# ilovin/lstm_ctc_ocr

Measured on AMD Instinct MI355X. Metric: captcha images/sec training (32x256, bs=64/GPU), higher is better.
Workload: dtype bf16; 1 GPU; VGG-7 + BiLSTM(256) + CTC train step, H=32 W=256, 10-char labels, C=64, bs=64/GPU (BASELINE.json configs[1]), Adam lr 1e-4 wd 1e-5 clip 10; global_batch=64, parallelism=dp1, hipgraph=True

## Files before the change

### include/ocr_hip.h

```cpp
#ifndef OCR_HIP_H
#define OCR_HIP_H
#include <stddef.h>
#ifdef __cplusplus
extern "C" {
#endif

enum { OCR_STATUS_OK = 0, OCR_STATUS_MEMOPS = 1, OCR_STATUS_INVALID = 2, OCR_STATUS_EXEC = 3 };

enum {
    OCR_EPI_BIAS = 1, OCR_EPI_RELU = 2, OCR_EPI_OUT_F32 = 4,
    OCR_EPI_MASK = 16, OCR_EPI_ROWSWAP = 32, OCR_EPI_ACCUM = 64
};

const char* ocr_status_string(int status);
int ocr_abi_version(void);
const char* ocr_build_id(void);

int ocr_ctc_workspace_size(int max_label_len, int max_time, int minibatch, size_t* bytes);
int ocr_ctc_loss(const float* activations, float* gradients, const int* flat_labels, const int* label_lengths,
                 const int* input_lengths, int alphabet_size, int minibatch, int max_time, int max_label_len,
                 int blank_label, float* costs, void* workspace, void* stream);
int ocr_ctc_debug(void* dbg);
int ocr_ctc_train_supported(int alphabet_size, int max_time, int max_label_len);
int ocr_ctc_loss_train(const float* activations, void* grad_ntc_bf16, float scale, const int* flat_labels,
                       const int* label_lengths, const int* input_lengths, int alphabet_size, int minibatch, int max_time,
                       int max_label_len, int blank_label, float* costs, void* stream);
int ocr_set_ctc_engine(int fast);
int ocr_ctc_greedy_decode(const float* activations, const int* input_lengths, int alphabet_size, int minibatch,
                          int max_time, int blank_label, int pad_value, int* decoded, int* decoded_lengths,
                          void* stream);

int ocr_ctc_beam_workspace_size(int alphabet_size, int minibatch, int max_time, int beam_width, size_t* bytes);
int ocr_ctc_beam_decode(const float* activations, const int* input_lengths, int alphabet_size, int minibatch,
                        int max_time, int beam_width, int merge_repeated, int pad_value, int* decoded,
                        int* decoded_lengths, float* neg_log_prob, void* workspace, size_t workspace_bytes, void* stream);

int ocr_gemm_nt_bf16(const void* P, long ldp, const void* Q, long ldq, void* out, long ldo, int M, int N, int K,
                     const float* bias, const void* mask, long ldmask, int flags, int splits, int row_group,
                     int row_skip, int swap_inner, int swap_outer, void* stream);
int ocr_set_gemm_engine(int use_large_tile);
int ocr_conv3x3_bf16(const void* x, const void* wpack, void* y, int Nb, int W, int H, int Cin, int Cout,
                     const float* bias, const void* mask, int flags, void* stream);
int ocr_conv3x3_stats_rows(int Nb, int W, int H, int Cin, int Cout, int flags);
int ocr_conv3x3_bf16_stats(const void* x, const void* wpack, void* y, int Nb, int W, int H, int Cin, int Cout, const float* bias, int flags,
                           float* partials, void* stream);
int ocr_conv3x3_kernel_choice(int Nb, int W, int H, int Cin, int Cout, int flags, int kw, int kh);
int ocr_conv3x3_accum_supported(int Nb, int W, int H, int Cin, int Cout);
int ocr_conv_halo_clock_debug(void* dbg);
int ocr_conv_ws_debug(void* dbg);
int ocr_conv3x3_pool_supported(int Nb, int W, int H, int Cin, int Cout, int kw, int kh);
int ocr_conv3x3_relu_pool_bf16(const void* x, const void* wpack, void* y, void* pooled, int Nb, int W, int H, int Cin, int Cout,
                               const float* bias, int kw, int kh, void* stream);
int ocr_gemm_tn_bf16(const void* A, long lda, const void* B, long ldb, float* out, long ldo, int Mk, int I, int J,
                     int row_group, int row_skip, long a_row_off, float scale, int splits, float* colsum, void* stream);
long ocr_gemm_tn_split_workspace_floats(int Mk, int I, int J);
int ocr_gemm_tn_split_bf16(const void* A, long lda, const void* B, long ldb, float* out, long ldo, int Mk, int I, int J, float scale,
                           float* colsum, float* part, long part_floats, void* stream);
int ocr_gemm_tn_batched_bf16(const void* A, long lda, long strideA, const void* B, long ldb, long strideB, float* out, long ldo,
                             long strideOut, int Mk, int I, int J, int nbatch, float scale, int splits, float* colsum,
                             long strideColsum, void* stream);
typedef struct ocr_tn_job {
    const void* A; long lda; long strideA;
    const void* B; long ldb; long strideB;
    float* out; long ldo; long strideOut;
    float* colsum; long strideColsum;
    int Mk, I, J, nbatch;
    int row_group, row_skip;
    float scale; int reserved;
} ocr_tn_job;
int ocr_gemm_tn_jobs_supported(const ocr_tn_job* jobs, int njobs);
int ocr_gemm_tn_jobs_bf16(const ocr_tn_job* jobs, int njobs, void* stream);
int ocr_set_wgrad_engine(int engine);
int ocr_conv3x3_wgrad_bf16(const void* x, const void* dy, float* dw, float* dbias, int Nb, int W, int H, int Cin,
                           int Cout, int splits, void* stream);
int ocr_conv3x3_wgrad_kernel_choice(int Nb, int W, int H, int Cin, int Cout, int has_workspace, int splits);

int ocr_conv3x3_wgrad_workspace_size(int Nb, int W, int H, int Cin, int Cout, size_t* bytes);
int ocr_conv3x3_wgrad_ws_bf16(const void* x, const void* dy, float* dw, float* dbias, int Nb, int W, int H, int Cin,
                              int Cout, int splits, void* workspace, size_t workspace_bytes, void* stream);
int ocr_conv3x3_wgrad_defer_bf16(const void* x, const void* dy, float* dw, float* dbias, int Nb, int W, int H, int Cin, int Cout,
                                 void* workspace, size_t workspace_bytes, void* job, int* job_blocks, int* deferred, void* stream);
int ocr_wgrad9_reduce_jobs(const void* jobs, int njobs, int total_blocks, void* stream);

int ocr_conv1_fwd(const float* x, const float* w, const float* bias, void* y, int Nb, int W, int H, int Cout,
                  int relu, void* stream);
int ocr_conv1_wgrad(const float* x, const void* dz, float* dw, float* db, int Nb, int W, int H, int Cout,
                    void* stream);
int ocr_eltwise_bf16(int op, const void* a, const void* b, void* out, long n, void* stream);
int ocr_conv1_pool_fwd(const float* x, const float* w, const float* bias, void* p, int Nb, int W, int H, int Cout, void* stream);
int ocr_conv1_pool_fwd_train(const float* x, const float* w, const float* bias, void* p, int Nb, int W, int H, int Cout,
                             void* codes, float* zero, long zero_n, void* ones, long ones_n, void* stream);
int ocr_conv1_pool_bwd_codes(const float* x, const float* w, const float* bias, const void* dp, float* dw, float* db,
                             int Nb, int W, int H, int Cout, const void* codes, void* stream);
int ocr_conv1_pool_bwd_slab_rows(int Nb, int W, int H);
int ocr_conv1_pool_bwd_slab(const float* x, const float* w, const float* bias, const void* dp, int Nb, int W, int H, int Cout,
                            const void* codes, float* slab, void* stream);
int ocr_conv1_pool_bwd(const float* x, const float* w, const float* bias, const void* dp, float* dw, float* db, int Nb,
                       int W, int H, int Cout, void* stream);
int ocr_maxpool_fwd(const void* x, void* y, int Nb, int W, int H, int C, int kw, int kh, void* stream);
int ocr_maxpool_bwd(const void* x, const void* dy, void* dx, int Nb, int W, int H, int C, int kw, int kh,
                    int relu_mask, void* stream);
size_t ocr_bn_workspace_bytes(long M, int C);
int ocr_bn_train_fwd(const void* x, void* y, const float* gamma, const float* beta, float* save_mean,
                     float* save_rstd, long M, int C, float eps, int relu, void* workspace, const void* residual, void* stream);
int ocr_bn_train_bwd(const void* x, const void* y, const void* dy, void* dx, const float* gamma,
                     const float* save_mean, const float* save_rstd, float* dgamma, float* dbeta, long M, int C,
                     int relu, void* workspace, void* stream);
int ocr_bn_train_fwd2(const void* x, void* y, const float* gamma, const float* beta, float* save_mean, float* save_rstd, long M, int C,
                      float eps, int relu, void* workspace, const void* residual, int partial_rows, void* pooled, void* stream);
int ocr_bn_train_bwd2(const void* x, const void* y, const void* dy, void* dx, const float* gamma, const float* save_mean,
                      const float* save_rstd, float* dgamma, float* dbeta, long M, int C, int relu, void* workspace, int pooled_dy,
                      int partial_rows, void* stream);
int ocr_conv3x3_bnbwd_rows(int Nb, int W, int H, int Cin, int Cout);
int ocr_conv3x3_dgrad_bnbwd_bf16(const void* dy, const void* wdgrad, void* dx, int Nb, int W, int H, int Cin, int Cout, const void* mask_y,
                                 const void* z, const float* mean, const float* rstd, float* partials, void* stream);
int ocr_colsum_bf16(const void* a, float* out, long M, int C, long lda, void* stream);
int ocr_pack_transpose(const float* in, void* out, int R, int Cc, long ldin, int lstm_units, void* stream);
int ocr_pack_conv_dgrad(const float* w, void* out, int Cin, int Cout, void* stream);
int ocr_pack_jobs(const void* jobs, int njobs, int total_blocks, void* stream);
int ocr_cast_f32_bf16(const float* in, void* out, long n, void* stream);
int ocr_u8_to_unit_f32(const void* in, float* out, long n, void* stream);
int ocr_step_report(const float* costs, int n, const double* scalars, const void* word_addrs, int nwords, double* out, void* stream);
int ocr_bind_batch(const void* pixels, int pixels_are_u8, float* x, long n_pixels, const int* seq_len, int* seq_len_dst, int n_seq,
                   const int* labels, int* labels_dst, int n_labels, const int* labels_len, int* labels_len_dst, int n_labels_len,
                   void* stream);
int ocr_cast2d_f32_bf16(const float* in, long ldin, void* out, long ldout, int rows, int cols, void* stream);
int ocr_tnc_to_ntc_bf16(const float* in, void* out, int T, int N, int C, float scale, void* stream);
int ocr_conv5_col2im(const void* col, void* dx, int Nb, int W, int HC, void* stream);

int ocr_bn_infer_fwd(const void* x, void* y, const float* gamma, const float* beta, const float* mean, const float* var,
                     long M, int C, float eps, int relu, void* stream);
int ocr_bn_infer_bwd(const void* x, const void* y, const void* dy, void* dx, const float* gamma, const float* mean,
                     const float* var, float* dgamma, float* dbeta, long M, int C, float eps, int relu, void* stream);
int ocr_dropout_bf16(const void* in, void* out, long n, unsigned seed, const void* step_counter, float keep_prob, void* stream);
int ocr_avgpool_bf16(const void* src, void* dst, int Nb, int W, int H, int C, int kw, int kh, int backward, void* stream);
int ocr_subsample_bf16(const void* src, void* dst, int Nb, int W, int H, int C, int Wo, int Ho, int sw, int sh, int ow, int oh,
                       int backward, void* stream);
int ocr_softmax_f32(const float* in, float* out, long rows, int C, void* stream);

int ocr_lstm_fwd_step(const float* xproj, const void* whT_packed, const int* seq_len, void* hout, float* gates,
                      float* cell, int Nb, int T, int U, int step, float forget_bias, int ndir, void* stream);
int ocr_lstm_bwd_step(const void* wh, long ldw, long w_dir_stride, const int* seq_len, const void* dhout,
                      const float* gates, const float* cell, void* dz, float* dc_state, int Nb, int T, int U,
                      int step, int ndir, void* stream);
int ocr_lstm_seq_supported(int Nb, int U);
long ocr_lstm_seq_sync_words(int Nb, int U);
int ocr_lstm_seq_debug(void* dbg );
int ocr_lstm_seq_test_skew(int units, int at);
int ocr_lstm_fwd_seq(const float* xproj, const void* whT_packed, const int* seq_len, void* hout, float* gates,
                     float* cell, int Nb, int T, int U, float forget_bias, void* sync, void* stream);
int ocr_lstm_bwd_seq(const void* wh, long ldw, long w_dir_stride, const int* seq_len, const void* dhout,
                     const float* gates, const float* cell, void* dz, int Nb, int T, int U, void* sync, void* stream);
#define OCR_LSTM_PREPARED 1
int ocr_lstm_fwd_seq2(const float* xproj, const void* whT_packed, const int* seq_len, void* hout, float* gates,
                      float* cell, int Nb, int T, int U, float forget_bias, void* sync, int flags, void* stream);
int ocr_lstm_bwd_seq2(const void* wh, long ldw, long w_dir_stride, const int* seq_len, const void* dhout,
                      const float* gates, const float* cell, void* dz, int Nb, int T, int U, void* sync, int flags, void* stream);
int ocr_lstm_fwd_seq_x_supported(int Nb, int U, int D);
int ocr_lstm_fwd_seq_x(const void* x, const void* wxT_packed, const float* bias_packed, int D, const void* whT_packed,
                       const int* seq_len, void* hout, float* gates, float* cell, int Nb, int T, int U, float forget_bias,
                       void* sync, int flags, void* stream);
int ocr_set_lstm_proto(int proto);
int ocr_set_lstm_ksplit(int waves);
int ocr_lstm_hprev(const void* hout, const int* seq_len, void* hprev, int Nb, int T, int U, int ndir, void* stream);
int ocr_lstm_xh(const void* x, const void* hout, const int* seq_len, void* xh, int Nb, int T, int D, int U, int ndir, void* stream);
int ocr_lstm_pack_bias(const float* b_fw, const float* b_bw , float* out, int U, int ndir, void* stream);

int ocr_optim_scalar_count(void);
int ocr_optim_init(void* scalars , double lr, void* stream);
int ocr_optim_set_lr(void* scalars, double lr, int multiply, void* stream);
int ocr_optim_step(float* params, float* grads, float* state1, float* state2, long n, long reg_begin, long reg_end,
                   float weight_decay, float clip_norm, int solver, float beta1, float beta2, float eps,
                   void* scalars, void* stream);
int ocr_optim_step_guarded(float* params, float* grads, float* state1, float* state2, long n, long reg_begin, long reg_end,
                           float weight_decay, float clip_norm, int solver, float beta1, float beta2, float eps,
                           void* scalars, const void* guard_addrs, int nguard, void* stream);
int ocr_optim_step_guarded2(float* params, float* grads, float* state1, float* state2, long n, long reg_begin, long reg_end,
                            float weight_decay, float clip_norm, int solver, float beta1, float beta2, float eps,
                            void* scalars, const void* guard_addrs, int nguard, const float* drop_flag, void* stream);
int ocr_guard_flag(const void* guard_addrs, int nguard, float* flag_out, void* stream);

int ocr_captcha_synth(const int* params, int n_images, int words_per_image, int max_glyphs, const void* atlas, const int* stamp, int n_stamp,
                      void* out, int W, int out_h, int canvas_cap, int width_cap, void* stream);

int ocr_wgrad9_debug(void* dbg);

int ocr_probe_tr16(const int* addr , int* out , void* stream);
int ocr_probe_xcc(int* out , int nblocks, int threads, void* stream);
int ocr_occupy_cus(int nblocks, int threads, int lds_bytes, float us, void* stream);
int ocr_mfma_busy_probe(float* out, int nblocks, int threads , int iters, long long* clk, void* stream);

#ifdef __cplusplus
}
#endif
#endif
// ... 1 lines not shown
```

### lstm_ctc_ocr_amd/_native.py

```python
import ctypes
import os
import re

_HERE = os.path.dirname(os.path.abspath(__file__))
LIB_PATH = os.environ.get("OCR_NATIVE_LIB") or os.path.join(_HERE, "libocrhip.so")
HEADER_PATH = os.path.join(os.path.dirname(_HERE), "include", "ocr_hip.h")

EPI_BIAS, EPI_RELU, EPI_OUT_F32, EPI_MASK, EPI_ROWSWAP, EPI_ACCUM = 1, 2, 4, 16, 32, 64

_P, _I, _L, _F, _D = ctypes.c_void_p, ctypes.c_int, ctypes.c_long, ctypes.c_float, ctypes.c_double

_SIGS = {
    "ocr_abi_version": ([], _I),
    "ocr_build_id": ([], ctypes.c_char_p),
    "ocr_status_string": ([_I], ctypes.c_char_p),
    "ocr_ctc_workspace_size": ([_I, _I, _I, ctypes.POINTER(ctypes.c_size_t)], _I),
    "ocr_ctc_loss": ([_P, _P, _P, _P, _P, _I, _I, _I, _I, _I, _P, _P, _P], _I),
    "ocr_set_ctc_engine": ([_I], _I),
    "ocr_ctc_debug": ([_P], _I),
    "ocr_ctc_train_supported": ([_I, _I, _I], _I),
    "ocr_ctc_loss_train": ([_P, _P, _F, _P, _P, _P, _I, _I, _I, _I, _I, _P, _P], _I),
    "ocr_ctc_greedy_decode": ([_P, _P, _I, _I, _I, _I, _I, _P, _P, _P], _I),
    "ocr_ctc_beam_workspace_size": ([_I, _I, _I, _I, ctypes.POINTER(ctypes.c_size_t)], _I),
    "ocr_ctc_beam_decode": ([_P, _P, _I, _I, _I, _I, _I, _I, _P, _P, _P, _P, ctypes.c_size_t, _P], _I),
    "ocr_gemm_nt_bf16": ([_P, _L, _P, _L, _P, _L, _I, _I, _I, _P, _P, _L, _I, _I, _I, _I, _I, _I, _P], _I),
    "ocr_set_gemm_engine": ([_I], _I),
    "ocr_gemm_tn_batched_bf16": ([_P, _L, _L, _P, _L, _L, _P, _L, _L, _I, _I, _I, _I, _F, _I, _P, _L, _P], _I),
    "ocr_gemm_tn_jobs_supported": ([_P, _I], _I),
    "ocr_gemm_tn_jobs_bf16": ([_P, _I, _P], _I),
    "ocr_lstm_xh": ([_P, _P, _P, _P, _I, _I, _I, _I, _I, _P], _I),
    "ocr_set_wgrad_engine": ([_I], _I),
    "ocr_conv3x3_bf16": ([_P, _P, _P, _I, _I, _I, _I, _I, _P, _P, _I, _P], _I),
    "ocr_conv_halo_clock_debug": ([_P], _I),
    "ocr_occupy_cus": ([_I, _I, _I, _F, _P], _I),
    "ocr_conv_ws_debug": ([_P], _I),
    "ocr_conv3x3_accum_supported": ([_I, _I, _I, _I, _I], _I),
    "ocr_conv3x3_kernel_choice": ([_I, _I, _I, _I, _I, _I, _I, _I], _I),
    "ocr_conv3x3_pool_supported": ([_I, _I, _I, _I, _I, _I, _I], _I),
    "ocr_conv3x3_relu_pool_bf16": ([_P, _P, _P, _P, _I, _I, _I, _I, _I, _P, _I, _I, _P], _I),
    "ocr_gemm_tn_bf16": ([_P, _L, _P, _L, _P, _L, _I, _I, _I, _I, _I, _L, _F, _I, _P, _P], _I),
    "ocr_gemm_tn_split_workspace_floats": ([_I, _I, _I], _L),
    "ocr_gemm_tn_split_bf16": ([_P, _L, _P, _L, _P, _L, _I, _I, _I, _F, _P, _P, _L, _P], _I),
    "ocr_conv3x3_wgrad_bf16": ([_P, _P, _P, _P, _I, _I, _I, _I, _I, _I, _P], _I),
    "ocr_conv3x3_wgrad_kernel_choice": ([_I, _I, _I, _I, _I, _I, _I], _I),
    "ocr_conv3x3_wgrad_workspace_size": ([_I, _I, _I, _I, _I, ctypes.POINTER(ctypes.c_size_t)], _I),
    "ocr_conv3x3_wgrad_ws_bf16": ([_P, _P, _P, _P, _I, _I, _I, _I, _I, _I, _P, ctypes.c_size_t, _P], _I),
    "ocr_conv3x3_wgrad_defer_bf16": ([_P, _P, _P, _P, _I, _I, _I, _I, _I, _P, ctypes.c_size_t, _P, ctypes.POINTER(_I),
                                      ctypes.POINTER(_I), _P], _I),
    "ocr_wgrad9_reduce_jobs": ([_P, _I, _I, _P], _I),
    "ocr_conv1_fwd": ([_P, _P, _P, _P, _I, _I, _I, _I, _I, _P], _I),
    "ocr_conv1_wgrad": ([_P, _P, _P, _P, _I, _I, _I, _I, _P], _I),
    "ocr_eltwise_bf16": ([_I, _P, _P, _P, _L, _P], _I),
    "ocr_conv1_pool_fwd": ([_P, _P, _P, _P, _I, _I, _I, _I, _P], _I),
    "ocr_conv1_pool_fwd_train": ([_P, _P, _P, _P, _I, _I, _I, _I, _P, _P, _L, _P, _L, _P], _I),
    "ocr_conv1_pool_bwd_codes": ([_P, _P, _P, _P, _P, _P, _I, _I, _I, _I, _P, _P], _I),
    "ocr_conv1_pool_bwd_slab_rows": ([_I, _I, _I], _I),
    "ocr_conv1_pool_bwd_slab": ([_P, _P, _P, _P, _I, _I, _I, _I, _P, _P, _P], _I),
    "ocr_conv1_pool_bwd": ([_P, _P, _P, _P, _P, _P, _I, _I, _I, _I, _P], _I),
    "ocr_maxpool_fwd": ([_P, _P, _I, _I, _I, _I, _I, _I, _P], _I),
    "ocr_maxpool_bwd": ([_P, _P, _P, _I, _I, _I, _I, _I, _I, _I, _P], _I),
    "ocr_bn_workspace_bytes": ([_L, _I], ctypes.c_size_t),
    "ocr_bn_train_fwd": ([_P, _P, _P, _P, _P, _P, _L, _I, _F, _I, _P, _P, _P], _I),
    "ocr_bn_train_bwd": ([_P, _P, _P, _P, _P, _P, _P, _P, _P, _L, _I, _I, _P, _P], _I),
    "ocr_bn_train_fwd2": ([_P, _P, _P, _P, _P, _P, _L, _I, _F, _I, _P, _P, _I, _P, _P], _I),
    "ocr_bn_train_bwd2": ([_P, _P, _P, _P, _P, _P, _P, _P, _P, _L, _I, _I, _P, _I, _I, _P], _I),
    "ocr_conv3x3_bnbwd_rows": ([_I, _I, _I, _I, _I], _I),
    "ocr_conv3x3_dgrad_bnbwd_bf16": ([_P, _P, _P, _I, _I, _I, _I, _I, _P, _P, _P, _P, _P, _P], _I),
    "ocr_conv3x3_stats_rows": ([_I, _I, _I, _I, _I, _I], _I),
    "ocr_conv3x3_bf16_stats": ([_P, _P, _P, _I, _I, _I, _I, _I, _P, _I, _P, _P], _I),
    "ocr_bn_infer_fwd": ([_P, _P, _P, _P, _P, _P, _L, _I, _F, _I, _P], _I),
    "ocr_bn_infer_bwd": ([_P, _P, _P, _P, _P, _P, _P, _P, _P, _L, _I, _F, _I, _P], _I),
    "ocr_dropout_bf16": ([_P, _P, _L, ctypes.c_uint, _P, _F, _P], _I),
    "ocr_avgpool_bf16": ([_P, _P, _I, _I, _I, _I, _I, _I, _I, _P], _I),
    "ocr_subsample_bf16": ([_P, _P, _I, _I, _I, _I, _I, _I, _I, _I, _I, _I, _I, _P], _I),
    "ocr_softmax_f32": ([_P, _P, _L, _I, _P], _I),
    "ocr_colsum_bf16": ([_P, _P, _L, _I, _L, _P], _I),
    "ocr_pack_transpose": ([_P, _P, _I, _I, _L, _I, _P], _I),
    "ocr_pack_conv_dgrad": ([_P, _P, _I, _I, _P], _I),
    "ocr_pack_jobs": ([_P, _I, _I, _P], _I),
    "ocr_cast_f32_bf16": ([_P, _P, _L, _P], _I),
    "ocr_u8_to_unit_f32": ([_P, _P, _L, _P], _I),
    "ocr_step_report": ([_P, _I, _P, _P, _I, _P, _P], _I),
    "ocr_bind_batch": ([_P, _I, _P, _L, _P, _P, _I, _P, _P, _I, _P, _P, _I, _P], _I),
    "ocr_captcha_synth": ([_P, _I, _I, _I, _P, _P, _I, _P, _I, _I, _I, _I, _P], _I),
    "ocr_cast2d_f32_bf16": ([_P, _L, _P, _L, _I, _I, _P], _I),
    "ocr_tnc_to_ntc_bf16": ([_P, _P, _I, _I, _I, _F, _P], _I),
    "ocr_conv5_col2im": ([_P, _P, _I, _I, _I, _P], _I),
    "ocr_lstm_fwd_step": ([_P, _P, _P, _P, _P, _P, _I, _I, _I, _I, _F, _I, _P], _I),
    "ocr_lstm_bwd_step": ([_P, _L, _L, _P, _P, _P, _P, _P, _P, _I, _I, _I, _I, _I, _P], _I),
    "ocr_lstm_seq_supported": ([_I, _I], _I),
    "ocr_lstm_seq_debug": ([_P], _I),
    "ocr_lstm_seq_test_skew": ([_I, _I], _I),
    "ocr_lstm_seq_sync_words": ([_I, _I], _L),
    "ocr_lstm_fwd_seq": ([_P, _P, _P, _P, _P, _P, _I, _I, _I, _F, _P, _P], _I),
    "ocr_lstm_bwd_seq": ([_P, _L, _L, _P, _P, _P, _P, _P, _I, _I, _I, _P, _P], _I),
    "ocr_lstm_fwd_seq2": ([_P, _P, _P, _P, _P, _P, _I, _I, _I, _F, _P, _I, _P], _I),
    "ocr_lstm_fwd_seq_x_supported": ([_I, _I, _I], _I),
    "ocr_lstm_fwd_seq_x": ([_P, _P, _P, _I, _P, _P, _P, _P, _P, _I, _I, _I, _F, _P, _I, _P], _I),
    "ocr_lstm_bwd_seq2": ([_P, _L, _L, _P, _P, _P, _P, _P, _I, _I, _I, _P, _I, _P], _I),
    "ocr_lstm_hprev": ([_P, _P, _P, _I, _I, _I, _I, _P], _I),
    "ocr_lstm_pack_bias": ([_P, _P, _P, _I, _I, _P], _I),
    "ocr_optim_scalar_count": ([], _I),
    "ocr_optim_init": ([_P, _D, _P], _I),
    "ocr_optim_set_lr": ([_P, _D, _I, _P], _I),
    "ocr_optim_step": ([_P, _P, _P, _P, _L, _L, _L, _F, _F, _I, _F, _F, _F, _P, _P], _I),
    "ocr_optim_step_guarded": ([_P, _P, _P, _P, _L, _L, _L, _F, _F, _I, _F, _F, _F, _P, _P, _I, _P], _I),
    "ocr_optim_step_guarded2": ([_P, _P, _P, _P, _L, _L, _L, _F, _F, _I, _F, _F, _F, _P, _P, _I, _P, _P], _I),
    "ocr_guard_flag": ([_P, _I, _P, _P], _I),
    "ocr_wgrad9_debug": ([_P], _I),
    "ocr_probe_tr16": ([_P, _P, _P], _I),
    "ocr_set_lstm_proto": ([_I], _I),
    "ocr_set_lstm_ksplit": ([_I], _I),
    "ocr_probe_xcc": ([_P, _I, _I, _P], _I),
    "ocr_mfma_busy_probe": ([_P, _I, _I, _I, _P, _P], _I),
}


class NativeError(RuntimeError):
    pass


def declared_symbols(header=HEADER_PATH):
    text = open(header).read()
    text = re.sub(r"/\*.*?\*/", "", text, flags=re.S)
    return sorted(set(re.findall(r"\b(ocr_[a-z0-9_]+)\s*\(", text)))


def source_build_id(csrc=os.path.join(_HERE, "csrc"), experiments=False):
    import glob
    import hashlib
    rel = [os.path.basename(f) for f in glob.glob(os.path.join(csrc, "*.hip"))]
    h = hashlib.sha256()
    for f in sorted(rel) + ["common.h", "conv_plan.h", "Makefile"]:
        h.update(open(os.path.join(csrc, f), "rb").read())
    return h.hexdigest()[:16] + ("-exp" if experiments else "")


def build_id():
    return lib().ocr_build_id().decode()


_lib = None


def lib():
    global _lib
    if _lib is None:
        if not os.path.exists(LIB_PATH):
# ... 32 lines not shown
```

### lstm_ctc_ocr_amd/csrc/common.h

```cpp
#pragma once
#include <stdlib.h>
#include <hip/hip_runtime.h>
#include <stdint.h>
#include <atomic>

#define OCR_WAVE 64

enum {
    OCR_OK = 0,
    OCR_ERR_MEMOPS = 1,
    OCR_ERR_INVALID = 2,
    OCR_ERR_EXEC = 3,
};

#define OCR_CHECK_LAUNCH()                                        \
    do {                                                          \
        hipError_t e__ = hipGetLastError();                       \
        if (e__ != hipSuccess) return OCR_ERR_EXEC;               \
    } while (0)

typedef uint16_t bf16_t;
typedef __attribute__((ext_vector_type(8))) __bf16 bf16x8;
typedef __attribute__((ext_vector_type(4))) float f32x4;
typedef __attribute__((ext_vector_type(4))) unsigned int u32x4;
typedef __attribute__((ext_vector_type(2))) unsigned int u32x2;

__device__ __forceinline__ bf16_t f2bf(float f) {
    uint32_t u = __float_as_uint(f);
    if ((u & 0x7fffffffu) > 0x7f800000u) return (bf16_t)((u >> 16) | 0x40);
    u += 0x7fffu + ((u >> 16) & 1u);
    return (bf16_t)(u >> 16);
}
__device__ __forceinline__ float bf2f(bf16_t h) { return __uint_as_float(((uint32_t)h) << 16); }
typedef __attribute__((ext_vector_type(2))) __bf16 bf16x2_t;
__device__ __forceinline__ uint32_t pack_bf2(float lo, float hi) {
    bf16x2_t v = {(__bf16)lo, (__bf16)hi};
    return __builtin_bit_cast(uint32_t, v);
}
__device__ __forceinline__ float bf_lo(uint32_t p) { return __uint_as_float(p << 16); }
__device__ __forceinline__ float bf_hi(uint32_t p) { return __uint_as_float(p & 0xffff0000u); }

__device__ __forceinline__ float wave_sum(float v) {
#pragma unroll
    for (int o = 32; o > 0; o >>= 1) v += __shfl_xor(v, o, 64);
    return v;
}
__device__ __forceinline__ float wave_max(float v) {
#pragma unroll
    for (int o = 32; o > 0; o >>= 1) v = fmaxf(v, __shfl_xor(v, o, 64));
    return v;
}

__device__ __forceinline__ float sigmoidf_(float x) { return __frcp_rn(1.0f + __expf(-x)); }
__device__ __forceinline__ float tanhf_(float x) {
    float e = __expf(-2.0f * fabsf(x));
    float t = (1.0f - e) * __frcp_rn(1.0f + e);
    return copysignf(t, x);
}

static inline const char* ocr_tune_env(const char* name) {
#ifdef OCR_EXPERIMENTS
    return getenv(name);
#else
    (void)name; return nullptr;
#endif
}
__device__ __forceinline__ long long ocr_wall_clock() { return (long long)__builtin_amdgcn_s_memrealtime(); }
__device__ __forceinline__ void ocr_clk_enter(long long* clk) {
    clk[0] = (long long)__builtin_amdgcn_s_memtime(); clk[1] = ocr_wall_clock();
}
__device__ __forceinline__ void ocr_clk_exit(long long* clk) {
    const long long c = (long long)__builtin_amdgcn_s_memtime(), t = ocr_wall_clock();
    clk[2] = c; clk[3] = t;
    clk[4] += c - clk[0]; clk[5] += t - clk[1]; clk[6] += 1;
}
__host__ __device__ static inline int ceil_div(long a, long b) { return (int)((a + b - 1) / b); }

#define OCR_MAX_DEVICES 64
template <auto KERNEL>
static inline hipError_t ocr_allow_lds(int bytes) {
    static std::atomic<int> allowed[OCR_MAX_DEVICES];
    int dev = 0;
    if (hipGetDevice(&dev) != hipSuccess || dev < 0 || dev >= OCR_MAX_DEVICES) return hipErrorInvalidDevice;
    int have = allowed[dev].load(std::memory_order_acquire);
    if (bytes <= have) return hipSuccess;
    const hipError_t e = hipFuncSetAttribute((const void*)KERNEL, hipFuncAttributeMaxDynamicSharedMemorySize, bytes);
    if (e != hipSuccess) return e;
    while (have < bytes && !allowed[dev].compare_exchange_weak(have, bytes, std::memory_order_acq_rel)) {}
    return hipSuccess;
}
```

### lstm_ctc_ocr_amd/csrc/conv_k3.hip

```cpp
#include "conv_plan.h"
#include <type_traits>

enum { K3_BIAS = 1, K3_RELU = 2, K3_MASK = 16, K3_ACCUM = 64 };

struct K3Args {
    const bf16_t* P; const bf16_t* Q;
    int M, N, C;
    int cW, cH;
    bf16_t* out; const float* bias; const bf16_t* mask; int flags;
    bf16_t* pool; int pool_kind;
    int prio;
    const bf16_t* bnz; const float* bn_mean; const float* bn_rstd;
};

#ifdef OCR_EXPERIMENTS
__device__ long long* k3_dbg;
extern "C" int ocr_conv_k3_debug(void* dbg) {
    long long* q = (long long*)dbg;
    return hipMemcpyToSymbol(HIP_SYMBOL(k3_dbg), &q, sizeof(q)) == hipSuccess ? OCR_OK : OCR_ERR_MEMOPS;
}
#define K3_PHASE(slot) do { if (k3_dbg && threadIdx.x == 0) k3_dbg[blockIdx.x * 8 + (slot)] = wall_clock64(); } while (0)
#else
#define K3_PHASE(slot) do { } while (0)
#endif
__device__ long long* g_k3_clk;
int k3_set_clock_debug(void* dbg) {
    long long* p = (long long*)dbg;
    return hipMemcpyToSymbol(HIP_SYMBOL(g_k3_clk), &p, sizeof(p)) == hipSuccess ? OCR_OK : OCR_ERR_EXEC;
}
__device__ __forceinline__ uint32_t k3_max2(uint32_t a, uint32_t b) {
    const uint32_t lo = (bf_lo(b) > bf_lo(a)) ? (b & 0xffffu) : (a & 0xffffu);
    const uint32_t hi = (bf_hi(b) > bf_hi(a)) ? (b & 0xffff0000u) : (a & 0xffff0000u);
    return lo | hi;
}
__device__ __forceinline__ u32x4 k3_max8(u32x4 a, u32x4 b) {
    u32x4 r = {k3_max2(a.x, b.x), k3_max2(a.y, b.y), k3_max2(a.z, b.z), k3_max2(a.w, b.w)};
    return r;
}
typedef __attribute__((address_space(3))) void* lptr_t;
#define K3_OOB 0x80000000u
#define K3_VMWAIT(n) asm volatile("s_waitcnt vmcnt(%0)" ::"n"(n) : "memory")

template <int FM , int BN ,
          int NST , int H ,
          bool SINGLE = false ,
          bool GENW = false ,
          bool BNB = false >
__device__ __forceinline__ void k3_body(const K3Args& g) {
    constexpr int NW = 8, FN = 4, BM = 256;
    constexpr int WN = BN / 64, WMW = 4 / WN;
    static_assert(FM * WMW == 16, "256-pixel tiles");
    constexpr int NC = BM / H, NCB = NC / 16;
    constexpr int PS = (NC + 2 + 7) / 8 * 8;
    constexpr int PPIECES = (H * PS / 8 + NW - 1) / NW * NW;
    constexpr int PBYTES = PPIECES * 1024, PI = PPIECES / NW;
    static_assert(H * PS <= PPIECES * 8 && PI <= 8, "planes fit the padded buffer; one piece per tap");
    constexpr int CBW = NCB / WMW > 0 ? NCB / WMW : 1;
    constexpr int HW = FM / CBW;
    constexpr int WGC = NCB / CBW;
    constexpr bool STATIC_H = HW == H;
    constexpr int QI = BN / 64;
    constexpr int QB = BN * 128, QTOT = NST * QB;
    constexpr int DEPTH = NST - 2;
    extern __shared__ __attribute__((aligned(16))) unsigned char smem[];

    const int tid = threadIdx.x, lane = tid & 63;
    K3_PHASE(0);
    long long* const clk = g_k3_clk;
    if (clk && blockIdx.x == 0 && tid == 0) ocr_clk_enter(clk);
    const int wave = __builtin_amdgcn_readfirstlane(tid >> 6);
    const int kh = wave >> 2, wm = (wave & 3) / WN, wn = (wave & 3) % WN;
    const int C = g.C;
    const int cb0 = (wm % WGC) * CBW, hbase = (wm / WGC) * HW;
    const bool top = STATIC_H || hbase == 0, bot = STATIC_H || hbase + HW == H;

    const int mtiles = g.M / BM, ntiles = (g.N + BN - 1) / BN;
    const int nblk = mtiles * ntiles;
    int Lb = blockIdx.x;
    if ((nblk & 7) == 0) Lb = (Lb & 7) * (nblk >> 3) + (Lb >> 3);
    const int m0 = (Lb / ntiles) * BM, n0 = (Lb % ntiles) * BN;
    const int col0 = m0 / H;
    const bool edge_l = col0 % g.cW == 0, edge_r = (col0 + NC) % g.cW == 0;

    const int rsub = lane >> 3;
    const int csrc = ((lane & 7) ^ rsub) * 8;

    const int pbytes_all = (int)((long)g.M * C * 2);
    const __amdgpu_buffer_rsrc_t qsrd = __builtin_amdgcn_make_buffer_rsrc((void*)g.Q, 0, (int)((long)g.N * 9 * C * 2), 0x00020000);
    unsigned voffQ[QI], voffP[PI];
#pragma unroll
    for (int j = 0; j < QI; ++j) {
        const int n = n0 + (wave * QI + j) * 8 + rsub;
        voffQ[j] = n < g.N ? (unsigned)(((long)n * 9 * C + csrc) * 2) : K3_OOB;
    }
    constexpr int KMAX = 8;
    const int b0w = g.cW - col0 % g.cW;
    auto kof = [&](int c) { int k = 0;
#pragma unroll
        for (int i = 0; i < KMAX; ++i) k += (c >= b0w + i * g.cW) ? 1 : 0;
        return k; };
#pragma unroll
    for (int j = 0; j < PI; ++j) {
        const int r = (j * NW + wave) * 8 + rsub;
        const int h = r / PS, cp = r % PS;
        if (!GENW) {
            const bool ok = h < H && cp < NC + 2 && !(cp == 0 && edge_l) && !(cp == NC + 1 && edge_r);
            const long m = (long)(col0 - 1 + cp) * H + h;
            voffP[j] = ok ? (unsigned)((m * C + csrc) * 2) : K3_OOB;
        } else {
            const int q = cp - 1, last = NC + kof(NC - 1);
            int n = 0; bool pad = false;
#pragma unroll
            for (int i = 0; i < KMAX; ++i) { const int z = b0w + i * g.cW + i; n += (q >= z) ? 1 : 0; pad = pad || q == z; }
            int col = col0 + q - n;
            bool ok = h < H && q >= 0 && q < last && !pad;
            if (h < H && q == -1) { ok = !edge_l; col = col0 - 1; }
            if (h < H && q == last) { ok = !edge_r; col = col0 + NC; }
            const long m = (long)col * H + h;
            voffP[j] = ok ? (unsigned)((m * C + csrc) * 2) : K3_OOB;
        }
    }
    auto load_q = [&](int k0 , int stage) {
#pragma unroll
        for (int j = 0; j < QI; ++j)
            __builtin_amdgcn_raw_ptr_buffer_load_lds(qsrd, (lptr_t)(smem + stage * QB + (wave * QI + j) * 1024), 16, (int)voffQ[j], k0 * 2, 0, 0);
    };
    auto load_p = [&](const __amdgpu_buffer_rsrc_t srd, int chunk, int buf, int j, unsigned voff) {
        __builtin_amdgcn_raw_ptr_buffer_load_lds(srd, (lptr_t)(smem + QTOT + buf * PBYTES + (j * NW + wave) * 1024), 16, (int)voff, chunk * 128, 0, 0);
    };

// ... 113 lines not shown
        if (decltype(khc)::value == 1) comp(std::integral_constant<int, 8>{}, khc);
    };
    if (kh == 0) run(std::integral_constant<int, 0>{}); else run(std::integral_constant<int, 1>{});
    asm volatile("s_waitcnt vmcnt(0)" ::: "memory");
    __syncthreads();
    K3_PHASE(2);

    constexpr int FH = FM / 2;
    auto tail = [&](auto half_c) {
        constexpr int KH = decltype(half_c)::value;
        {
            f32x4* mine = (f32x4*)smem + (size_t)wave * (FN * FH * 64);
            const f32x4* theirs = (const f32x4*)smem + (size_t)(wave ^ 4) * (FN * FH * 64);
#pragma unroll
            for (int a = 0; a < FN; ++a)
#pragma unroll
                for (int b = 0; b < FH; ++b) mine[(a * FH + b) * 64 + lane] = acc[a][(1 - KH) * FH + b];
            __syncthreads();
#pragma unroll
            for (int a = 0; a < FN; ++a)
#pragma unroll
                for (int b = 0; b < FH; ++b) acc[a][KH * FH + b] += theirs[(a * FH + b) * 64 + lane];
        }
        K3_PHASE(3);
        const int flags = g.flags;
        f32x4 bv[FN];
#pragma unroll
        for (int a = 0; a < FN; ++a) {
            const int n = n0 + wn * 64 + a * 16 + (lane >> 4) * 4;
            bv[a] = (f32x4){0.f, 0.f, 0.f, 0.f};
            if ((flags & K3_BIAS) && n < g.N) bv[a] = *(const f32x4*)(g.bias + n);
        }
        if (!(flags & K3_ACCUM)) {
            constexpr int ROWB = BN * 2, U = ROWB / 16, SWM = BN == 128 ? 7 : 3;
            __syncthreads();
#pragma unroll
            for (int bb = 0; bb < FH; ++bb) {
                const int b = KH * FH + bb;
                const int lp = ((cb0 + b % CBW) * 16 + frow) * H + hbase + b / CBW;
#pragma unroll
                for (int a = 0; a < FN; ++a) {
                    f32x4 v = acc[a][b] + bv[a];
                    if (flags & K3_RELU) {
                        v.x = fmaxf(v.x, 0.f); v.y = fmaxf(v.y, 0.f); v.z = fmaxf(v.z, 0.f); v.w = fmaxf(v.w, 0.f);
                    }
                    u32x2 pk;
                    pk.x = pack_bf2(v.x, v.y);
                    pk.y = pack_bf2(v.z, v.w);
                    const int slot = wn * 16 + a * 4 + (lane >> 4);
                    *(u32x2*)(smem + lp * ROWB + ((slot ^ ((frow & SWM) << 2)) << 3)) = pk;
                }
            }
            __syncthreads();
            constexpr int NIT = 256 * U / 512;
            u32x4 val[NIT], mk[NIT], zt[BNB ? NIT : 1];
            float st_s[8] = {0.f, 0.f, 0.f, 0.f, 0.f, 0.f, 0.f, 0.f}, st_q[8] = {0.f, 0.f, 0.f, 0.f, 0.f, 0.f, 0.f, 0.f};
            float bmu[8], brs[8];
            if (BNB) {
#pragma unroll
                for (int c = 0; c < 8; ++c) { bmu[c] = g.bn_mean[n0 + (tid % U) * 8 + c]; brs[c] = g.bn_rstd[n0 + (tid % U) * 8 + c]; }
            }
#pragma unroll
            for (int it = 0; it < NIT; ++it) {
                const int idx = it * 512 + tid, lp = idx / U, u = idx % U;
                if (flags & K3_MASK) mk[it] = *(const u32x4*)(g.mask + ((long)m0 + lp) * g.N + n0 + u * 8);
                if (BNB) zt[it] = *(const u32x4*)(g.bnz + ((long)m0 + lp) * g.N + n0 + u * 8);
                val[it] = *(const u32x4*)(smem + lp * ROWB + ((u ^ (((lp / H) & SWM) << 1)) << 4));
            }
#pragma unroll
            for (int it = 0; it < NIT; ++it) {
                const int idx = it * 512 + tid, lp = idx / U, u = idx % U;
                u32x4 v = val[it];
                if (flags & K3_MASK) {
                    const u32x4 q = mk[it];
                    if (!(bf_lo(q.x) > 0.f)) v.x &= 0xffff0000u;
                    if (!(bf_hi(q.x) > 0.f)) v.x &= 0x0000ffffu;
                    if (!(bf_lo(q.y) > 0.f)) v.y &= 0xffff0000u;
                    if (!(bf_hi(q.y) > 0.f)) v.y &= 0x0000ffffu;
                    if (!(bf_lo(q.z) > 0.f)) v.z &= 0xffff0000u;
                    if (!(bf_hi(q.z) > 0.f)) v.z &= 0x0000ffffu;
                    if (!(bf_lo(q.w) > 0.f)) v.w &= 0xffff0000u;
                    if (!(bf_hi(q.w) > 0.f)) v.w &= 0x0000ffffu;
                }
                *(u32x4*)(g.out + ((long)m0 + lp) * g.N + n0 + u * 8) = v;
                if (!BNB && g.pool_kind == 3) {
                    const float f[8] = {bf_lo(v.x), bf_hi(v.x), bf_lo(v.y), bf_hi(v.y), bf_lo(v.z), bf_hi(v.z), bf_lo(v.w), bf_hi(v.w)};
#pragma unroll
                    for (int c = 0; c < 8; ++c) { st_s[c] += f[c]; st_q[c] = fmaf(f[c], f[c], st_q[c]); }
                } else if (BNB) {
                    const u32x4 z = zt[it];
                    const float f[8] = {bf_lo(v.x), bf_hi(v.x), bf_lo(v.y), bf_hi(v.y), bf_lo(v.z), bf_hi(v.z), bf_lo(v.w), bf_hi(v.w)};
                    const float zf[8] = {bf_lo(z.x), bf_hi(z.x), bf_lo(z.y), bf_hi(z.y), bf_lo(z.z), bf_hi(z.z), bf_lo(z.w), bf_hi(z.w)};
#pragma unroll
                    for (int c = 0; c < 8; ++c) { st_s[c] += f[c]; st_q[c] = fmaf(f[c], (zf[c] - bmu[c]) * brs[c], st_q[c]); }
                }
            }
            if (BNB || g.pool_kind == 3) {
                constexpr int RL = 512 / U;
                float* red = (float*)(smem + 256 * ROWB);
                const int u = tid % U, rl = tid / U;
#pragma unroll
                for (int c = 0; c < 8; ++c) { red[rl * BN + u * 8 + c] = st_s[c]; red[(RL + rl) * BN + u * 8 + c] = st_q[c]; }
                __syncthreads();
                if (tid < 2 * BN) {
                    const int which = tid / BN, ch = tid % BN;
                    float t = 0.f;
                    for (int r = 0; r < RL; ++r) t += red[(which * RL + r) * BN + ch];
                    if (n0 + ch < g.N) ((float*)g.pool)[((long)(m0 / 256) * 2 + which) * g.N + n0 + ch] = t;
                }
            } else if (g.pool_kind) {
                const int kind = g.pool_kind;
                const int nq = kind == 1 ? 128 : 64;
                const long pbase = kind == 1 ? ((long)m0 >> 1) : (long)(col0 >> 1) * (H >> 1);
                for (int idx = tid; idx < nq * U; idx += 512) {
                    const int q = idx / U, u = idx % U;
                    int lp0, cl;
                    if (kind == 1) { lp0 = 2 * q; cl = lp0 / H; }
                    else { cl = 2 * (q / (H >> 1)); lp0 = cl * H + 2 * (q % (H >> 1)); }
                    const unsigned char* r0 = smem + lp0 * ROWB;
                    const int u0 = (u ^ ((cl & SWM) << 1)) << 4;
                    u32x4 m = k3_max8(*(const u32x4*)(r0 + u0), *(const u32x4*)(r0 + ROWB + u0));
                    if (kind == 2) {
                        const int u1 = (u ^ (((cl + 1) & SWM) << 1)) << 4;
                        m = k3_max8(m, k3_max8(*(const u32x4*)(r0 + H * ROWB + u1), *(const u32x4*)(r0 + (H + 1) * ROWB + u1)));
                    }
                    *(u32x4*)(g.pool + (pbase + q) * g.N + n0 + u * 8) = m;
                }
            }
            return;
        }
#pragma unroll
        for (int bb = 0; bb < FH; ++bb) {
            const int b = KH * FH + bb;
            const int h = hbase + b / CBW, col = col0 + (cb0 + b % CBW) * 16 + frow;
            const long m = (long)col * H + h;
#pragma unroll
            for (int a = 0; a < FN; ++a) {
                const int n = n0 + wn * 64 + a * 16 + (lane >> 4) * 4;
                if (n >= g.N) continue;
                f32x4 v = acc[a][b] + bv[a];
                if (flags & K3_RELU) {
                    v.x = fmaxf(v.x, 0.f); v.y = fmaxf(v.y, 0.f); v.z = fmaxf(v.z, 0.f); v.w = fmaxf(v.w, 0.f);
                }
                if (flags & K3_MASK) {
                    u32x2 mk = *(const u32x2*)(g.mask + m * g.N + n);
                    if (!(bf_lo(mk.x) > 0.f)) v.x = 0.f;
                    if (!(bf_hi(mk.x) > 0.f)) v.y = 0.f;
                    if (!(bf_lo(mk.y) > 0.f)) v.z = 0.f;
                    if (!(bf_hi(mk.y) > 0.f)) v.w = 0.f;
                }
                if (flags & K3_ACCUM) {
                    const u32x2 old = *(const u32x2*)(g.out + m * g.N + n);
                    v.x += bf_lo(old.x); v.y += bf_hi(old.x); v.z += bf_lo(old.y); v.w += bf_hi(old.y);
                }
                u32x2 pk;
                pk.x = pack_bf2(v.x, v.y);
                pk.y = pack_bf2(v.z, v.w);
                *(u32x2*)(g.out + m * g.N + n) = pk;
            }
        }
    };
    if (kh) tail(std::integral_constant<int, 1>{}); else tail(std::integral_constant<int, 0>{});
    if (clk && blockIdx.x == 0 && tid == 0) ocr_clk_exit(clk);
#ifdef OCR_EXPERIMENTS
    K3_PHASE(4);
    asm volatile("s_waitcnt vmcnt(0)" ::: "memory");
    K3_PHASE(5);
#endif
}

template <int FM, int BN, int NST, int H, bool SINGLE = false>
__global__ __launch_bounds__(512) __attribute__((amdgpu_waves_per_eu(2, 2))) void conv_k3_kernel(K3Args g) { k3_body<FM, BN, NST, H, SINGLE, false>(g); }
template <int FM, int BN, int NST, int H>
__global__ __launch_bounds__(512) __attribute__((amdgpu_waves_per_eu(2, 2))) void conv_k3w_kernel(K3Args g) { k3_body<FM, BN, NST, H, false, true>(g); }
template <int FM, int BN, int NST, int H, bool GENW>
__global__ __launch_bounds__(512) __attribute__((amdgpu_waves_per_eu(2, 2))) void conv_k3b_kernel(K3Args g) { k3_body<FM, BN, NST, H, false, GENW, true>(g); }

template <int FM, int BN, int NST, int H, bool GENW>
static int run_k3b(const K3Args& g, hipStream_t stream) {
    constexpr int PS = (256 / H + 2 + 7) / 8 * 8, PPIECES = (H * PS / 8 + 7) / 8 * 8;
    constexpr int need = NST * BN * 128 + 2 * PPIECES * 1024, xch = 8 * (FM / 2) * 4 * 1024, lds = need > xch ? need : xch;
    static_assert(lds <= 163840 && 256 * BN * 2 + 2 * (512 / (BN / 8)) * BN * 4 <= lds, "LDS");
    if (ocr_allow_lds<conv_k3b_kernel<FM, BN, NST, H, GENW>>(lds) != hipSuccess) return OCR_ERR_EXEC;
    conv_k3b_kernel<FM, BN, NST, H, GENW><<<(g.M / 256) * ((g.N + BN - 1) / BN), 512, lds, stream>>>(g);
    OCR_CHECK_LAUNCH();
    return OCR_OK;
}

template <int FM, int BN, int NST, int H, bool SINGLE = false, bool GENW = false>
static int run_k3(const K3Args& g, hipStream_t stream) {
    constexpr int PS = (256 / H + 2 + 7) / 8 * 8, PPIECES = (H * PS / 8 + 7) / 8 * 8;
    constexpr int need = NST * BN * 128 + (SINGLE ? 1 : 2) * PPIECES * 1024;
    constexpr int xch = 8 * (FM / 2) * 4 * 1024;
    constexpr int lds = need > xch ? need : xch;
    static_assert(lds <= 163840, "LDS");
    static_assert(256 * BN * 2 + 2 * (512 / (BN / 8)) * BN * 4 <= lds, "staged image + the statistics scratch behind it");
    const int mt = g.M / 256, nt = (g.N + BN - 1) / BN;
    if constexpr (GENW) {
        if (ocr_allow_lds<conv_k3w_kernel<FM, BN, NST, H>>(lds) != hipSuccess) return OCR_ERR_EXEC;
        conv_k3w_kernel<FM, BN, NST, H><<<mt * nt, 512, lds, stream>>>(g);
    } else {
        if (ocr_allow_lds<conv_k3_kernel<FM, BN, NST, H, SINGLE>>(lds) != hipSuccess) return OCR_ERR_EXEC;
        conv_k3_kernel<FM, BN, NST, H, SINGLE><<<mt * nt, 512, lds, stream>>>(g);
    }
    OCR_CHECK_LAUNCH();
    return OCR_OK;
}

int launch_k3(const ConvPlan& p, const ConvOperands& o, hipStream_t stream) {
    const K3Args g = {(const bf16_t*)o.x, (const bf16_t*)o.wpack, p.M, p.Cout, p.Cin, p.W, p.H, (bf16_t*)o.y, o.bias, (const bf16_t*)o.mask,
                      p.flags, (bf16_t*)o.pool, p.epi_kind, p.prio, (const bf16_t*)o.bnz, o.bn_mean, o.bn_rstd};
    const int H = p.H;
    const bool A = p.tile == 'A';
    if (p.epi_kind == CONV_EPI_BNBWD) {
        if (A) {
            if (p.genw) return H == 4 ? run_k3b<8, 128, 5, 4, true>(g, stream) : run_k3b<8, 128, 5, 8, true>(g, stream);
            return H == 4 ? run_k3b<8, 128, 5, 4, false>(g, stream) : run_k3b<8, 128, 5, 8, false>(g, stream);
        }
        if (p.genw) return H == 4 ? run_k3b<4, 64, 4, 4, true>(g, stream) : run_k3b<4, 64, 4, 8, true>(g, stream);
        return H == 4 ? run_k3b<4, 64, 4, 4, false>(g, stream) : run_k3b<4, 64, 4, 8, false>(g, stream);
    }
    if (p.genw) {
        if (A) return H == 2 ? run_k3<8, 128, 5, 2, false, true>(g, stream) : H == 4 ? run_k3<8, 128, 5, 4, false, true>(g, stream)
                                                                                   : run_k3<8, 128, 5, 8, false, true>(g, stream);
        return H == 2 ? run_k3<4, 64, 4, 2, false, true>(g, stream) : H == 4 ? run_k3<4, 64, 4, 4, false, true>(g, stream)
                                                                               : run_k3<4, 64, 4, 8, false, true>(g, stream);
    }
    if (A) {
        if (H == 16) return p.single ? run_k3<8, 128, 5, 16, true>(g, stream) : run_k3<8, 128, 4, 16>(g, stream);
        return H == 4 ? run_k3<8, 128, 5, 4>(g, stream) : run_k3<8, 128, 5, 8>(g, stream);
    }
    if (H == 16) return p.single ? run_k3<4, 64, 4, 16, true>(g, stream) : run_k3<4, 64, 4, 16>(g, stream);
    return H == 4 ? run_k3<4, 64, 4, 4>(g, stream) : run_k3<4, 64, 4, 8>(g, stream);
}
```

### lstm_ctc_ocr_amd/csrc/conv_plan.h

```cpp
#pragma once
#include "common.h"

enum {
    CONV_GEMM = 0,
    CONV_HALO = 1,
    CONV_K2 = 2,
    CONV_K3 = 4,
    CONV_WS = 8,
};
enum {
    CONV_EPI_PLAIN = 0,
    CONV_EPI_POOL12 = 1,
    CONV_EPI_POOL22 = 2,
    CONV_EPI_STATS = 3,
    CONV_EPI_BNBWD = 4,
};

struct ConvPlan {
    int family;
    int M, W, H, Cin, Cout;
    int flags, epi_kind;
    char tile;
    int bn, nw;
    bool genw;
    bool single;
    int ws_nc, ws_ksplit;
    int grid, slots, per_slot, xcd_map;
    int prio, stagger, stagger_bit, abl;
    int nst;
    int choice() const {
        if (family == CONV_K2) return CONV_K2 + (tile == 'D');
        if (family == CONV_K3) return CONV_K3 + (tile == 'D') + 2 * genw;
        return family;
    }
};
ConvPlan conv3x3_plan(int M, int W, int H, int Cin, int Cout, int flags, int epi_kind);

struct ConvOperands {
    const void* x; const void* wpack; void* y;
    const float* bias; const void* mask;
    void* pool;
    const void* bnz; const float* bn_mean; const float* bn_rstd;
};
int launch_halo(const ConvPlan& p, const ConvOperands& o, hipStream_t stream);
int launch_k2(const ConvPlan& p, const ConvOperands& o, hipStream_t stream);
int launch_k3(const ConvPlan& p, const ConvOperands& o, hipStream_t stream);
int launch_ws(const ConvPlan& p, const ConvOperands& o, hipStream_t stream);
```

### lstm_ctc_ocr_amd/csrc/conv_ws.hip

```cpp
#include "conv_plan.h"
#include <type_traits>

enum { WS_BIAS = 1, WS_RELU = 2, WS_MASK = 16, WS_ACCUM = 64 };

struct WsArgs {
    const bf16_t* P; const bf16_t* Q;
    int M, N, C, cW, cH;
    bf16_t* out; const float* bias; const bf16_t* mask; int flags;
    bf16_t* pool; int pool_kind;
    int ntiles, slots, per_slot, xcd_map;
};

typedef __attribute__((address_space(3))) void* ws_lptr_t;
#define WS_OOB 0x80000000u

__device__ long long* g_ws_dbg;
extern "C" int ocr_conv_ws_debug(void* dbg) {
    long long* q = (long long*)dbg;
    return hipMemcpyToSymbol(HIP_SYMBOL(g_ws_dbg), &q, sizeof(q)) == hipSuccess ? OCR_OK : OCR_ERR_MEMOPS;
}
#define WS_PHASE(slot) do { if (wsdbg && tid == 0 && (slot) < 64) wsdbg[blockIdx.x * 64 + (slot)] = ocr_wall_clock(); } while (0)
__device__ long long* g_ws_clk;
int ws_set_clock_debug(void* dbg) {
    long long* p = (long long*)dbg;
    return hipMemcpyToSymbol(HIP_SYMBOL(g_ws_clk), &p, sizeof(p)) == hipSuccess ? OCR_OK : OCR_ERR_EXEC;
}

typedef short ws_s16x2 __attribute__((ext_vector_type(2)));
__device__ __forceinline__ uint32_t ws_max2(uint32_t a, uint32_t b) {
    return __builtin_bit_cast(uint32_t, __builtin_elementwise_max(__builtin_bit_cast(ws_s16x2, a), __builtin_bit_cast(ws_s16x2, b)));
}
__device__ __forceinline__ u32x4 ws_max8(u32x4 a, u32x4 b) {
    u32x4 r = {ws_max2(a.x, b.x), ws_max2(a.y, b.y), ws_max2(a.z, b.z), ws_max2(a.w, b.w)};
    return r;
}

template <int H, int NC, int KSPLIT>
struct WsCfg {
    static constexpr int BM = NC * H;
    static constexpr int PG = 4 / KSPLIT;
    static constexpr int CF = NC < 16 ? NC : 16;
    static constexpr int HF = 16 / CF;
    static constexpr int HW = 4 * HF;
    static constexpr int PS = NC + 2;
    static constexpr int CHB = (H + 2) * PS * 128;
    static constexpr int BUFB = KSPLIT * CHB;
    static constexpr int PPC = H * PS / 8;
    static constexpr int PI = KSPLIT * PPC / 4;
    static constexpr int NFE = 4 / KSPLIT;
    static constexpr int HWE = NFE * HF;
    static constexpr int NPE = NC * HWE;
    static constexpr int XOFF = 2 * BUFB;
    static constexpr int SOFF = XOFF + (KSPLIT == 2 ? 4 * 8192 : 0);
    static constexpr int STW = NPE * 128;
    static constexpr int TOFF = SOFF + 4 * STW;
    static constexpr int BOFF = TOFF + 4 * PI * 128;
    static constexpr int MOFF = BOFF + 256;
    static constexpr int LDS_PLAIN = MOFF, LDS_MASK = MOFF + 4 * STW;
    static_assert(((NC + 1) * H + H) * 128 * 2 / 16 * 4 < 65536, "table entries fit 16 bits");
    static_assert(NC == CF && PG * HW == H && (H * PS) % 8 == 0 && (KSPLIT * PPC) % 4 == 0 && LDS_MASK <= 163840, "geometry");
    static_assert(((H + 1) * PS) * 128 < 65536, "ds_read immediates");
};

template <int H, int NC, int KSPLIT, bool MASK >
__global__ __launch_bounds__(256) __attribute__((amdgpu_waves_per_eu(1, 1))) void conv_ws_kernel(WsArgs g) {
    using G = WsCfg<H, NC, KSPLIT>;
    constexpr int CF = G::CF, HF = G::HF, PS = G::PS, PI = G::PI, HWE = G::HWE, NPE = G::NPE;
    extern __shared__ __attribute__((aligned(16))) unsigned char smem[];

    const int tid = threadIdx.x, lane = tid & 63, lane_id = lane;
    long long* const clk = g_ws_clk;
    long long* const wsdbg = g_ws_dbg;
    if (clk && blockIdx.x == 0 && tid == 0) ocr_clk_enter(clk);
    WS_PHASE(0);
    const int wave = __builtin_amdgcn_readfirstlane(tid >> 6);
    const int pg = KSPLIT == 1 ? wave : (wave & 1), kh = KSPLIT == 1 ? 0 : (wave >> 1);
    const int C = g.C, N = g.N;

    int id = blockIdx.x, nt, slot;
    if (g.xcd_map) {
        const int per_xcd = (int)gridDim.x >> 3, j = id >> 3;
        nt = j % g.ntiles; slot = (id & 7) * (per_xcd / g.ntiles) + j / g.ntiles;
    } else { nt = id % g.ntiles; slot = id / g.ntiles; }
    const int n0 = nt * 64;
    const int mtiles = g.M / G::BM;
    const int t_begin = slot * g.per_slot;
    int t_end = t_begin + g.per_slot; if (t_end > mtiles) t_end = mtiles;

    const int frow = lane & 15, fq = lane >> 4;
    const int rsub = lane >> 3;
    const unsigned lds0 = (unsigned)(size_t)(ws_lptr_t)smem;

    unsigned short* const dtab = (unsigned short*)(smem + G::TOFF) + wave * PI * 64 + lane;
#pragma unroll
    for (int j = 0; j < PI; ++j) {
        const int q = j * 4 + wave;
        const int c = q / G::PPC, pc = q % G::PPC;
        const int r = pc * 8 + rsub;
        const int h = r / PS, cp = r % PS;
        const unsigned off = (unsigned)((((cp * H + h) * C + c * 64) + (((lane & 7) ^ (cp & 7)) << 3)) * 2);
        dtab[j * 64] = (unsigned short)((off >> 2) | (cp == 0 ? 1u : 0u) | (cp == NC + 1 ? 2u : 0u));
    }
    if (tid < 64) ((float*)(smem + G::BOFF))[tid] = (g.flags & WS_BIAS) ? g.bias[n0 + tid] : 0.f;
    const long pbytes = (long)g.M * C * 2;
    unsigned e_[PI];
    auto read_table = [&]() {
#pragma unroll
        for (int j = 0; j < PI; ++j) e_[j] = dtab[j * 64];
    };
    auto issue_halo = [&](int t, int buf, auto partc) {
        constexpr int PART = decltype(partc)::value;
        const int col0 = t * NC;
        const bool edge_l = col0 % g.cW == 0, edge_r = (col0 + NC) % g.cW == 0;
        const long base = (long)(col0 - 1) * H * C * 2;
        long left = pbytes - base; if (left > 0x7fffffffL) left = 0x7fffffffL;
        const __amdgpu_buffer_rsrc_t srd = __builtin_amdgcn_make_buffer_rsrc((void*)((const char*)g.P + base), 0, (int)left, 0x00020000);
        const unsigned em = (edge_l ? 1u : 0u) | (edge_r ? 2u : 0u);
#pragma unroll
        for (int j = (PART < 0 ? 0 : PART); j < (PART < 0 ? PI : PART + 1); ++j) {
            const int q = j * 4 + wave;
            const unsigned e = e_[j];
            const unsigned v = (e & em) ? WS_OOB : ((e & ~3u) << 2);
            __builtin_amdgcn_raw_ptr_buffer_load_lds(srd, (ws_lptr_t)(smem + buf * G::BUFB + (q / G::PPC) * G::CHB + PS * 128 + (q % G::PPC) * 1024), 16, (int)v, 0, 0, 0);
        }
    };

    unsigned pb[3][2];
    {
        const int colf = frow % CF, hsub = frow / CF;
#pragma unroll
        for (int d = 0; d < 3; ++d)
#pragma unroll
            for (int j = 0; j < 2; ++j) {
                const int cp = colf + d;
                pb[d][j] = lds0 + kh * G::CHB + ((pg * 4 * HF + hsub) * PS + cp) * 128 + (((j * 4 + fq) ^ (cp & 7)) << 4);
            }
    }

    asm volatile("s_waitcnt lgkmcnt(0)" ::: "memory");
    read_table();
    if (t_begin < t_end) issue_halo(t_begin, 0, std::integral_constant<int, -1>{});

    u32x4 wq[4][18];
    {
        constexpr int NSH = 4 / KSPLIT, R = KSPLIT == 1 ? 2 : 4, FR = 72 / R, OWN = 72 / NSH;
        static_assert(KSPLIT * FR * 1024 <= G::BUFB && FR % NSH == 0, "a round fits buffer 1");
        const int rank = KSPLIT == 1 ? wave : pg;
// ... 61 lines not shown
#pragma unroll
        for (int a = 0; a < 4; ++a) {
            binit[a] = *(const f32x4*)(smem + G::BOFF + (a * 16 + fq * 4) * 4);
            if (KSPLIT == 2 && kh) binit[a] = (f32x4){0.f, 0.f, 0.f, 0.f};
        }
        asm volatile("s_waitcnt lgkmcnt(0)" : "+v"(binit[0]), "+v"(binit[1]), "+v"(binit[2]), "+v"(binit[3]));
        f32x4 acc[4][4];
        u32x4 bfr[2][4];
#define WS_RD(S_, DST_) do { \
            constexpr int TAP_ = (S_) >> 1, J_ = (S_) & 1, DW_ = TAP_ / 3, DH_ = TAP_ % 3 - 1; \
            asm volatile("ds_read_b128 %0, %1 offset:%2" : "=v"(DST_[0]) : "v"(pb[DW_][J_]), "n"(((0 * HF + 1 + DH_) * PS) * 128)); \
            asm volatile("ds_read_b128 %0, %1 offset:%2" : "=v"(DST_[1]) : "v"(pb[DW_][J_]), "n"(((1 * HF + 1 + DH_) * PS) * 128)); \
            asm volatile("ds_read_b128 %0, %1 offset:%2" : "=v"(DST_[2]) : "v"(pb[DW_][J_]), "n"(((2 * HF + 1 + DH_) * PS) * 128)); \
            asm volatile("ds_read_b128 %0, %1 offset:%2" : "=v"(DST_[3]) : "v"(pb[DW_][J_]), "n"(((3 * HF + 1 + DH_) * PS) * 128)); \
        } while (0)
#define WS_MM(S_, SRC_, FIRST_) do { \
            _Pragma("unroll") for (int b = 0; b < 4; ++b) \
            _Pragma("unroll") for (int a = 0; a < 4; ++a) \
                acc[a][b] = __builtin_amdgcn_mfma_f32_16x16x32_bf16(__builtin_bit_cast(bf16x8, wq[a][S_]), __builtin_bit_cast(bf16x8, SRC_[b]), \
                                                                    (FIRST_) ? binit[a] : acc[a][b], 0, 0, 0); \
        } while (0)
#define WS_WAIT(N_, SRC_) asm volatile("s_waitcnt lgkmcnt(" #N_ ")" : "+v"(SRC_[0]), "+v"(SRC_[1]), "+v"(SRC_[2]), "+v"(SRC_[3]))
#define WS_STEP(S_) do { \
            WS_RD((S_) + 1, bfr[((S_) + 1) & 1]); \
            WS_WAIT(4, bfr[(S_) & 1]);               \
            WS_MM(S_, bfr[(S_) & 1], (S_) == 0); \
            __builtin_amdgcn_sched_barrier(0); \
        } while (0)
        WS_RD(0, bfr[0]);
        WS_STEP(0); WS_STEP(1); WS_STEP(2); WS_STEP(3); WS_STEP(4); WS_STEP(5); WS_STEP(6); WS_STEP(7); WS_STEP(8);
        WS_STEP(9); WS_STEP(10); WS_STEP(11); WS_STEP(12); WS_STEP(13); WS_STEP(14); WS_STEP(15); WS_STEP(16);
        WS_WAIT(0, bfr[1]);
        WS_MM(17, bfr[1], false);
        __builtin_amdgcn_sched_barrier(0);
#undef WS_STEP
#undef WS_WAIT
#undef WS_MM
#undef WS_RD
        WS_PHASE(ph0 + 2);
        asm volatile("s_waitcnt vmcnt(0)" ::: "memory");
        WS_PHASE(ph0 + 3);

        auto tail = [&](auto khc) {
            constexpr int KH = decltype(khc)::value;
            constexpr int B0 = KSPLIT == 2 ? 2 * KH : 0;
            if (KSPLIT == 2) {
                f32x4* mine = (f32x4*)(smem + G::XOFF) + (size_t)wave * 512;
                const f32x4* theirs = (const f32x4*)(smem + G::XOFF) + (size_t)(wave ^ 2) * 512;
#pragma unroll
                for (int a = 0; a < 4; ++a)
#pragma unroll
                    for (int i = 0; i < 2; ++i) mine[(a * 2 + i) * 64 + lane_id] = acc[a][2 * (1 - KH) + i];
                asm volatile("s_waitcnt lgkmcnt(0)" ::: "memory");
                __builtin_amdgcn_s_barrier();
                asm volatile("" ::: "memory");
#pragma unroll
                for (int a = 0; a < 4; ++a)
#pragma unroll
                    for (int i = 0; i < 2; ++i) acc[a][B0 + i] += theirs[(a * 2 + i) * 64 + lane_id];
            }
            WS_PHASE(ph0 + 4);
            int lane = lane_id;
            asm volatile("" : "+v"(lane));
            const int frow = lane & 15, fq = lane >> 4;
            unsigned char* const S = smem + G::SOFF + wave * G::STW;
            const int colf = frow % CF, hsub = frow / CF;
            const bool relu = (g.flags & WS_RELU) != 0;
#pragma unroll
            for (int i = 0; i < G::NFE; ++i) {
                const int row = colf * HWE + i * HF + hsub;
#pragma unroll
                for (int a = 0; a < 4; ++a) {
                    const f32x4 v = acc[a][B0 + i];
                    u32x2 pk;
                    pk.x = pack_bf2(v.x, v.y);
                    pk.y = pack_bf2(v.z, v.w);
                    if (relu) { pk.x = ws_max2(pk.x, 0u); pk.y = ws_max2(pk.y, 0u); }
                    const int slot = a * 4 + fq;
                    *(u32x2*)(S + row * 128 + ((slot ^ ((colf & 3) << 2)) << 3)) = pk;
                }
            }
            asm volatile("s_waitcnt lgkmcnt(0)" ::: "memory");
            u32x4 val[NIT], mkv[MASK ? NIT : 1];
#pragma unroll
            for (int it = 0; it < NIT; ++it) {
                const int idx = it * 64 + lane, row = idx >> 3, u = idx & 7;
                val[it] = *(const u32x4*)(S + row * 128 + ((u ^ (((row / HWE) & 3) << 1)) << 4));
                if (has_mask) mkv[it] = *(const u32x4*)(smem + G::MOFF + wave * G::STW + idx * 16);
            }
#pragma unroll
            for (int it = 0; it < NIT; ++it) {
                const int idx = it * 64 + lane, row = idx >> 3, u = idx & 7;
                u32x4 v = val[it];
                if (has_mask) {
                    const u32x4 q = mkv[it];
                    if (!(bf_lo(q.x) > 0.f)) v.x &= 0xffff0000u;
                    if (!(bf_hi(q.x) > 0.f)) v.x &= 0x0000ffffu;
                    if (!(bf_lo(q.y) > 0.f)) v.y &= 0xffff0000u;
                    if (!(bf_hi(q.y) > 0.f)) v.y &= 0x0000ffffu;
                    if (!(bf_lo(q.z) > 0.f)) v.z &= 0xffff0000u;
                    if (!(bf_hi(q.z) > 0.f)) v.z &= 0x0000ffffu;
                    if (!(bf_lo(q.w) > 0.f)) v.w &= 0xffff0000u;
                    if (!(bf_hi(q.w) > 0.f)) v.w &= 0x0000ffffu;
                }
                const long m = (long)(col0 + row / HWE) * H + h_lo + row % HWE;
                *(u32x4*)(g.out + m * N + n0 + u * 8) = v;
            }
            if (g.pool_kind == 1) {
                constexpr int NQ = NC * (HWE / 2), PIT = NQ * 8 / 64;
                static_assert(NQ * 8 % 64 == 0, "whole wave iterations");
                u32x4 p0[PIT], p1[PIT];
#pragma unroll
                for (int it = 0; it < PIT; ++it) {
                    const int idx = it * 64 + lane, q = idx >> 3, u = idx & 7, col = q / (HWE / 2), ph = q % (HWE / 2);
                    const unsigned char* r0 = S + (col * HWE + 2 * ph) * 128 + ((u ^ ((col & 3) << 1)) << 4);
                    p0[it] = *(const u32x4*)r0; p1[it] = *(const u32x4*)(r0 + 128);
                }
#pragma unroll
                for (int it = 0; it < PIT; ++it) {
                    const int idx = it * 64 + lane, q = idx >> 3, u = idx & 7, col = q / (HWE / 2), ph = q % (HWE / 2);
                    const long pm = (long)(col0 + col) * (H / 2) + (h_lo >> 1) + ph;
                    *(u32x4*)(g.pool + pm * N + n0 + u * 8) = ws_max8(p0[it], p1[it]);
                }
            } else if (g.pool_kind == 2) {
                constexpr int NQ = (NC / 2) * (HWE / 2), PIT = NQ * 8 / 64;
                static_assert(NQ * 8 % 64 == 0, "whole wave iterations");
                u32x4 p0[PIT], p1[PIT], p2[PIT], p3[PIT];
#pragma unroll
                for (int it = 0; it < PIT; ++it) {
                    const int idx = it * 64 + lane, q = idx >> 3, u = idx & 7, pc = q / (HWE / 2), ph = q % (HWE / 2);
                    const int c0 = 2 * pc, c1 = c0 + 1;
                    const unsigned char* r0 = S + (c0 * HWE + 2 * ph) * 128 + ((u ^ ((c0 & 3) << 1)) << 4);
                    const unsigned char* r1 = S + (c1 * HWE + 2 * ph) * 128 + ((u ^ ((c1 & 3) << 1)) << 4);
                    p0[it] = *(const u32x4*)r0; p1[it] = *(const u32x4*)(r0 + 128); p2[it] = *(const u32x4*)r1; p3[it] = *(const u32x4*)(r1 + 128);
                }
#pragma unroll
                for (int it = 0; it < PIT; ++it) {
                    const int idx = it * 64 + lane, q = idx >> 3, u = idx & 7, pc = q / (HWE / 2), ph = q % (HWE / 2);
                    const long pm = (long)((col0 >> 1) + pc) * (H / 2) + (h_lo >> 1) + ph;
                    *(u32x4*)(g.pool + pm * N + n0 + u * 8) = ws_max8(ws_max8(p0[it], p1[it]), ws_max8(p2[it], p3[it]));
                }
            }
        };
        if (KSPLIT == 2 && kh) tail(std::integral_constant<int, 1>{}); else tail(std::integral_constant<int, 0>{});
        WS_PHASE(ph0 + 5);
        const unsigned flip = buf ? (unsigned)-G::BUFB : (unsigned)G::BUFB;
#pragma unroll
        for (int d = 0; d < 3; ++d)
#pragma unroll
            for (int j = 0; j < 2; ++j) pb[d][j] += flip;
    }
    if (clk && blockIdx.x == 0 && tid == 0) ocr_clk_exit(clk);
}

template <int H, int NC, int KSPLIT, bool MASK>
static int launch_ws_(const WsArgs& g, int grid, hipStream_t stream) {
    using G = WsCfg<H, NC, KSPLIT>;
    constexpr int lds = MASK ? G::LDS_MASK : G::LDS_PLAIN;
    if (ocr_allow_lds<conv_ws_kernel<H, NC, KSPLIT, MASK>>(lds) != hipSuccess) return OCR_ERR_EXEC;
    conv_ws_kernel<H, NC, KSPLIT, MASK><<<grid, 256, lds, stream>>>(g);
    OCR_CHECK_LAUNCH();
    return OCR_OK;
}
template <int H, int NC, int KSPLIT>
static int launch_ws(const WsArgs& g, int grid, hipStream_t stream) {
    return (g.flags & WS_MASK) ? launch_ws_<H, NC, KSPLIT, true>(g, grid, stream) : launch_ws_<H, NC, KSPLIT, false>(g, grid, stream);
}
int launch_ws(const ConvPlan& p, const ConvOperands& o, hipStream_t stream) {
    const WsArgs g = {(const bf16_t*)o.x, (const bf16_t*)o.wpack, p.M, p.Cout, p.Cin, p.W, p.H, (bf16_t*)o.y, o.bias, (const bf16_t*)o.mask,
                      p.flags, (bf16_t*)o.pool, p.epi_kind, p.Cout / 64, p.slots, p.per_slot, p.xcd_map};
    if (p.H == 16 && p.ws_ksplit == 1) return launch_ws<16, 16, 1>(g, p.grid, stream);
    if (p.H == 16) return launch_ws<16, 8, 2>(g, p.grid, stream);
    return launch_ws<8, 16, 2>(g, p.grid, stream);
}
```

### lstm_ctc_ocr_amd/csrc/gemm.hip

```cpp
#include "conv_plan.h"
#include <string.h>

enum {
    EPI_BIAS = 1,
    EPI_RELU = 2,
    EPI_OUT_F32 = 4,
    EPI_ATOMIC = 8,
    EPI_MASK = 16,
    EPI_ROWSWAP = 32,
    EPI_ACCUM = 64,
};

struct GemmArgs {
    const bf16_t* P;
    const bf16_t* Q;
    long ldp, ldq;
    int M, N, K;
    int k_per_split;
    int grp, skip;
    int cW, cH, cC;
    void* out;
    long ldo;
    const float* bias;
    const bf16_t* mask;
// ... 390 lines not shown
        if (M % (epi_kind == CONV_EPI_POOL22 ? 2 * H : 2)) return p;
    }
    if (k.k2 && plan_k3_k2(p, k)) return p;
    plan_halo(p, k);
    return p;
}

static int conv3x3_launch(const ConvPlan& p, const ConvOperands& o, hipStream_t stream) {
    switch (p.family) {
    case CONV_WS: return launch_ws(p, o, stream);
    case CONV_K3: return launch_k3(p, o, stream);
    case CONV_K2: return launch_k2(p, o, stream);
    case CONV_HALO: return launch_halo(p, o, stream);
    }
    return OCR_ERR_INVALID;
}
static int conv3x3_pixels(int Nb, int W, int H, int Cin, int Cout) {
    const long M = (long)Nb * W * H;
    return (Nb <= 0 || W <= 0 || H <= 0 || Cin <= 0 || Cout <= 0 || M > 0x7fffffffL) ? 0 : (int)M;
}

extern "C" int ocr_conv3x3_accum_supported(int Nb, int W, int H, int Cin, int Cout) {
    return conv3x3_plan(conv3x3_pixels(Nb, W, H, Cin, Cout), W, H, Cin, Cout, EPI_ACCUM, CONV_EPI_PLAIN).family != CONV_GEMM;
}
extern "C" int ocr_conv3x3_kernel_choice(int Nb, int W, int H, int Cin, int Cout, int flags, int kw, int kh) {
    if (Nb <= 0 || W <= 0 || H <= 0 || Cin <= 0 || Cout <= 0) return -OCR_ERR_INVALID;
    const int pool_kind = (kw == 1 && kh == 2) ? 1 : ((kw == 2 && kh == 2) ? 2 : 0);
    if ((kw || kh) && !pool_kind) return 0;
    return conv3x3_plan(Nb * W * H, W, H, Cin, Cout, flags & ~(EPI_ATOMIC | EPI_ROWSWAP), pool_kind).choice();
}

extern "C" int ocr_conv3x3_bf16(const void* x, const void* wpack, void* y, int Nb, int W, int H,
                                int Cin, int Cout, const float* bias, const void* mask, int flags,
                                void* stream) {
    GemmArgs g = {};
    g.P = (const bf16_t*)x; g.Q = (const bf16_t*)wpack; g.ldp = Cin; g.ldq = 9L * Cin;
    g.M = Nb * W * H; g.N = Cout; g.K = 9 * Cin; g.cW = W; g.cH = H; g.cC = Cin;
    g.out = y; g.ldo = Cout; g.bias = bias; g.mask = (const bf16_t*)mask; g.ldmask = Cout;
    g.flags = flags & ~(EPI_ATOMIC | EPI_ROWSWAP);
    if ((flags & EPI_BIAS) && !bias) return OCR_ERR_INVALID;
    if ((flags & EPI_MASK) && !mask) return OCR_ERR_INVALID;
    if ((flags & EPI_ACCUM) && !ocr_conv3x3_accum_supported(Nb, W, H, Cin, Cout)) return OCR_ERR_INVALID;
    if (!x || !wpack || !y || g.M <= 0 || Cout <= 0 || Cin <= 0) return dispatch_gemm(g, 1, 1, (hipStream_t)stream);
    const ConvPlan p = conv3x3_plan(g.M, W, H, Cin, Cout, g.flags, CONV_EPI_PLAIN);
    if (p.family != CONV_GEMM) return conv3x3_launch(p, {x, wpack, y, bias, mask}, (hipStream_t)stream);
    if (g_use_igemm) {
        int rc = ig_try_dispatch(x, Cin, wpack, 9L * Cin, y, Cout, g.M, Cout, 9 * Cin, bias, mask, Cout, g.flags, 1, 0, 0, W, H, Cin,
                                 0, 0, (hipStream_t)stream);
        if (rc >= 0) return rc;
    }
    return dispatch_gemm(g, 1, 1, (hipStream_t)stream);
}
extern "C" int ocr_conv3x3_stats_rows(int Nb, int W, int H, int Cin, int Cout, int flags) {
    const int M = conv3x3_pixels(Nb, W, H, Cin, Cout);
    return conv3x3_plan(M, W, H, Cin, Cout, flags & ~(EPI_ATOMIC | EPI_ROWSWAP), CONV_EPI_STATS).family != CONV_GEMM ? M / 256 : 0;
}
extern "C" int ocr_conv3x3_bf16_stats(const void* x, const void* wpack, void* y, int Nb, int W, int H, int Cin, int Cout, const float* bias,
                                      int flags, float* partials, void* stream) {
    if (!x || !wpack || !y || !partials || ((flags & EPI_BIAS) && !bias) || !ocr_conv3x3_stats_rows(Nb, W, H, Cin, Cout, flags)) return OCR_ERR_INVALID;
    const ConvPlan p = conv3x3_plan(Nb * W * H, W, H, Cin, Cout, flags & ~(EPI_ATOMIC | EPI_ROWSWAP), CONV_EPI_STATS);
    return conv3x3_launch(p, {x, wpack, y, bias, nullptr, partials}, (hipStream_t)stream);
}
extern "C" int ocr_conv3x3_bnbwd_rows(int Nb, int W, int H, int Cin, int Cout) {
    const int M = conv3x3_pixels(Nb, W, H, Cin, Cout);
    return conv3x3_plan(M, W, H, Cin, Cout, EPI_MASK, CONV_EPI_BNBWD).family != CONV_GEMM ? M / 256 : 0;
}
extern "C" int ocr_conv3x3_dgrad_bnbwd_bf16(const void* dy, const void* wdgrad, void* dx, int Nb, int W, int H, int Cin, int Cout, const void* mask_y,
                                            const void* z, const float* mean, const float* rstd, float* partials, void* stream) {
    if (!dy || !wdgrad || !dx || !mask_y || !z || !mean || !rstd || !partials || !ocr_conv3x3_bnbwd_rows(Nb, W, H, Cin, Cout)) return OCR_ERR_INVALID;
    const ConvPlan p = conv3x3_plan(Nb * W * H, W, H, Cin, Cout, EPI_MASK, CONV_EPI_BNBWD);
    return conv3x3_launch(p, {dy, wdgrad, dx, nullptr, mask_y, partials, z, mean, rstd}, (hipStream_t)stream);
}
static int conv3x3_pool_kind(int kw, int kh) { return (kw == 1 && kh == 2) ? 1 : ((kw == 2 && kh == 2) ? 2 : 0); }
extern "C" int ocr_conv3x3_pool_supported(int Nb, int W, int H, int Cin, int Cout, int kw, int kh) {
    const int kind = conv3x3_pool_kind(kw, kh);
    return kind && conv3x3_plan(conv3x3_pixels(Nb, W, H, Cin, Cout), W, H, Cin, Cout, EPI_BIAS | EPI_RELU, kind).family != CONV_GEMM;
}
extern "C" int ocr_conv3x3_relu_pool_bf16(const void* x, const void* wpack, void* y, void* pooled, int Nb, int W, int H, int Cin,
                                          int Cout, const float* bias, int kw, int kh, void* stream) {
    if (!x || !wpack || !y || !pooled || !bias || !ocr_conv3x3_pool_supported(Nb, W, H, Cin, Cout, kw, kh)) return OCR_ERR_INVALID;
    const ConvPlan p = conv3x3_plan(Nb * W * H, W, H, Cin, Cout, EPI_BIAS | EPI_RELU, conv3x3_pool_kind(kw, kh));
    return conv3x3_launch(p, {x, wpack, y, bias, nullptr, pooled}, (hipStream_t)stream);
}
```

### lstm_ctc_ocr_amd/csrc/nn_ops.hip

```cpp
#include "common.h"
#include <stdlib.h>

__device__ __forceinline__ void unpack8(u32x4 p, float* f) {
    f[0] = bf_lo(p.x); f[1] = bf_hi(p.x); f[2] = bf_lo(p.y); f[3] = bf_hi(p.y);
    f[4] = bf_lo(p.z); f[5] = bf_hi(p.z); f[6] = bf_lo(p.w); f[7] = bf_hi(p.w);
}

__global__ __launch_bounds__(256) void conv1_fwd_kernel(const float* __restrict__ x,
                                                        const float* __restrict__ w,
                                                        const float* __restrict__ bias,
                                                        bf16_t* __restrict__ y, int Nb, int W, int H,
                                                        int Cout, int relu) {
    const int groups = Cout >> 3;
    const int gq = threadIdx.x % groups;
    const int plane = threadIdx.x / groups;
    const int planes = 256 / groups;
    float wr[9][8], br[8];
#pragma unroll
    for (int t = 0; t < 9; ++t)
#pragma unroll
        for (int c = 0; c < 8; ++c) wr[t][c] = w[t * Cout + gq * 8 + c];
#pragma unroll
    for (int c = 0; c < 8; ++c) br[c] = bias[gq * 8 + c];
    const long npix = (long)Nb * W * H;
// ... 428 lines not shown
}
__device__ __forceinline__ u32x4 max8(u32x4 a, u32x4 b) {
    u32x4 r = {max2(a.x, b.x), max2(a.y, b.y), max2(a.z, b.z), max2(a.w, b.w)};
    return r;
}

template <int KW, int KH>
__global__ __launch_bounds__(256) void maxpool_fwd_kernel(const bf16_t* __restrict__ x, bf16_t* __restrict__ y,
                                                          int Nb, int W, int H, int C) {
    constexpr int kw = KW, kh = KH;
    const int Wo = W / kw, Ho = H / kh, groups = C >> 3;
    const long total = (long)Nb * Wo * Ho * groups;
    for (long idx = (long)blockIdx.x * 256 + threadIdx.x; idx < total; idx += (long)gridDim.x * 256) {
        int gq = (int)(idx % groups);
        long op = idx / groups;
        int ho = (int)(op % Ho);
        long q = op / Ho;
        int wo = (int)(q % Wo);
        long n = q / Wo;
        const bf16_t* base = x + (((n * W + (long)wo * kw) * H) + (long)ho * kh) * C + gq * 8;
        u32x4 m = *(const u32x4*)base;
#pragma unroll
        for (int a = 0; a < kw; ++a)
#pragma unroll
            for (int b = 0; b < kh; ++b) {
                if (a == 0 && b == 0) continue;
                m = max8(m, *(const u32x4*)(base + ((long)a * H + b) * C));
            }
        *(u32x4*)(y + op * C + gq * 8) = m;
    }
}

template <int KW, int KH>
__global__ __launch_bounds__(256) void maxpool_bwd_kernel(const bf16_t* __restrict__ x, const bf16_t* __restrict__ dy,
                                                          bf16_t* __restrict__ dx, int Nb, int W, int H, int C,
                                                          int relu_mask) {
    constexpr int kw = KW, kh = KH, cnt_all = KW * KH;
    const int Wo = W / kw, Ho = H / kh, groups = C >> 3;
    const long total = (long)Nb * Wo * Ho * groups;
    for (long idx = (long)blockIdx.x * 256 + threadIdx.x; idx < total; idx += (long)gridDim.x * 256) {
        int gq = (int)(idx % groups);
        long op = idx / groups;
        int ho = (int)(op % Ho);
        long q = op / Ho;
        int wo = (int)(q % Wo);
        long n = q / Wo;
        long boff = (((n * W + (long)wo * kw) * H) + (long)ho * kh) * C + gq * 8;
        float xv[cnt_all][8];
#pragma unroll
        for (int a = 0; a < kw; ++a)
#pragma unroll
            for (int b = 0; b < kh; ++b) {
                u32x4 v = *(const u32x4*)(x + boff + ((long)a * H + b) * C);
                unpack8(v, xv[a * kh + b]);
            }
        float g[8];
        unpack8(*(const u32x4*)(dy + op * C + gq * 8), g);
        int win[8];
#pragma unroll
        for (int c = 0; c < 8; ++c) {
            int best = 0; float bv = xv[0][c];
#pragma unroll
            for (int e = 1; e < cnt_all; ++e) if (xv[e][c] > bv) { bv = xv[e][c]; best = e; }
            win[c] = best;
        }
#pragma unroll
        for (int a = 0; a < kw; ++a)
#pragma unroll
            for (int b = 0; b < kh; ++b) {
                const int cnt = a * kh + b;
                float o[8];
#pragma unroll
                for (int c = 0; c < 8; ++c) {
                    float v = (win[c] == cnt) ? g[c] : 0.f;
                    if (relu_mask && !(xv[cnt][c] > 0.f)) v = 0.f;
                    o[c] = v;
                }
                u32x4 pk = {pack_bf2(o[0], o[1]), pack_bf2(o[2], o[3]), pack_bf2(o[4], o[5]), pack_bf2(o[6], o[7])};
                *(u32x4*)(dx + boff + ((long)a * H + b) * C) = pk;
            }
    }
}

template <typename AccT, bool STORE = false>
__device__ __forceinline__ void block_channel_reduce(const float (&v)[8], float* red, AccT* dst, int C, int groups,
                                                     int rl, int gq, int rlanes) {
    __syncthreads();
    if (rl < rlanes) {
#pragma unroll
        for (int c = 0; c < 8; ++c) red[rl * C + gq * 8 + c] = v[c];
    }
    __syncthreads();
    for (int ch = threadIdx.x; ch < C; ch += 256) {
        float t = 0.f;
        for (int r = 0; r < rlanes; ++r) t += red[r * C + ch];
        if (STORE) dst[ch] = (AccT)t;
        else atomicAdd(&dst[ch], (AccT)t);
    }
}

static int bn_rows_per_block_host(long M, int target) {
    long r = (M + target - 1) / target;
    r = (r + 7) / 8 * 8;
    return (int)(r < 8 ? 8 : r);
}
__global__ __launch_bounds__(256) void bn_stats_kernel(const bf16_t* __restrict__ x, float* __restrict__ part,
                                                       long M, int C, int rows_per_block) {
    const int groups = C >> 3;
    const int rl = threadIdx.x / groups;
    const int gq = threadIdx.x % groups;
    const int rlanes = 256 / groups;
    const long r0 = (long)blockIdx.x * rows_per_block, r1 = min(M, r0 + rows_per_block);
    float s[8], ss[8];
#pragma unroll
    for (int c = 0; c < 8; ++c) { s[c] = 0.f; ss[c] = 0.f; }
    if (rl < rlanes) {
#pragma unroll 4
        for (long r = r0 + rl; r < r1; r += rlanes) {
            float v[8];
            unpack8(*(const u32x4*)(x + r * C + gq * 8), v);
#pragma unroll
            for (int c = 0; c < 8; ++c) { s[c] += v[c]; ss[c] = fmaf(v[c], v[c], ss[c]); }
        }
    }
    __shared__ float red[2048];
    float* dst = part + (long)blockIdx.x * 2 * C;
    block_channel_reduce<float, true>(s, red, dst, C, groups, rl, gq, rlanes);
    block_channel_reduce<float, true>(ss, red, dst + C, C, groups, rl, gq, rlanes);
}
__device__ __forceinline__ bool bn_pair_sum(const float* __restrict__ part, int nblk, int C, double& t0, double& t1, int& ch) {
    __shared__ double red[2][16][17];
    const int cl = threadIdx.x & 15, rl = threadIdx.x >> 4;
    ch = blockIdx.x * 16 + cl;
    double a0 = 0, a1 = 0;
    if (ch < C) {
#pragma unroll 4
        for (int b = rl; b < nblk; b += 16) {
            a0 += (double)part[(long)b * 2 * C + ch];
            a1 += (double)part[(long)b * 2 * C + C + ch];
        }
    }
    red[0][rl][cl] = a0; red[1][rl][cl] = a1;
    __syncthreads();
    if (rl != 0 || ch >= C) return false;
    t0 = 0; t1 = 0;
#pragma unroll
    for (int r = 0; r < 16; ++r) { t0 += red[0][r][cl]; t1 += red[1][r][cl]; }
    return true;
}
__global__ __launch_bounds__(256) void bn_finalize_kernel(const float* __restrict__ part, int nblk, float* __restrict__ mean,
                                                          float* __restrict__ rstd, long M, int C, float eps) {
    double s, ss; int c;
    if (bn_pair_sum(part, nblk, C, s, ss, c)) {
        double mu = s / (double)M;
        double var = ss / (double)M - mu * mu;
        if (var < 0) var = 0;
        mean[c] = (float)mu;
        rstd[c] = (float)(1.0 / sqrt(var + (double)eps));
    }
}
__global__ __launch_bounds__(256) void bn_apply_kernel(const bf16_t* __restrict__ x, bf16_t* __restrict__ y,
                                                       const float* __restrict__ mean, const float* __restrict__ rstd,
                                                       const float* __restrict__ gamma, const float* __restrict__ beta,
                                                       long M, int C, int relu, int rows_per_block, const bf16_t* __restrict__ res) {
    const int groups = C >> 3;
    const int rl = threadIdx.x / groups, gq = threadIdx.x % groups, rlanes = 256 / groups;
    if (rl >= rlanes) return;
    float mu[8], rs[8], gm[8], bt[8];
#pragma unroll
    for (int c = 0; c < 8; ++c) {
        const int ch = gq * 8 + c;
        mu[c] = mean[ch]; rs[c] = rstd[ch]; gm[c] = gamma[ch]; bt[c] = beta[ch];
    }
    const long r0 = (long)blockIdx.x * rows_per_block, r1 = min(M, r0 + rows_per_block);
#pragma unroll 4
    for (long r = r0 + rl; r < r1; r += rlanes) {
        float v[8], o[8];
        unpack8(*(const u32x4*)(x + r * C + gq * 8), v);
#pragma unroll
        for (int c = 0; c < 8; ++c) o[c] = (v[c] - mu[c]) * rs[c] * gm[c] + bt[c];
        if (res != nullptr) {
            float q[8];
            unpack8(*(const u32x4*)(res + r * C + gq * 8), q);
            u32x4 rb = {pack_bf2(o[0], o[1]), pack_bf2(o[2], o[3]), pack_bf2(o[4], o[5]), pack_bf2(o[6], o[7])};
            unpack8(rb, o);
#pragma unroll
            for (int c = 0; c < 8; ++c) o[c] += q[c];
        }
        if (relu) {
#pragma unroll
            for (int c = 0; c < 8; ++c) o[c] = fmaxf(o[c], 0.f);
        }
        u32x4 pk = {pack_bf2(o[0], o[1]), pack_bf2(o[2], o[3]), pack_bf2(o[4], o[5]), pack_bf2(o[6], o[7])};
        *(u32x4*)(y + r * C + gq * 8) = pk;
    }
}
__global__ __launch_bounds__(256) void bn_apply_pool_kernel(const bf16_t* __restrict__ x, bf16_t* __restrict__ y, bf16_t* __restrict__ pooled,
                                                            const float* __restrict__ mean, const float* __restrict__ rstd,
                                                            const float* __restrict__ gamma, const float* __restrict__ beta,
                                                            long M, int C, int relu, int pairs_per_block) {
    const int groups = C >> 3;
    const int rl = threadIdx.x / groups, gq = threadIdx.x % groups, rlanes = 256 / groups;
    if (rl >= rlanes) return;
    float mu[8], rs[8], gm[8], bt[8];
#pragma unroll
    for (int c = 0; c < 8; ++c) {
        const int ch = gq * 8 + c;
        mu[c] = mean[ch]; rs[c] = rstd[ch]; gm[c] = gamma[ch]; bt[c] = beta[ch];
    }
    const long q0 = (long)blockIdx.x * pairs_per_block, q1 = min(M >> 1, q0 + pairs_per_block);
#pragma unroll 2
    for (long q = q0 + rl; q < q1; q += rlanes) {
        u32x4 pk[2];
#pragma unroll
        for (int e = 0; e < 2; ++e) {
            float v[8], o[8];
            unpack8(*(const u32x4*)(x + (2 * q + e) * C + gq * 8), v);
#pragma unroll
            for (int c = 0; c < 8; ++c) {
                o[c] = (v[c] - mu[c]) * rs[c] * gm[c] + bt[c];
                if (relu) o[c] = fmaxf(o[c], 0.f);
            }
            pk[e] = (u32x4){pack_bf2(o[0], o[1]), pack_bf2(o[2], o[3]), pack_bf2(o[4], o[5]), pack_bf2(o[6], o[7])};
            *(u32x4*)(y + (2 * q + e) * C + gq * 8) = pk[e];
        }
        *(u32x4*)(pooled + q * C + gq * 8) = max8(pk[0], pk[1]);
    }
}
__device__ __forceinline__ void bn_pool_route(const bf16_t* __restrict__ y, const bf16_t* __restrict__ dp, long r, int C, int gq,
                                              const float (&yv)[8], float (&g)[8]) {
    float other[8];
    unpack8(*(const u32x4*)(y + (r ^ 1) * C + gq * 8), other);
    unpack8(*(const u32x4*)(dp + (r >> 1) * C + gq * 8), g);
    const bool odd = (r & 1) != 0;
#pragma unroll
    for (int c = 0; c < 8; ++c) {
        const bool win = odd ? (yv[c] > other[c]) : !(other[c] > yv[c]);
        if (!win) g[c] = 0.f;
    }
}
__global__ __launch_bounds__(256) void bn_bwd_stats_kernel(const bf16_t* __restrict__ x, const bf16_t* __restrict__ y,
                                                           const bf16_t* __restrict__ dy, const float* __restrict__ mean,
                                                           const float* __restrict__ rstd, float* __restrict__ part,
                                                           long M, int C, int rows_per_block, int relu, int pooled) {
    const int groups = C >> 3;
    const int rl = threadIdx.x / groups, gq = threadIdx.x % groups, rlanes = 256 / groups;
    const long r0 = (long)blockIdx.x * rows_per_block, r1 = min(M, r0 + rows_per_block);
    float s[8], sx[8], mu[8], rs[8];
#pragma unroll
    for (int c = 0; c < 8; ++c) { s[c] = 0.f; sx[c] = 0.f; mu[c] = mean[gq * 8 + c]; rs[c] = rstd[gq * 8 + c]; }
    if (rl < rlanes) {
#pragma unroll 4
        for (long r = r0 + rl; r < r1; r += rlanes) {
            float xv[8], yv[8], g[8];
            unpack8(*(const u32x4*)(x + r * C + gq * 8), xv);
            if (relu || pooled) unpack8(*(const u32x4*)(y + r * C + gq * 8), yv);
            if (pooled) bn_pool_route(y, dy, r, C, gq, yv, g);
            else unpack8(*(const u32x4*)(dy + r * C + gq * 8), g);
            if (relu) {
#pragma unroll
                for (int c = 0; c < 8; ++c) if (!(yv[c] > 0.f)) g[c] = 0.f;
            }
#pragma unroll
            for (int c = 0; c < 8; ++c) { s[c] += g[c]; sx[c] = fmaf(g[c], (xv[c] - mu[c]) * rs[c], sx[c]); }
        }
    }
    __shared__ float red[2048];
    float* dst = part + (long)blockIdx.x * 2 * C;
    block_channel_reduce<float, true>(s, red, dst, C, groups, rl, gq, rlanes);
    block_channel_reduce<float, true>(sx, red, dst + C, C, groups, rl, gq, rlanes);
}
__global__ __launch_bounds__(256) void bn_bwd_finalize_kernel(const float* __restrict__ part, int nblk, double* __restrict__ sums,
                                                              float* __restrict__ dgamma, float* __restrict__ dbeta, int C) {
    double s, sx; int c;
    if (bn_pair_sum(part, nblk, C, s, sx, c)) {
        sums[c] = s; sums[C + c] = sx;
        dbeta[c] += (float)s;
        dgamma[c] += (float)sx;
    }
}
__global__ __launch_bounds__(256) void bn_bwd_apply_kernel(const bf16_t* __restrict__ x, const bf16_t* __restrict__ y,
                                                           const bf16_t* __restrict__ dy, bf16_t* __restrict__ dx,
                                                           const float* __restrict__ mean, const float* __restrict__ rstd,
                                                           const float* __restrict__ gamma, const double* __restrict__ sums,
                                                           float* __restrict__ dgamma, float* __restrict__ dbeta,
                                                           long M, int C, int relu, int rows_per_block, int pooled) {
    const int groups = C >> 3;
    const int rl = threadIdx.x / groups, gq = threadIdx.x % groups, rlanes = 256 / groups;
    if (rl >= rlanes) return;
    const double invM = 1.0 / (double)M;
    float mu[8], rs[8], gr[8], mdz[8], mdzx[8];
#pragma unroll
    for (int c = 0; c < 8; ++c) {
        const int ch = gq * 8 + c;
        mu[c] = mean[ch]; rs[c] = rstd[ch]; gr[c] = gamma[ch] * rstd[ch];
        mdz[c] = (float)(sums[ch] * invM); mdzx[c] = (float)(sums[C + ch] * invM);
    }
    const long r0 = (long)blockIdx.x * rows_per_block, r1 = min(M, r0 + rows_per_block);
#pragma unroll 2
    for (long r = r0 + rl; r < r1; r += rlanes) {
        float xv[8], yv[8], g[8], o[8];
        unpack8(*(const u32x4*)(x + r * C + gq * 8), xv);
        if (relu || pooled) unpack8(*(const u32x4*)(y + r * C + gq * 8), yv);
        if (pooled) bn_pool_route(y, dy, r, C, gq, yv, g);
        else unpack8(*(const u32x4*)(dy + r * C + gq * 8), g);
        if (relu) {
#pragma unroll
            for (int c = 0; c < 8; ++c) if (!(yv[c] > 0.f)) g[c] = 0.f;
        }
#pragma unroll
        for (int c = 0; c < 8; ++c) {
            float xh = (xv[c] - mu[c]) * rs[c];
            o[c] = gr[c] * (g[c] - mdz[c] - xh * mdzx[c]);
        }
        u32x4 pk = {pack_bf2(o[0], o[1]), pack_bf2(o[2], o[3]), pack_bf2(o[4], o[5]), pack_bf2(o[6], o[7])};
        *(u32x4*)(dx + r * C + gq * 8) = pk;
    }
}

#ifdef OCR_EXPERIMENTS
struct BnBar { unsigned cnt[16][32]; unsigned gen[16][32]; unsigned gcnt[32]; unsigned timeouts[32]; };
__device__ BnBar bn_bar;
__device__ __forceinline__ bool bn_grid_barrier(unsigned nblocks) {
    __syncthreads();
    __shared__ int ok_s;
    if (threadIdx.x == 0) {
        int ok = 1;
        __threadfence();
        const unsigned g = blockIdx.x & 15u, ngroups = nblocks < 16u ? nblocks : 16u, ng = (nblocks - g + 15u) >> 4;
        const unsigned gen = __hip_atomic_load(&bn_bar.gen[g][0], __ATOMIC_RELAXED, __HIP_MEMORY_SCOPE_AGENT);
        const unsigned prev = __hip_atomic_fetch_add(&bn_bar.cnt[g][0], 1u, __ATOMIC_RELAXED, __HIP_MEMORY_SCOPE_AGENT);
        bool released = false;
        if (prev == ng - 1) {
            __hip_atomic_store(&bn_bar.cnt[g][0], 0u, __ATOMIC_RELAXED, __HIP_MEMORY_SCOPE_AGENT);
            const unsigned gp = __hip_atomic_fetch_add(&bn_bar.gcnt[0], 1u, __ATOMIC_RELAXED, __HIP_MEMORY_SCOPE_AGENT);
            if (gp == ngroups - 1) {
                __hip_atomic_store(&bn_bar.gcnt[0], 0u, __ATOMIC_RELAXED, __HIP_MEMORY_SCOPE_AGENT);
                for (unsigned k = 0; k < ngroups; ++k) __hip_atomic_store(&bn_bar.gen[k][0], gen + 1u, __ATOMIC_RELAXED, __HIP_MEMORY_SCOPE_AGENT);
                released = true;
            }
        }
        if (!released) {
            long spins = 0;
            while (__hip_atomic_load(&bn_bar.gen[g][0], __ATOMIC_RELAXED, __HIP_MEMORY_SCOPE_AGENT) == gen) {
                __builtin_amdgcn_s_sleep(2);
                if (++spins > (1L << 22)) { ok = 0; atomicAdd(&bn_bar.timeouts[0], 1u); break; }
            }
        }
        __threadfence();
        ok_s = ok;
    }
    __syncthreads();
    return ok_s != 0;
}
constexpr int BNF_NIT = 16;
__device__ __forceinline__ void bnf_pair_total(const float* __restrict__ part, int nblk, int C, int ch, double* red , double& t0, double& t1) {
    double a0 = 0, a1 = 0;
    for (int b = threadIdx.x; b < nblk; b += 256) { a0 += (double)part[(long)b * 2 * C + ch]; a1 += (double)part[(long)b * 2 * C + C + ch]; }
    red[threadIdx.x] = a0; red[256 + threadIdx.x] = a1;
    __syncthreads();
    for (int s = 128; s > 0; s >>= 1) {
        if (threadIdx.x < s) { red[threadIdx.x] += red[threadIdx.x + s]; red[256 + threadIdx.x] += red[256 + threadIdx.x + s]; }
        __syncthreads();
    }
    t0 = red[0]; t1 = red[256];
    __syncthreads();
}
__global__ __launch_bounds__(256) void bn_fused_fwd_kernel(const bf16_t* __restrict__ x, bf16_t* __restrict__ y, const float* __restrict__ gamma,
                                                           const float* __restrict__ beta, float* __restrict__ mean, float* __restrict__ rstd,
                                                           float* __restrict__ part, long M, int C, float eps, int relu, int rows_per_block,
                                                           const bf16_t* __restrict__ res) {
    const int groups = C >> 3, rl = threadIdx.x / groups, gq = threadIdx.x % groups, rlanes = 256 / groups;
    const long r0 = (long)blockIdx.x * rows_per_block, r1 = min(M, r0 + rows_per_block);
    const bool act = rl < rlanes;
    u32x4 v[BNF_NIT];
    float s[8], ss[8];
#pragma unroll
    for (int c = 0; c < 8; ++c) { s[c] = 0.f; ss[c] = 0.f; }
#pragma unroll
    for (int i = 0; i < BNF_NIT; ++i) {
        const long r = r0 + rl + (long)i * rlanes;
        v[i] = (u32x4){0, 0, 0, 0};
        if (act && r < r1) v[i] = *(const u32x4*)(x + r * C + gq * 8);
    }
#pragma unroll
    for (int i = 0; i < BNF_NIT; ++i) {
        float f[8];
        unpack8(v[i], f);
#pragma unroll
        for (int c = 0; c < 8; ++c) { s[c] += f[c]; ss[c] = fmaf(f[c], f[c], ss[c]); }
    }
// ... 440 lines not shown
                                                                                                 zero_n / 4, nullptr, (u32x4*)ones, ones_n / 4);
    }
    OCR_CHECK_LAUNCH();
    return OCR_OK;
}
extern "C" int ocr_conv1_pool_fwd(const float* x, const float* w, const float* bias, void* p, int Nb, int W, int H, int Cout,
                                  void* stream) {
    return conv1_pool_fwd_impl(x, w, bias, p, Nb, W, H, Cout, nullptr, 0, nullptr, nullptr, 0, stream);
}
extern "C" int ocr_conv1_pool_fwd_train(const float* x, const float* w, const float* bias, void* p, int Nb, int W, int H, int Cout,
                                        void* codes, float* zero, long zero_n, void* ones, long ones_n, void* stream) {
    return conv1_pool_fwd_impl(x, w, bias, p, Nb, W, H, Cout, zero, zero_n, codes, ones, ones_n, stream);
}
static int conv1_ppb() {
    static int v = -1;
    if (v < 0) { const char* e = getenv("OCR_CONV1_PPB"); v = e ? atoi(e) : 256; if (v < 32 || v > 1024 || (v & 31)) v = 256; }
    return v;
}
static int conv1_pool_bwd_impl(const float* x, const float* w, const float* bias, const void* dp, float* dw, float* db,
                               int Nb, int W, int H, int Cout, const void* codes, float* slab, void* stream) {
    if (!x || !w || !bias || !dp || (!slab && (!dw || !db)) || Cout != 64 || (W & 1) || (H & 1) || ((size_t)codes & 3)) return OCR_ERR_INVALID;
    long npix = (long)Nb * (W / 2) * (H / 2);
    int ppb = slab ? conv1_ppb() : 256;
#ifdef OCR_EXPERIMENTS
    if (!codes && !slab && !conv1_v1() && npix < 0x7fffffffL - 512 && (long)Nb * W * H < 0x7fffffffL)
        conv1_pool_bwd2_kernel<<<ceil_div(npix, ppb), 256, 0, (hipStream_t)stream>>>(x, w, bias, (const bf16_t*)dp, dw, db, Nb, W, H,
                                                                                     Cout, ppb);
    else
#endif
    {
        if (codes) conv1_pool_bwd_kernel<true><<<ceil_div(npix, ppb), 256, 0, (hipStream_t)stream>>>(x, w, bias, (const bf16_t*)dp, dw, db, Nb, W, H,
                                                                                                   Cout, ppb, (const uint32_t*)codes, slab);
        else conv1_pool_bwd_kernel<false><<<ceil_div(npix, ppb), 256, 0, (hipStream_t)stream>>>(x, w, bias, (const bf16_t*)dp, dw, db, Nb, W, H,
                                                                                               Cout, ppb, nullptr, slab);
    }
    OCR_CHECK_LAUNCH();
    return OCR_OK;
}
extern "C" int ocr_conv1_pool_bwd(const float* x, const float* w, const float* bias, const void* dp, float* dw, float* db,
                                  int Nb, int W, int H, int Cout, void* stream) {
    return conv1_pool_bwd_impl(x, w, bias, dp, dw, db, Nb, W, H, Cout, nullptr, nullptr, stream);
}
extern "C" int ocr_conv1_pool_bwd_codes(const float* x, const float* w, const float* bias, const void* dp, float* dw, float* db,
                                        int Nb, int W, int H, int Cout, const void* codes, void* stream) {
    if (!codes) return OCR_ERR_INVALID;
    return conv1_pool_bwd_impl(x, w, bias, dp, dw, db, Nb, W, H, Cout, codes, nullptr, stream);
}
extern "C" int ocr_conv1_pool_bwd_slab_rows(int Nb, int W, int H) {
    if (Nb <= 0 || W <= 0 || H <= 0 || (W & 1) || (H & 1)) return 0;
    return (int)ceil_div((long)Nb * (W / 2) * (H / 2), (long)conv1_ppb());
}
extern "C" int ocr_conv1_pool_bwd_slab(const float* x, const float* w, const float* bias, const void* dp, int Nb, int W, int H, int Cout,
                                       const void* codes, float* slab, void* stream) {
    if (!slab || ((size_t)slab & 15)) return OCR_ERR_INVALID;
    return conv1_pool_bwd_impl(x, w, bias, dp, nullptr, nullptr, Nb, W, H, Cout, codes, slab, stream);
}
extern "C" int ocr_maxpool_fwd(const void* x, void* y, int Nb, int W, int H, int C, int kw, int kh, void* stream) {
    if (!x || !y || (C & 7) || kw < 1 || kw > 2 || kh < 1 || kh > 2 || W % kw || H % kh) return OCR_ERR_INVALID;
    long total = (long)Nb * (W / kw) * (H / kh) * (C >> 3);
    const bf16_t* xi = (const bf16_t*)x; bf16_t* yo = (bf16_t*)y;
    hipStream_t st = (hipStream_t)stream;
    int gr = grid_for(total, 8192);
    if (kw == 2 && kh == 2) maxpool_fwd_kernel<2, 2><<<gr, 256, 0, st>>>(xi, yo, Nb, W, H, C);
    else if (kw == 1 && kh == 2) maxpool_fwd_kernel<1, 2><<<gr, 256, 0, st>>>(xi, yo, Nb, W, H, C);
    else if (kw == 2 && kh == 1) maxpool_fwd_kernel<2, 1><<<gr, 256, 0, st>>>(xi, yo, Nb, W, H, C);
    else return OCR_ERR_INVALID;
    OCR_CHECK_LAUNCH();
    return OCR_OK;
}
extern "C" int ocr_maxpool_bwd(const void* x, const void* dy, void* dx, int Nb, int W, int H, int C, int kw, int kh,
                               int relu_mask, void* stream) {
    if (!x || !dy || !dx || (C & 7) || kw < 1 || kw > 2 || kh < 1 || kh > 2 || W % kw || H % kh) return OCR_ERR_INVALID;
    long total = (long)Nb * (W / kw) * (H / kh) * (C >> 3);
    const bf16_t* xi = (const bf16_t*)x; const bf16_t* dyi = (const bf16_t*)dy; bf16_t* dxo = (bf16_t*)dx;
    hipStream_t st = (hipStream_t)stream;
    int gr = grid_for(total, 8192);
    if (kw == 2 && kh == 2) maxpool_bwd_kernel<2, 2><<<gr, 256, 0, st>>>(xi, dyi, dxo, Nb, W, H, C, relu_mask);
    else if (kw == 1 && kh == 2) maxpool_bwd_kernel<1, 2><<<gr, 256, 0, st>>>(xi, dyi, dxo, Nb, W, H, C, relu_mask);
    else if (kw == 2 && kh == 1) maxpool_bwd_kernel<2, 1><<<gr, 256, 0, st>>>(xi, dyi, dxo, Nb, W, H, C, relu_mask);
    else return OCR_ERR_INVALID;
    OCR_CHECK_LAUNCH();
    return OCR_OK;
}
extern "C" size_t ocr_bn_workspace_bytes(long M, int C) {
    if (M <= 0 || C <= 0) return 0;
    const long nblk = ceil_div(M, (long)bn_rows_per_block_host(M, 512));
    return (size_t)nblk * 2 * C * sizeof(float) + 2 * (size_t)C * sizeof(double);
}
static constexpr int bn_rows_per_thread() { return 4; }
static int bn_train_fwd_impl(const void* x, void* y, const float* gamma, const float* beta, float* save_mean,
                             float* save_rstd, long M, int C, float eps, int relu, void* workspace, const void* residual,
                             int partial_rows, void* pooled, void* stream_) {
    hipStream_t stream = (hipStream_t)stream_;
    if (!x || !y || !gamma || !beta || !save_mean || !save_rstd || !workspace || (C & 7) || C > 2048 || M <= 0)
        return OCR_ERR_INVALID;
    int rlanes = 256 / (C >> 3); if (rlanes < 1) return OCR_ERR_INVALID;
    if (partial_rows < 0 || (size_t)partial_rows * 2 * C * sizeof(float) > ocr_bn_workspace_bytes(M, C) - 2 * (size_t)C * sizeof(double)) return OCR_ERR_INVALID;
    if (pooled && ((M & 1) || residual)) return OCR_ERR_INVALID;
#ifdef OCR_EXPERIMENTS
    if (!partial_rows && !pooled) {
        int frpb = 0;
        const int fnb = bnf_blocks(M, C, &frpb);
        if (fnb > 0) {
            bn_fused_fwd_kernel<<<fnb, 256, 0, stream>>>((const bf16_t*)x, (bf16_t*)y, gamma, beta, save_mean, save_rstd, (float*)workspace, M, C,
                                                         eps, relu, frpb, (const bf16_t*)residual);
            OCR_CHECK_LAUNCH();
            return OCR_OK;
        }
    }
#endif
    const int rpb = bn_rows_per_block_host(M, 256);
    int nblk = (int)ceil_div(M, (long)rpb);
    if (partial_rows > 0) nblk = partial_rows;
    else {
        bn_stats_kernel<<<nblk, 256, 0, stream>>>((const bf16_t*)x, (float*)workspace, M, C, rpb);
        OCR_CHECK_LAUNCH();
    }
    bn_finalize_kernel<<<ceil_div(C, 16), 256, 0, stream>>>((const float*)workspace, nblk, save_mean, save_rstd, M, C, eps);
    OCR_CHECK_LAUNCH();
    const int arows = bn_rows_per_thread() * rlanes;
    if (pooled)
        bn_apply_pool_kernel<<<ceil_div(M / 2, (long)(arows / 2)), 256, 0, stream>>>((const bf16_t*)x, (bf16_t*)y, (bf16_t*)pooled, save_mean, save_rstd,
                                                                                       gamma, beta, M, C, relu, arows / 2);
    else
        bn_apply_kernel<<<ceil_div(M, (long)arows), 256, 0, stream>>>((const bf16_t*)x, (bf16_t*)y, save_mean, save_rstd, gamma,
                                                                        beta, M, C, relu, arows, (const bf16_t*)residual);
    OCR_CHECK_LAUNCH();
    return OCR_OK;
}
extern "C" int ocr_bn_train_fwd(const void* x, void* y, const float* gamma, const float* beta, float* save_mean,
                                float* save_rstd, long M, int C, float eps, int relu, void* workspace, const void* residual, void* stream_) {
    return bn_train_fwd_impl(x, y, gamma, beta, save_mean, save_rstd, M, C, eps, relu, workspace, residual, 0, nullptr, stream_);
}
extern "C" int ocr_bn_train_fwd2(const void* x, void* y, const float* gamma, const float* beta, float* save_mean, float* save_rstd, long M,
                                 int C, float eps, int relu, void* workspace, const void* residual, int partial_rows, void* pooled, void* stream_) {
    return bn_train_fwd_impl(x, y, gamma, beta, save_mean, save_rstd, M, C, eps, relu, workspace, residual, partial_rows, pooled, stream_);
}
static int bn_train_bwd_impl(const void* x, const void* y, const void* dy, void* dx, const float* gamma,
                             const float* save_mean, const float* save_rstd, float* dgamma, float* dbeta, long M,
                             int C, int relu, void* workspace, int pooled_dy, int partial_rows, void* stream_) {
    hipStream_t stream = (hipStream_t)stream_;
    if (!x || !y || !dy || !dx || !gamma || !save_mean || !save_rstd || !dgamma || !dbeta || !workspace || (C & 7) ||
        C > 2048 || M <= 0 || (pooled_dy && (M & 1)) || partial_rows < 0 || (partial_rows && pooled_dy))
        return OCR_ERR_INVALID;
    const int rpb = bn_rows_per_block_host(M, 512);
    const int nblk = (int)ceil_div(M, (long)rpb);
    float* part = (float*)workspace;
    double* sums = (double*)((char*)workspace + (size_t)nblk * 2 * C * sizeof(float));
#ifdef OCR_EXPERIMENTS
    {
        int frpb = 0;
        const int fnb = (pooled_dy || partial_rows) ? 0 : bnf_blocks(M, C, &frpb);
        if (fnb > 0) {
            bn_fused_bwd_kernel<<<fnb, 256, 0, stream>>>((const bf16_t*)x, (const bf16_t*)y, (const bf16_t*)dy, (bf16_t*)dx, save_mean, save_rstd,
                                                         gamma, part, sums, dgamma, dbeta, M, C, relu, frpb);
            OCR_CHECK_LAUNCH();
            return OCR_OK;
        }
    }
#endif
    if (partial_rows > nblk) return OCR_ERR_INVALID;
    if (partial_rows) relu = 0;
    else {
        bn_bwd_stats_kernel<<<nblk, 256, 0, stream>>>((const bf16_t*)x, (const bf16_t*)y, (const bf16_t*)dy, save_mean,
                                                      save_rstd, part, M, C, rpb, relu, pooled_dy);
        OCR_CHECK_LAUNCH();
    }
    bn_bwd_finalize_kernel<<<ceil_div(C, 16), 256, 0, stream>>>(part, partial_rows ? partial_rows : nblk, sums, dgamma, dbeta, C);
    OCR_CHECK_LAUNCH();
    const int arows = bn_rows_per_thread() * (256 / (C >> 3));
    bn_bwd_apply_kernel<<<ceil_div(M, (long)arows), 256, 0, stream>>>((const bf16_t*)x, (const bf16_t*)y, (const bf16_t*)dy,
                                                                        (bf16_t*)dx, save_mean, save_rstd, gamma,
                                                                        sums, dgamma, dbeta, M, C, relu, arows, pooled_dy);
    OCR_CHECK_LAUNCH();
    return OCR_OK;
}
extern "C" int ocr_bn_train_bwd(const void* x, const void* y, const void* dy, void* dx, const float* gamma,
                                const float* save_mean, const float* save_rstd, float* dgamma, float* dbeta, long M,
                                int C, int relu, void* workspace, void* stream_) {
    return bn_train_bwd_impl(x, y, dy, dx, gamma, save_mean, save_rstd, dgamma, dbeta, M, C, relu, workspace, 0, 0, stream_);
}
extern "C" int ocr_bn_train_bwd2(const void* x, const void* y, const void* dy, void* dx, const float* gamma, const float* save_mean,
                                 const float* save_rstd, float* dgamma, float* dbeta, long M, int C, int relu, void* workspace,
                                 int pooled_dy, int partial_rows, void* stream_) {
    return bn_train_bwd_impl(x, y, dy, dx, gamma, save_mean, save_rstd, dgamma, dbeta, M, C, relu, workspace, pooled_dy, partial_rows, stream_);
}
extern "C" int ocr_colsum_bf16(const void* a, float* out, long M, int C, long lda, void* stream) {
    if (!a || !out || (C & 7) || C > 2048 || M <= 0) return OCR_ERR_INVALID;
    int rpb = 128;
    colsum_kernel<<<ceil_div(M, rpb), 256, 0, (hipStream_t)stream>>>((const bf16_t*)a, out, M, C, lda, rpb);
    OCR_CHECK_LAUNCH();
    return OCR_OK;
}
extern "C" int ocr_pack_transpose(const float* in, void* out, int R, int Cc, long ldin, int lstm_units, void* stream) {
    if (!in || !out || R <= 0 || Cc <= 0) return OCR_ERR_INVALID;
    if (lstm_units > 0 && Cc != 4 * lstm_units) return OCR_ERR_INVALID;
    dim3 grid(ceil_div(Cc, 32), ceil_div(R, 32));
    pack_transpose_kernel<<<grid, 256, 0, (hipStream_t)stream>>>(in, (bf16_t*)out, R, Cc, ldin, lstm_units);
    OCR_CHECK_LAUNCH();
    return OCR_OK;
}
extern "C" int ocr_pack_conv_dgrad(const float* w, void* out, int Cin, int Cout, void* stream) {
    if (!w || !out) return OCR_ERR_INVALID;
    pack_conv_dgrad_kernel<<<grid_for(9L * Cin * Cout), 256, 0, (hipStream_t)stream>>>(w, (bf16_t*)out, Cin, Cout);
    OCR_CHECK_LAUNCH();
    return OCR_OK;
}
extern "C" int ocr_pack_jobs(const void* jobs, int njobs, int total_blocks, void* stream) {
    if (!jobs || njobs <= 0 || total_blocks <= 0) return OCR_ERR_INVALID;
    pack_jobs_kernel<<<total_blocks, 256, 0, (hipStream_t)stream>>>((const PackJob*)jobs, njobs);
    OCR_CHECK_LAUNCH();
    return OCR_OK;
}
extern "C" int ocr_cast_f32_bf16(const float* in, void* out, long n, void* stream) {
    if (!in || !out || n < 0) return OCR_ERR_INVALID;
    if (n == 0) return OCR_OK;
    cast_f32_bf16_kernel<<<grid_for((n + 3) / 4), 256, 0, (hipStream_t)stream>>>(in, (bf16_t*)out, n);
    OCR_CHECK_LAUNCH();
    return OCR_OK;
}
__global__ void u8_to_unit_f32_kernel(const uint8_t* __restrict__ in, float* __restrict__ out, long n4) {
    const long stride = (long)gridDim.x * blockDim.x;
    for (long i = (long)blockIdx.x * blockDim.x + threadIdx.x; i < n4; i += stride) {
        const uint32_t p = ((const uint32_t*)in)[i];
        f32x4 v = {__fdiv_rn((float)(p & 0xff), 255.0f), __fdiv_rn((float)((p >> 8) & 0xff), 255.0f),
                   __fdiv_rn((float)((p >> 16) & 0xff), 255.0f), __fdiv_rn((float)(p >> 24), 255.0f)};
        ((f32x4*)out)[i] = v;
    }
}
extern "C" int ocr_u8_to_unit_f32(const void* in, float* out, long n, void* stream) {
    if (!in || !out || n < 0 || (n & 3)) return OCR_ERR_INVALID;
    if (n == 0) return OCR_OK;
    u8_to_unit_f32_kernel<<<grid_for(n / 4), 256, 0, (hipStream_t)stream>>>((const uint8_t*)in, out, n / 4);
    OCR_CHECK_LAUNCH();
    return OCR_OK;
}
__global__ void bind_batch_kernel(const void* __restrict__ pix, int is_u8, float* __restrict__ x, long n4,
                                  const int* __restrict__ s0, int* __restrict__ d0, int n0, const int* __restrict__ s1, int* __restrict__ d1, int n1,
                                  const int* __restrict__ s2, int* __restrict__ d2, int n2) {
    const long stride = (long)gridDim.x * blockDim.x;
    for (long i = (long)blockIdx.x * blockDim.x + threadIdx.x; i < n4; i += stride) {
        if (is_u8) {
            const uint32_t p = ((const uint32_t*)pix)[i];
            ((f32x4*)x)[i] = (f32x4){__fdiv_rn((float)(p & 0xff), 255.0f), __fdiv_rn((float)((p >> 8) & 0xff), 255.0f),
                                     __fdiv_rn((float)((p >> 16) & 0xff), 255.0f), __fdiv_rn((float)(p >> 24), 255.0f)};
        } else {
            ((f32x4*)x)[i] = ((const f32x4*)pix)[i];
        }
    }
    if (blockIdx.x == gridDim.x - 1) {
        for (int i = threadIdx.x; i < n0; i += blockDim.x) d0[i] = s0[i];
        for (int i = threadIdx.x; i < n1; i += blockDim.x) d1[i] = s1[i];
        for (int i = threadIdx.x; i < n2; i += blockDim.x) d2[i] = s2[i];
    }
}
extern "C" int ocr_bind_batch(const void* pixels, int pixels_are_u8, float* x, long n_pixels, const int* seq_len, int* seq_len_dst, int n_seq,
                              const int* labels, int* labels_dst, int n_labels, const int* labels_len, int* labels_len_dst, int n_labels_len,
                              void* stream) {
    if (!pixels || !x || n_pixels <= 0 || (n_pixels & 3) || n_seq < 0 || n_labels < 0 || n_labels_len < 0) return OCR_ERR_INVALID;
    if ((n_seq && (!seq_len || !seq_len_dst)) || (n_labels && (!labels || !labels_dst)) || (n_labels_len && (!labels_len || !labels_len_dst)))
        return OCR_ERR_INVALID;
    if (((size_t)pixels & (pixels_are_u8 ? 3 : 15)) || ((size_t)x & 15)) return OCR_ERR_INVALID;
    bind_batch_kernel<<<grid_for(n_pixels / 4), 256, 0, (hipStream_t)stream>>>(pixels, pixels_are_u8, x, n_pixels / 4, seq_len, seq_len_dst, n_seq,
                                                                              labels, labels_dst, n_labels, labels_len, labels_len_dst, n_labels_len);
    OCR_CHECK_LAUNCH();
    return OCR_OK;
}
__global__ void step_report_kernel(const float* __restrict__ costs, int n, const double* __restrict__ scalars,
// ... 42 lines not shown
```

### lstm_ctc_ocr_amd/engine.py

```python
import math

import os
import time

import numpy as np
import torch

from . import dist as ocr_dist
from . import ops
from ._native import NativeError
from .layout import FlatLayout, execution_order, init_host_parameters
from ._native import call as nat_call

BF16, F32, I32 = torch.bfloat16, torch.float32, torch.int32
BN_EPS = 1e-3
ALIGN = 64


def _round_up(x, m):
    return (x + m - 1) // m * m


def _take_ring(sp, key):
    ready = getattr(sp, 'rings_ready', None)
# ... 34 lines not shown
        pass

    def bwd(self, sp):
        pass

    def y(self, sp):
        return sp.buf[self.key + '/y']

    def dy(self, sp):
        return sp.buf[self.key + '/dy']


class _InputOp(_Op):
    def __init__(self, eng):
        self.eng, self.name, self.prev, self.node = eng, 'data', None, None
        self.key = 'data'
        self.inputs, self.consumers = [], 0

    def y(self, sp):
        return sp.x

    def dy(self, sp):
        return None


class _ConvOp(_Op):
    def __init__(self, eng, node, prev):
        super(_ConvOp, self).__init__(eng, node, prev)
        a = node.attrs
        self.kh, self.kw, self.co, self.ci = a['k_h'], a['k_w'], a['c_o'], a['c_i']
        self.bn, self.relu, self.biased, self.padding = a['bn'], a['relu'], a['biased'], a['padding']
        if self.ci == 1:
            if (self.kh, self.kw, self.padding) != (3, 3, 'SAME') or self.co != 64 or self.bn or not self.biased:
                raise NotImplementedError('%s: the single-channel input conv is lowered for 3x3 SAME, 64 filters' % self.name)
            self.kind = 'c1'
        elif (self.kh, self.kw, self.padding) == (3, 3, 'SAME'):
            if self.ci % 32 or self.co % 8:
                raise NotImplementedError('%s: 3x3 conv needs C_in %% 32 == 0 and C_out %% 8 == 0' % self.name)
            self.kind = '3x3'
        elif (self.kh, self.kw) == (1, 1):
            if self.ci % 8 or self.co % 8:
                raise NotImplementedError('%s: 1x1 conv needs C_in %% 8 == 0 and C_out %% 8 == 0' % self.name)
            self.kind = '1x1'
        elif self.padding == 'VALID':
            self.kind = 'full'
        else:
            raise NotImplementedError('%s: %dx%d %s convolution is not lowered' % (self.name, self.kh, self.kw, self.padding))
        self.mask_in_consumer = self.relu and not self.bn
        dev = eng.device
        K = self.kh * self.kw * self.ci
        if self.kind != 'c1':
            self.wpack = torch.empty((self.co, K), dtype=BF16, device=dev)
            if self.kind == '3x3' and prev.dy_needed():
                self.wdgrad = torch.empty((self.ci, 9 * self.co), dtype=BF16, device=dev)

    def dy_needed(self):
        return True

    def out_shape(self, s):
        N, W, H = s[0], s[1], s[2]
        if self.kind == 'full':
            if self.kw != H:
                raise NotImplementedError('%s: VALID conv is lowered only when k_w equals the feature-axis size '
                                          '(got k_w=%d, H=%d)' % (self.name, self.kw, H))
            return (N, W - self.kh + 1, 1, self.co)
        return (N, W, H, self.co)

    fused_pool = None
    tail_into = None
    mask_from = None
    bn_pool = None
    pool_after = None

    def alloc(self, sp, s):
        o = self.out_shape(s)
        dev = self.eng.device
        sp.shape[self.key] = (s, o)
        if self.fused_pool is not None:
            if self.co == 64 and self.eng.defer_w9 and os.environ.get('OCR_CONV1_SLAB', '1') != '0':
                sp.buf[self.key + '/slab'] = torch.empty((ops.conv1_pool_bwd_slab_rows(s[0], s[1], s[2]), 640), dtype=F32, device=dev)
            if self.co == 64 and os.environ.get('OCR_CONV1_CODES', '1') != '0':
                sp.buf[self.key + '/codes'] = torch.empty((s[0] * (s[1] // 2) * (s[2] // 2), 8), dtype=torch.int32, device=dev)
            return
        sp.buf[self.key + '/y'] = torch.empty(o, dtype=BF16, device=dev)
        sp.buf[self.key + '/dy'] = torch.empty(o, dtype=BF16, device=dev)
        if self.bn:
            sp.buf[self.key + '/z'] = torch.empty(o, dtype=BF16, device=dev)
            sp.buf[self.key + '/dz'] = torch.empty(o, dtype=BF16, device=dev)
            sp.buf[self.key + '/mean'] = torch.empty(self.co, dtype=F32, device=dev)
            sp.buf[self.key + '/rstd'] = torch.empty(self.co, dtype=F32, device=dev)
            sp.buf[self.key + '/bnws'] = ops.bn_workspace(o[0] * o[1] * o[2], self.co, dev)
            rows = 0
            if self.kind == '3x3' and self.eng.fuse_bn_stats:
                rows = ops.conv3x3_stats_rows(s[0], s[1], s[2], self.ci, self.co, bias=self.biased)
                if rows * 2 * self.co * 4 > sp.buf[self.key + '/bnws'].numel() - 2 * self.co * 8:
                    rows = 0
            sp.bn_stat_rows = getattr(sp, 'bn_stat_rows', {})
            sp.bn_stat_rows[self.key] = rows
        if self.kind == 'full':
            N, W, H, C = s
            sp.buf[self.key + '/col'] = torch.empty((N * o[1], self.kh * H * C), dtype=BF16, device=dev)
        if self.pool_after is not None:
            p = self.pool_after
            sp.fused_pools = getattr(sp, 'fused_pools', set())
            if ops.conv3x3_pool_supported(s[0], s[1], s[2], self.ci, self.co, p.kw_t, p.kh_f):
                sp.fused_pools.add(p.key)
        if self.kind == '3x3' and hasattr(self, 'wdgrad') and self.eng.fuse_bn_stats and os.environ.get('OCR_FUSE_BN_BWD', '1') != '0':
            p = self.prev
            rows = 0
            if (isinstance(p, _ConvOp) and p.bn and p.relu and p.consumers == 1 and p.tail_into is None and p.mask_from is None
                    and p.bn_pool is None and p.kind != 'c1'):
                rows = ops.conv3x3_bnbwd_rows(s[0], s[1], s[2], self.co, self.ci)
                if rows * 2 * self.ci * 4 > sp.buf[p.key + '/bnws'].numel() - 2 * self.ci * 8:
                    rows = 0
            sp.bn_bwd_rows = getattr(sp, 'bn_bwd_rows', {})
            if isinstance(p, _ConvOp):
                assert p.bn_pool is None or not rows, (p.key, rows)
                sp.bn_bwd_rows[p.key] = rows
        if self.kind == '3x3':
            need = ops.conv3x3_wgrad_workspace_bytes(s[0], s[1], s[2], self.ci, self.co)
            have = sp.buf.get('wgrad_ws')
            if need and self.eng.defer_w9:
                pool = self.eng.w9_ws_pool
                have_ws = pool.get(self.key)
                if have_ws is None or have_ws.numel() < need:
                    wmax = max(int(os.environ.get('OCR_MAX_WIDTH', '320')), sp.W)
                    scale = max(1, wmax // sp.W + (1 if wmax % sp.W else 0))
                    big = need
                    if scale > 1:
                        big = max(need, ops.conv3x3_wgrad_workspace_bytes(s[0], s[1] * scale, s[2], self.ci, self.co))
                    have_ws = pool[self.key] = torch.empty(big, dtype=torch.uint8, device=dev)
                sp.buf[self.key + '/w9ws'] = have_ws[:need]
            elif need and (have is None or have.numel() < need):
                sp.buf['wgrad_ws'] = torch.empty(need, dtype=torch.uint8, device=dev)

    def shadow_params(self):
        return [self.name + '/weights'] if self.kind in ('1x1', 'full') else []

    def pack_jobs(self):
        if self.kind == 'c1':
            return []
        w = self.eng.param(self.name + '/weights')
        K = self.kh * self.kw * self.ci
        jobs = [dict(type=0, R=K, Cc=self.co, ldin=self.co, src=w, dst=self.wpack)]
        if hasattr(self, 'wdgrad'):
            jobs.append(dict(type=1, R=self.ci, Cc=self.co, src=w, dst=self.wdgrad, n=w.numel()))
        return jobs

    def fwd(self, sp):
        e = self.eng
        x = self.prev.y(sp)
        s, o = sp.shape[self.key]
        bias = e.param(self.name + '/biases') if self.biased else None
        if self.fused_pool is not None:
            zero, e._zero_pending = (e.grads if e._zero_pending else None), False
            codes = sp.buf.get(self.key + '/codes') if e.training else None
            ones, e._ones_pending = e._ones_pending, None
            ops.conv1_pool_fwd(x, e.param(self.name + '/weights'), bias, out=self.fused_pool.y(sp), zero=zero, codes=codes, ones=ones)
            sp.rings_ready = set(getattr(sp, 'lstm_sync_keys', ())) if ones is not None else set()
            sp.rings_armed = ones is not None
            return
        y = self.y(sp)
        if self.kind == 'c1':
            ops.conv1_fwd(x, e.param(self.name + '/weights'), bias, relu=self.relu, out=y)
            return
        tgt = sp.buf[self.key + '/z'] if self.bn else y
        relu_now = self.relu and not self.bn
        if self.kind == '3x3' and self.pool_after is not None and self.pool_after.key in sp.fused_pools:
            p = self.pool_after
            ops.conv3x3_relu_pool(x, self.wpack.view(self.co, 3, 3, self.ci), y, p.y(sp), bias, p.kw_t, p.kh_f)
        elif self.kind == '3x3' and self.bn and sp.bn_stat_rows[self.key]:
            ops.conv3x3_stats(x, self.wpack.view(self.co, 3, 3, self.ci), tgt, sp.buf[self.key + '/bnws'], bias=bias)
        elif self.kind == '3x3':
            ops.conv3x3(x, self.wpack.view(self.co, 3, 3, self.ci), out=tgt, bias=bias, relu=relu_now)
        elif self.kind == '1x1':
            Mx = s[0] * s[1] * s[2]
            ops.gemm_nt(x.view(Mx, self.ci), self.wpack, out=tgt.view(Mx, self.co), bias=bias, relu=relu_now)
        else:
            N, W, H, C = s
            Wo = o[1]
            ops.gemm_nt(x, self.wpack, out=tgt.view(N * Wo, self.co), M=N * Wo, N=self.co, K=self.kh * H * C,
                        ldp=H * C, ldq=self.kh * H * C, bias=bias, relu=relu_now, row_group=Wo, row_skip=self.kh - 1)
        if self.bn:
            M = o[0] * o[1] * o[2]
            res, relu = None, self.relu
            if self.tail_into is not None:
                add, other = self.tail_into
                y, res, relu = add.y(sp), other.y(sp).view(M, self.co), True
            pooled = self.bn_pool.y(sp).view(M // 2, self.co) if self.bn_pool is not None else None
            ops.bn_train_fwd(tgt.view(M, self.co), e.param('%s/%s/gamma' % (self.name, self.name)),
                             e.param('%s/%s/beta' % (self.name, self.name)), BN_EPS, relu,
                             sp.buf[self.key + '/bnws'], out=y.view(M, self.co),
                             save_mean=sp.buf[self.key + '/mean'], save_rstd=sp.buf[self.key + '/rstd'], residual=res,
                             partial_rows=sp.bn_stat_rows[self.key], pooled=pooled)

    def bwd(self, sp):
        e = self.eng
        if self.fused_pool is not None:
            slab = sp.buf.get(self.key + '/slab')
            if slab is not None:
                ops.conv1_pool_bwd_slab(self.prev.y(sp), e.param(self.name + '/weights'), e.param(self.name + '/biases'), self.fused_pool.dy(sp),
                                        slab, codes=sp.buf.get(self.key + '/codes'))
                S = slab.shape[0]
                for dst, off, n4 in ((e.grad(self.name + '/weights'), 0, 144), (e.grad(self.name + '/biases'), 576, 16)):
                    job = np.zeros(1, dtype=e.W9_JOB_DTYPE)
                    job['dw'], job['part'], job['n4'], job['slab4'] = dst.data_ptr(), slab.data_ptr() + 4 * off, n4, 160
                    job['S'], job['rows'], job['Cout'] = S, 8, 64
                    sp.w9_pending.append((job.tobytes(), (n4 + 31) // 32))
                return
            ops.conv1_pool_bwd(self.prev.y(sp), e.param(self.name + '/weights'), e.param(self.name + '/biases'),
                               self.fused_pool.dy(sp), e.grad(self.name + '/weights'), e.grad(self.name + '/biases'),
                               codes=sp.buf.get(self.key + '/codes'))
            return
        s, o = sp.shape[self.key]
        x = self.prev.y(sp)
        dy = self.dy(sp)
        M = o[0] * o[1] * o[2]
        dz = dy
        if self.bn:
            dz = sp.buf[self.key + '/dz']
            ymask, relu = self.y(sp), self.relu
            if self.mask_from is not None:
                dy, ymask, relu = self.mask_from.dy(sp), self.mask_from.y(sp), True
            dy2 = dy.view(M, self.co)
            if self.bn_pool is not None:
                dy2 = self.bn_pool.dy(sp).view(M // 2, self.co)
            ops.bn_train_bwd(sp.buf[self.key + '/z'].view(M, self.co), ymask.view(M, self.co), dy2,
                             e.param('%s/%s/gamma' % (self.name, self.name)), sp.buf[self.key + '/mean'],
                             sp.buf[self.key + '/rstd'], e.grad('%s/%s/gamma' % (self.name, self.name)),
                             e.grad('%s/%s/beta' % (self.name, self.name)), relu, sp.buf[self.key + '/bnws'],
                             out=dz.view(M, self.co), pooled_dy=self.bn_pool is not None,
                             partial_rows=getattr(sp, 'bn_bwd_rows', {}).get(self.key, 0))
        dw = e.grad(self.name + '/weights')
        db = e.grad(self.name + '/biases') if self.biased else None
        if self.kind == 'c1':
            ops.conv1_wgrad(x, dz, dw, db)
            return
        pmask = self.prev.y(sp) if self.prev.mask_in_consumer else None
        if self.kind == '3x3':
            own_ws = sp.buf.get(self.key + '/w9ws')
            if own_ws is not None:
                job, nblk = ops.conv3x3_wgrad_deferred(x, dz, dw, db, own_ws)
                if job is not None:
                    sp.w9_pending.append((job, nblk))
                    sp.w9_pending_bytes = getattr(sp, 'w9_pending_bytes', 0) + own_ws.numel()
                    if e.w9_flush_bytes and sp.w9_pending_bytes >= e.w9_flush_bytes:
                        e._flush_w9(sp)
            else:
                ops.conv3x3_wgrad(x, dz, dw, dbias=db, workspace=sp.buf.get('wgrad_ws'))
            pdy, finish, acc = e.grad_dst_acc(sp, self.prev, ops.conv3x3_accum_supported(o[0], o[1], o[2], self.co, self.ci))
            if pdy is not None:
                p = self.prev
                if getattr(sp, 'bn_bwd_rows', {}).get(p.key, 0) and not acc:
                    ops.conv3x3_dgrad_bnbwd(dz, self.wdgrad.view(self.ci, 3, 3, self.co), pdy, p.y(sp), sp.buf[p.key + '/z'],
                                            sp.buf[p.key + '/mean'], sp.buf[p.key + '/rstd'], sp.buf[p.key + '/bnws'])
                else:
                    ops.conv3x3(dz, self.wdgrad.view(self.ci, 3, 3, self.co), out=pdy, mask=pmask, accumulate=acc)
                finish()
            return
        pdy, finish = e.grad_dst(sp, self.prev)
        if self.kind == '1x1':
            ops.gemm_tn(x.view(M, self.ci), dz.view(M, self.co), dw.view(self.ci, self.co), colsum=db)
            if pdy is not None:
                wsh = e.shadow(self.name + '/weights').view(self.ci, self.co)
                ops.gemm_nt(dz.view(M, self.co), wsh, out=pdy.view(M, self.ci),
                            mask=None if pmask is None else pmask.view(M, self.ci))
                finish()
        else:
            N, W, H, C = s
            Wo = o[1]
            K = self.kh * H * C
            dz2, dw2 = dz.view(M, self.co), dw.view(K, self.co)
            e.tn_push(sp, ops.tn_job(x, H * C, dz2, self.co, dw2, self.co, M, K, self.co, row_group=Wo, row_skip=self.kh - 1, colsum=db),
                      (x, dz2, dw2, db),
                      lambda: ops.gemm_tn(x, dz2, dw2, Mk=M, I=K, J=self.co, lda=H * C, ldb=self.co,
                                          ldo=self.co, row_group=Wo, row_skip=self.kh - 1, colsum=db))
            if pdy is not None:
                if pmask is not None or self.kh != 2:
                    raise NotImplementedError('%s: data gradient of a full-height VALID conv is lowered for k_h = 2 '
                                              'behind a non-ReLU producer' % self.name)
                col = sp.buf[self.key + '/col']
                wsh = e.shadow(self.name + '/weights').view(K, self.co)
                ops.gemm_nt(dz.view(M, self.co), wsh, out=col, M=M, N=K, K=self.co)
                ops.conv5_col2im(col, pdy, N, W, H * C)
                finish()


class _FcOp(_ConvOp):

    def __init__(self, eng, node, prev):
        super(_FcOp, self).__init__(eng, node, prev)
        assert self.kind == '1x1'

    def out_shape(self, s):
        return tuple(s[:-1]) + (self.co,)

    def alloc(self, sp, s):
        o = self.out_shape(s)
        rows = int(np.prod(s[:-1]))
        sp.shape[self.key] = ((rows, 1, 1, s[-1]), (rows, 1, 1, self.co))
        sp.buf[self.key + '/y'] = torch.empty(o, dtype=BF16, device=self.eng.device)
        sp.buf[self.key + '/dy'] = torch.empty(o, dtype=BF16, device=self.eng.device)


class _PoolOp(_Op):
    def __init__(self, eng, node, prev):
        super(_PoolOp, self).__init__(eng, node, prev)
        a = node.attrs
        self.kw_t, self.kh_f = a['k_h'], a['k_w']
        if (a['s_h'], a['s_w']) != (a['k_h'], a['k_w']) or self.kw_t not in (1, 2) or self.kh_f not in (1, 2):
            raise NotImplementedError('%s: max-pool is lowered for window == stride in {1,2}' % self.name)

    def dy_needed(self):
        return True

    def out_shape(self, s):
        N, W, H, C = s
        if W % self.kw_t or H % self.kh_f:
            raise NotImplementedError('%s: pooled axes must divide evenly (W=%d, H=%d)' % (self.name, W, H))
        return (N, W // self.kw_t, H // self.kh_f, C)

    def alloc(self, sp, s):
        o = self.out_shape(s)
        sp.shape[self.key] = (s, o)
        sp.buf[self.key + '/y'] = torch.empty(o, dtype=BF16, device=self.eng.device)
        sp.buf[self.key + '/dy'] = torch.empty(o, dtype=BF16, device=self.eng.device)

    fused_into = None
    bn_fused_into = None

    def fwd(self, sp):
        if self.bn_fused_into is not None:
            return
        if self.fused_into is None and self.key not in getattr(sp, 'fused_pools', ()):
            ops.maxpool_fwd(self.prev.y(sp), self.kw_t, self.kh_f, out=self.y(sp))

    def bwd(self, sp):
        if self.fused_into is not None or self.bn_fused_into is not None:
            return
        pdy, finish = self.eng.grad_dst(sp, self.prev)
        if pdy is not None:
            ops.maxpool_bwd(self.prev.y(sp), self.dy(sp), self.kw_t, self.kh_f, self.prev.mask_in_consumer, out=pdy)
            finish()


class _ViewOp(_Op):

    def __init__(self, eng, node, prev):
        super(_ViewOp, self).__init__(eng, node, prev)
        self.mask_in_consumer = prev.mask_in_consumer

    def dy_needed(self):
        return True

    def out_shape(self, s):
        if self.node.op == 'reshape_squeeze':
            N, A, B, C = s
            return (N, A * B, C)
        return s

    def alloc(self, sp, s):
        sp.shape[self.key] = (s, self.out_shape(s))

    def y(self, sp):
        return self.prev.y(sp).view(sp.shape[self.key][1])

    def dy(self, sp):
        d = self.prev.dy(sp)
        return None if d is None else d.view(sp.shape[self.key][1])

    def grad_owner(self):
        return self.prev.grad_owner()


class _AddOp(_Op):

    def dy_needed(self):
        return True

    def out_shape(self, s):
        return s

    def alloc(self, sp, s):
        sp.shape[self.key] = (s, s)
        sp.buf[self.key + '/y'] = torch.empty(s, dtype=BF16, device=self.eng.device)
        sp.buf[self.key + '/dy'] = torch.empty(s, dtype=BF16, device=self.eng.device)

    relu = False

    fwd_by = None

    def fwd(self, sp):
        if self.fwd_by is None:
            ops.eltwise(3 if self.relu else 0, self.inputs[0].y(sp), self.inputs[1].y(sp), self.y(sp))

    def bwd(self, sp):
        for p in self.inputs:
            if getattr(p, 'mask_from', None) is self:
                continue
            self.eng.deliver(sp, p, self.dy(sp), mask=self.y(sp) if self.relu else None)


class _ReluOp(_Op):

    def dy_needed(self):
        return True

    def out_shape(self, s):
        return s

    fused_into = None

    def alloc(self, sp, s):
        sp.shape[self.key] = (s, s)
        if self.fused_into is None:
            sp.buf[self.key + '/y'] = torch.empty(s, dtype=BF16, device=self.eng.device)
            sp.buf[self.key + '/dy'] = torch.empty(s, dtype=BF16, device=self.eng.device)

    def y(self, sp):
        return self.fused_into.y(sp) if self.fused_into is not None else sp.buf[self.key + '/y']

    def dy(self, sp):
        return self.fused_into.dy(sp) if self.fused_into is not None else sp.buf[self.key + '/dy']

    def grad_owner(self):
# ... 1174 lines not shown
```

### lstm_ctc_ocr_amd/ops.py

```python
import ctypes

import torch

from . import _native as nat
from ._native import EPI_ACCUM, EPI_BIAS, EPI_MASK, EPI_OUT_F32, EPI_RELU, EPI_ROWSWAP, call, ptr

BF16 = torch.bfloat16
F32 = torch.float32


def _st():
    return nat.stream()


def _dev(t):
    if not t.is_cuda:
        raise nat.NativeError("hot-path operators take device tensors only (got a CPU tensor)")
    return t


def ctc_workspace_bytes(max_label_len, max_time, minibatch):
    sz = ctypes.c_size_t(0)
    call("ocr_ctc_workspace_size", max_label_len, max_time, minibatch, ctypes.byref(sz))
    return sz.value
# ... 30 lines not shown
    out = torch.empty((N, T), dtype=torch.int32, device=acts.device)
    lens = torch.empty(N, dtype=torch.int32, device=acts.device)
    call("ocr_ctc_greedy_decode", ptr(_dev(acts)), ptr(input_lengths), C, N, T, blank, pad_value, ptr(out), ptr(lens), _st())
    return out, lens


def ctc_beam_decode(acts, input_lengths, beam_width=100, merge_repeated=True, pad_value=0, workspace=None):
    T, N, C = acts.shape
    sz = ctypes.c_size_t(0)
    call("ocr_ctc_beam_workspace_size", C, N, T, beam_width, ctypes.byref(sz))
    if workspace is None or workspace.numel() < sz.value:
        workspace = torch.empty(sz.value, dtype=torch.uint8, device=acts.device)
    out = torch.empty((N, T), dtype=torch.int32, device=acts.device)
    lens = torch.empty(N, dtype=torch.int32, device=acts.device)
    nlp = torch.empty(N, dtype=F32, device=acts.device)
    call("ocr_ctc_beam_decode", ptr(_dev(acts)), ptr(input_lengths), C, N, T, beam_width, int(merge_repeated), pad_value,
         ptr(out), ptr(lens), ptr(nlp), ptr(workspace), workspace.numel(), _st())
    return out, lens, nlp


def gemm_nt(P, Q, out=None, *, M=None, N=None, K=None, ldp=None, ldq=None, ldo=None, bias=None, relu=False,
            out_f32=False, mask=None, accumulate=False, splits=1, row_group=0, row_skip=0, rowswap=None):
    M = P.shape[0] if M is None else M
    K = P.shape[1] if K is None else K
    N = Q.shape[0] if N is None else N
    ldp = P.stride(0) if ldp is None else ldp
    ldq = Q.stride(0) if ldq is None else ldq
    if out is None:
        out = torch.empty((M, N), dtype=F32 if out_f32 else BF16, device=P.device)
    ldo = out.stride(0) if ldo is None else ldo
    flags = 0
    if bias is not None: flags |= EPI_BIAS
    if relu: flags |= EPI_RELU
    if out.dtype == F32: flags |= EPI_OUT_F32
    if mask is not None: flags |= EPI_MASK
    if accumulate: flags |= EPI_ACCUM
    si = so = 0
    if rowswap is not None:
        flags |= EPI_ROWSWAP
        si, so = rowswap
    call("ocr_gemm_nt_bf16", ptr(_dev(P)), ldp, ptr(Q), ldq, ptr(out), ldo, M, N, K, ptr(bias), ptr(mask),
         mask.stride(0) if mask is not None else 0, flags, splits, row_group, row_skip, si, so, _st())
    return out


CONV_KERNEL_NAMES = ("gemm", "conv_halo", "conv_k2/A", "conv_k2/D", "conv_k3/A", "conv_k3/D", "conv_k3w/A", "conv_k3w/D", "conv_ws")


def conv3x3_kernel_choice(Nb, W, H, Cin, Cout, *, bias=True, relu=True, mask=False, accumulate=False, pool=(0, 0)):
    flags = (nat.EPI_BIAS if bias else 0) | (nat.EPI_RELU if relu else 0) | (nat.EPI_MASK if mask else 0) | (nat.EPI_ACCUM if accumulate else 0)
    rc = nat.lib().ocr_conv3x3_kernel_choice(int(Nb), int(W), int(H), int(Cin), int(Cout), flags, int(pool[0]), int(pool[1]))
    if rc < 0:
        raise nat.NativeError("ocr_conv3x3_kernel_choice failed: status %d (%s)" % (-rc, nat.status_string(-rc)))
    return CONV_KERNEL_NAMES[rc]


def conv3x3_accum_supported(Nb, W, H, Cin, Cout):
    return bool(nat.lib().ocr_conv3x3_accum_supported(Nb, W, H, Cin, Cout))


def conv3x3(x, wpack, out=None, *, bias=None, relu=False, mask=None, accumulate=False):
    Nb, W, H, Cin = x.shape
    Cout = wpack.shape[0]
    if out is None:
        assert not accumulate
        out = torch.empty((Nb, W, H, Cout), dtype=BF16, device=x.device)
    flags = ((EPI_BIAS if bias is not None else 0) | (EPI_RELU if relu else 0) | (EPI_MASK if mask is not None else 0) |
             (EPI_ACCUM if accumulate else 0))
    call("ocr_conv3x3_bf16", ptr(_dev(x)), ptr(wpack), ptr(out), Nb, W, H, Cin, Cout, ptr(bias), ptr(mask), flags, _st())
    return out


def conv3x3_pool_supported(Nb, W, H, Cin, Cout, kw, kh):
    return bool(nat.lib().ocr_conv3x3_pool_supported(Nb, W, H, Cin, Cout, kw, kh))


def conv3x3_relu_pool(x, wpack, out, pooled, bias, kw, kh):
    Nb, W, H, Cin = x.shape
    call("ocr_conv3x3_relu_pool_bf16", ptr(_dev(x)), ptr(wpack), ptr(out), ptr(pooled), Nb, W, H, Cin, wpack.shape[0], ptr(bias),
         kw, kh, _st())
    return out, pooled


def gemm_tn(A, B, out, *, Mk=None, I=None, J=None, lda=None, ldb=None, ldo=None, row_group=0, row_skip=0,
            a_row_off=0, scale=1.0, splits=0, colsum=None):
    Mk = B.shape[0] if Mk is None else Mk
    I = A.shape[1] if I is None else I
    J = B.shape[1] if J is None else J
    lda = A.stride(0) if lda is None else lda
    ldb = B.stride(0) if ldb is None else ldb
    ldo = out.stride(0) if ldo is None else ldo
    call("ocr_gemm_tn_bf16", ptr(_dev(A)), lda, ptr(B), ldb, ptr(out), ldo, Mk, I, J, row_group, row_skip, a_row_off,
         float(scale), splits, ptr(colsum), _st())
    return out


def gemm_tn_split_workspace(Mk, I, J):
    n = nat.lib().ocr_gemm_tn_split_workspace_floats(int(Mk), int(I), int(J))
    if n < 0:
        raise nat.NativeError("ocr_gemm_tn_split_workspace_floats: invalid shape (%d, %d, %d)" % (Mk, I, J))
    return int(n)


def gemm_tn_split(A, B, out, ws, *, colsum=None, scale=1.0):
    Mk, I, J = B.shape[0], A.shape[1], B.shape[1]
    call("ocr_gemm_tn_split_bf16", ptr(_dev(A)), A.stride(0), ptr(B), B.stride(0), ptr(out), out.stride(0), Mk, I, J, float(scale),
         ptr(colsum), ptr(ws), ws.numel(), _st())
    return out


def gemm_tn_batched(A, lda, strideA, B, ldb, strideB, out, ldo, strideOut, Mk, I, J, nbatch, colsum=None, strideColsum=0,
                    scale=1.0, splits=0):
    call("ocr_gemm_tn_batched_bf16", ptr(_dev(A)), lda, strideA, ptr(B), ldb, strideB, ptr(out), ldo, strideOut, Mk, I, J, nbatch,
         float(scale), splits, ptr(colsum), strideColsum, _st())
    return out


class TnJob(ctypes.Structure):
    _fields_ = [("A", ctypes.c_void_p), ("lda", ctypes.c_long), ("strideA", ctypes.c_long),
                ("B", ctypes.c_void_p), ("ldb", ctypes.c_long), ("strideB", ctypes.c_long),
                ("out", ctypes.c_void_p), ("ldo", ctypes.c_long), ("strideOut", ctypes.c_long),
                ("colsum", ctypes.c_void_p), ("strideColsum", ctypes.c_long),
                ("Mk", ctypes.c_int), ("I", ctypes.c_int), ("J", ctypes.c_int), ("nbatch", ctypes.c_int),
                ("row_group", ctypes.c_int), ("row_skip", ctypes.c_int), ("scale", ctypes.c_float), ("reserved", ctypes.c_int)]


def tn_job(A, lda, B, ldb, out, ldo, Mk, I, J, *, nbatch=1, strideA=0, strideB=0, strideOut=0, colsum=None, strideColsum=0, row_group=0,
           row_skip=0, scale=1.0):
    return TnJob(ptr(_dev(A)), lda, strideA, ptr(_dev(B)), ldb, strideB, ptr(out), ldo, strideOut, ptr(colsum), strideColsum,
                 Mk, I, J, nbatch, row_group, row_skip, float(scale), 0)


def gemm_tn_jobs_supported(jobs):
    arr = (TnJob * len(jobs))(*jobs)
    return bool(nat.lib().ocr_gemm_tn_jobs_supported(ctypes.cast(arr, ctypes.c_void_p), len(jobs)))


def gemm_tn_jobs(jobs):
    arr = (TnJob * len(jobs))(*jobs)
    call("ocr_gemm_tn_jobs_bf16", ctypes.cast(arr, ctypes.c_void_p), len(jobs), _st())


def lstm_xh(x2d, hout, seq_len, xh, Nb, T, D, U, ndir=2):
    call("ocr_lstm_xh", ptr(_dev(x2d)), ptr(hout), ptr(seq_len), ptr(xh), Nb, T, D, U, ndir, _st())
    return xh


def conv3x3_wgrad_workspace_bytes(Nb, W, H, Cin, Cout):
    sz = ctypes.c_size_t(0)
    call("ocr_conv3x3_wgrad_workspace_size", Nb, W, H, Cin, Cout, ctypes.byref(sz))
    return sz.value


WGRAD_KERNEL_NAMES = ("wgrad9", "wgrad9p<4>", "wgrad9p<8>", "wgrad9p<4>/zero-row", "wgrad9p<8>/zero-row", "gemm_tn2/nine-tap",
                      "gemm_tn2/paired-tap", "gemm_tn<1,4,4>", "gemm_tn<1,2,2>")


def conv3x3_wgrad_kernel_choice(Nb, W, H, Cin, Cout, *, workspace=True, splits=0):
    rc = nat.lib().ocr_conv3x3_wgrad_kernel_choice(int(Nb), int(W), int(H), int(Cin), int(Cout), int(bool(workspace)), int(splits))
    if rc < 0:
        raise nat.NativeError("ocr_conv3x3_wgrad_kernel_choice failed: status %d (%s)" % (-rc, nat.status_string(-rc)))
    return WGRAD_KERNEL_NAMES[rc & 255], rc >> 8


def conv3x3_wgrad(x, dy, dw, splits=0, dbias=None, workspace=None):
    Nb, W, H, Cin = x.shape
# ... 7 lines not shown


def conv3x3_wgrad_deferred(x, dy, dw, dbias, workspace):
    Nb, W, H, Cin = x.shape
    Cout = dy.shape[-1]
    job = (ctypes.c_ubyte * 64)()
    nblk, deferred = ctypes.c_int(0), ctypes.c_int(0)
    call("ocr_conv3x3_wgrad_defer_bf16", ptr(_dev(x)), ptr(dy), ptr(dw), ptr(dbias), Nb, W, H, Cin, Cout, ptr(workspace),
         workspace.numel(), ctypes.cast(job, ctypes.c_void_p), ctypes.byref(nblk), ctypes.byref(deferred), _st())
    return (bytes(job), nblk.value) if deferred.value else (None, 0)


def wgrad9_reduce_jobs(table, njobs, total_blocks):
    call("ocr_wgrad9_reduce_jobs", ptr(_dev(table)), njobs, total_blocks, _st())


def conv1_fwd(x, w, bias, relu=True, out=None):
    Nb, W, H = x.shape
    Cout = w.shape[-1]
    if out is None:
        out = torch.empty((Nb, W, H, Cout), dtype=BF16, device=x.device)
    call("ocr_conv1_fwd", ptr(_dev(x)), ptr(w), ptr(bias), ptr(out), Nb, W, H, Cout, int(relu), _st())
    return out


def conv1_wgrad(x, dz, dw, db):
    Nb, W, H = x.shape
    call("ocr_conv1_wgrad", ptr(_dev(x)), ptr(dz), ptr(dw), ptr(db), Nb, W, H, dz.shape[-1], _st())


def eltwise(op, a, b, out):
    call("ocr_eltwise_bf16", op, ptr(_dev(a)), ptr(b), ptr(out), a.numel(), _st())
    return out


def conv1_pool_fwd(x, w, bias, out=None, zero=None, codes=None, ones=None):
    Nb, W, H = x.shape
    Cout = w.shape[-1]
    if out is None:
        out = torch.empty((Nb, W // 2, H // 2, Cout), dtype=BF16, device=x.device)
    if zero is not None or codes is not None or ones is not None:
        call("ocr_conv1_pool_fwd_train", ptr(_dev(x)), ptr(w), ptr(bias), ptr(out), Nb, W, H, Cout, ptr(codes),
             ptr(_dev(zero)) if zero is not None else None, 0 if zero is None else zero.numel(),
             ptr(_dev(ones)) if ones is not None else None, 0 if ones is None else ones.numel(), _st())
    else:
        call("ocr_conv1_pool_fwd", ptr(_dev(x)), ptr(w), ptr(bias), ptr(out), Nb, W, H, Cout, _st())
    return out


def conv1_pool_bwd(x, w, bias, dp, dw, db, codes=None):
    Nb, W, H = x.shape
    if codes is not None:
        call("ocr_conv1_pool_bwd_codes", ptr(_dev(x)), ptr(w), ptr(bias), ptr(dp), ptr(dw), ptr(db), Nb, W, H, w.shape[-1], ptr(codes), _st())
    else:
        call("ocr_conv1_pool_bwd", ptr(_dev(x)), ptr(w), ptr(bias), ptr(dp), ptr(dw), ptr(db), Nb, W, H, w.shape[-1], _st())


def conv1_pool_bwd_slab_rows(Nb, W, H):
    return int(nat.lib().ocr_conv1_pool_bwd_slab_rows(int(Nb), int(W), int(H)))


def conv1_pool_bwd_slab(x, w, bias, dp, slab, codes=None):
    Nb, W, H = x.shape
    assert slab.dtype == torch.float32 and tuple(slab.shape) == (conv1_pool_bwd_slab_rows(Nb, W, H), 640)
    call("ocr_conv1_pool_bwd_slab", ptr(_dev(x)), ptr(w), ptr(bias), ptr(dp), Nb, W, H, w.shape[-1], ptr(codes), ptr(slab), _st())


def maxpool_fwd(x, kw, kh, out=None):
    Nb, W, H, C = x.shape
    if out is None:
        out = torch.empty((Nb, W // kw, H // kh, C), dtype=BF16, device=x.device)
    call("ocr_maxpool_fwd", ptr(_dev(x)), ptr(out), Nb, W, H, C, kw, kh, _st())
    return out


def maxpool_bwd(x, dy, kw, kh, relu_mask, out=None):
    Nb, W, H, C = x.shape
    if out is None:
        out = torch.empty_like(x)
    call("ocr_maxpool_bwd", ptr(_dev(x)), ptr(dy), ptr(out), Nb, W, H, C, kw, kh, int(relu_mask), _st())
    return out


def bn_workspace(M, C, device):
    return torch.empty(int(nat.lib().ocr_bn_workspace_bytes(int(M), int(C))), dtype=torch.uint8, device=device)


def bn_train_fwd(x2d, gamma, beta, eps, relu, workspace, out=None, save_mean=None, save_rstd=None, residual=None, partial_rows=0,
                 pooled=None):
    M, C = x2d.shape
    if out is None: out = torch.empty_like(x2d)
    if save_mean is None: save_mean = torch.empty(C, dtype=F32, device=x2d.device)
    if save_rstd is None: save_rstd = torch.empty(C, dtype=F32, device=x2d.device)
    if partial_rows or pooled is not None:
        call("ocr_bn_train_fwd2", ptr(_dev(x2d)), ptr(out), ptr(gamma), ptr(beta), ptr(save_mean), ptr(save_rstd), M, C,
             float(eps), int(relu), ptr(workspace), ptr(residual), int(partial_rows), ptr(pooled), _st())
    else:
        call("ocr_bn_train_fwd", ptr(_dev(x2d)), ptr(out), ptr(gamma), ptr(beta), ptr(save_mean), ptr(save_rstd), M, C,
             float(eps), int(relu), ptr(workspace), ptr(residual), _st())
    return out, save_mean, save_rstd


def bn_train_bwd(x2d, y2d, dy2d, gamma, save_mean, save_rstd, dgamma, dbeta, relu, workspace, out=None, pooled_dy=False, partial_rows=0):
    M, C = x2d.shape
    if out is None: out = torch.empty_like(x2d)
    if pooled_dy or partial_rows:
        assert tuple(dy2d.shape) == ((M // 2, C) if pooled_dy else (M, C))
        call("ocr_bn_train_bwd2", ptr(_dev(x2d)), ptr(y2d), ptr(dy2d), ptr(out), ptr(gamma), ptr(save_mean), ptr(save_rstd),
             ptr(dgamma), ptr(dbeta), M, C, int(relu), ptr(workspace), int(bool(pooled_dy)), int(partial_rows), _st())
    else:
        call("ocr_bn_train_bwd", ptr(_dev(x2d)), ptr(y2d), ptr(dy2d), ptr(out), ptr(gamma), ptr(save_mean), ptr(save_rstd),
             ptr(dgamma), ptr(dbeta), M, C, int(relu), ptr(workspace), _st())
    return out


def conv3x3_stats_rows(Nb, W, H, Cin, Cout, *, bias=True, relu=False):
    flags = (EPI_BIAS if bias else 0) | (EPI_RELU if relu else 0)
    return int(nat.lib().ocr_conv3x3_stats_rows(int(Nb), int(W), int(H), int(Cin), int(Cout), flags))


def conv3x3_bnbwd_rows(Nb, W, H, Cin, Cout):
    return int(nat.lib().ocr_conv3x3_bnbwd_rows(int(Nb), int(W), int(H), int(Cin), int(Cout)))


def conv3x3_dgrad_bnbwd(dy, wdgrad, out, mask_y, z, mean, rstd, partials):
    Nb, W, H, Cin = dy.shape
    Cout = wdgrad.shape[0]
    call("ocr_conv3x3_dgrad_bnbwd_bf16", ptr(_dev(dy)), ptr(wdgrad), ptr(out), Nb, W, H, Cin, Cout, ptr(mask_y), ptr(z), ptr(mean), ptr(rstd),
         ptr(partials), _st())
    return out


def conv3x3_stats(x, wpack, out, partials, *, bias=None, relu=False):
    Nb, W, H, Cin = x.shape
    Cout = wpack.shape[0]
    flags = (EPI_BIAS if bias is not None else 0) | (EPI_RELU if relu else 0)
    call("ocr_conv3x3_bf16_stats", ptr(_dev(x)), ptr(wpack), ptr(out), Nb, W, H, Cin, Cout, ptr(bias), flags, ptr(partials), _st())
    return out


def bn_infer_fwd(x2d, gamma, beta, mean, var, eps, relu, out):
    M, C = x2d.shape
    call("ocr_bn_infer_fwd", ptr(_dev(x2d)), ptr(out), ptr(gamma), ptr(beta), ptr(mean), ptr(var), M, C, float(eps), int(relu), _st())
    return out


def bn_infer_bwd(x2d, y2d, dy2d, gamma, mean, var, dgamma, dbeta, eps, relu, out):
    M, C = x2d.shape
    call("ocr_bn_infer_bwd", ptr(_dev(x2d)), ptr(y2d), ptr(dy2d), ptr(out), ptr(gamma), ptr(mean), ptr(var), ptr(dgamma), ptr(dbeta),
         M, C, float(eps), int(relu), _st())
    return out


def dropout(src, dst, seed, step_counter, keep_prob):
    call("ocr_dropout_bf16", ptr(_dev(src)), ptr(dst), src.numel(), int(seed) & 0xffffffff, ptr(step_counter), float(keep_prob), _st())
    return dst


def avgpool(src, dst, Nb, W, H, C, kw, kh, backward=False):
    call("ocr_avgpool_bf16", ptr(_dev(src)), ptr(dst), Nb, W, H, C, kw, kh, int(backward), _st())
    return dst


def subsample(src, dst, Nb, W, H, C, Wo, Ho, sw, sh, ow, oh, backward=False):
    call("ocr_subsample_bf16", ptr(_dev(src)), ptr(dst), Nb, W, H, C, Wo, Ho, sw, sh, ow, oh, int(backward), _st())
    return dst


def softmax(src_f32, dst_f32):
    C = src_f32.shape[-1]
    call("ocr_softmax_f32", ptr(_dev(src_f32)), ptr(dst_f32), src_f32.numel() // C, C, _st())
    return dst_f32


def colsum(a2d, out, M=None, C=None, lda=None):
    M = a2d.shape[0] if M is None else M
    C = a2d.shape[1] if C is None else C
    lda = a2d.stride(0) if lda is None else lda
    call("ocr_colsum_bf16", ptr(_dev(a2d)), ptr(out), M, C, lda, _st())
    return out


def pack_transpose(w2d, out, lstm_units=0, R=None, Cc=None, ldin=None):
    R = w2d.shape[0] if R is None else R
    Cc = w2d.shape[1] if Cc is None else Cc
    ldin = w2d.stride(0) if ldin is None else ldin
    call("ocr_pack_transpose", ptr(_dev(w2d)), ptr(out), R, Cc, ldin, lstm_units, _st())
    return out
# ... 153 lines not shown
```

Measured before the change: 56860 images/sec.

## Store 4-bit max-pool argmax codes instead of full pre-pool activations

For conv and batch-norm layers followed by a fused max-pool, the forward kernels now write compact per-element argmax and positive-sign codes (4 bits per channel) in place of the full-resolution bf16 activation. Max-pool backward and BN backward then read these codes to route gradients and apply the ReLU mask. This is meant to remove the large activation write in forward and its re-read in backward. The cost is extra integer code generation in the kernel epilogues and new kernel variants across conv, BN and pool paths.

```diff
diff --git a/include/ocr_hip.h b/include/ocr_hip.h
--- a/include/ocr_hip.h
+++ b/include/ocr_hip.h
@@ -49,6 +49,9 @@
 int ocr_conv_halo_clock_debug(void* dbg);
 int ocr_conv_ws_debug(void* dbg);
 int ocr_conv3x3_pool_supported(int Nb, int W, int H, int Cin, int Cout, int kw, int kh);
+int ocr_conv3x3_pool_codes_supported(int Nb, int W, int H, int Cin, int Cout, int kw, int kh);
+int ocr_conv3x3_relu_pool_codes_bf16(const void* x, const void* wpack, void* y, void* pooled, void* codes, int Nb, int W, int H, int Cin,
+                                     int Cout, const float* bias, int kw, int kh, void* stream);
 int ocr_conv3x3_relu_pool_bf16(const void* x, const void* wpack, void* y, void* pooled, int Nb, int W, int H, int Cin, int Cout,
                                const float* bias, int kw, int kh, void* stream);
 int ocr_gemm_tn_bf16(const void* A, long lda, const void* B, long ldb, float* out, long ldo, int Mk, int I, int J,
@@ -100,6 +103,8 @@
 int ocr_maxpool_fwd(const void* x, void* y, int Nb, int W, int H, int C, int kw, int kh, void* stream);
 int ocr_maxpool_bwd(const void* x, const void* dy, void* dx, int Nb, int W, int H, int C, int kw, int kh,
                     int relu_mask, void* stream);
+int ocr_maxpool_bwd_codes(const void* codes, const void* dy, void* dx, int Nb, int W, int H, int C, int kw, int kh,
+                          int relu_mask, void* stream);
 size_t ocr_bn_workspace_bytes(long M, int C);
 int ocr_bn_train_fwd(const void* x, void* y, const float* gamma, const float* beta, float* save_mean,
                      float* save_rstd, long M, int C, float eps, int relu, void* workspace, const void* residual, void* stream);
@@ -111,6 +116,10 @@
 int ocr_bn_train_bwd2(const void* x, const void* y, const void* dy, void* dx, const float* gamma, const float* save_mean,
                       const float* save_rstd, float* dgamma, float* dbeta, long M, int C, int relu, void* workspace, int pooled_dy,
                       int partial_rows, void* stream);
+int ocr_bn_train_fwd_codes(const void* x, const float* gamma, const float* beta, float* save_mean, float* save_rstd, long M, int C,
+                           float eps, int relu, void* workspace, int partial_rows, void* pooled, void* codes, void* stream);
+int ocr_bn_train_bwd_codes(const void* x, const void* codes, const void* dy, void* dx, const float* gamma, const float* save_mean,
+                           const float* save_rstd, float* dgamma, float* dbeta, long M, int C, int relu, void* workspace, void* stream);
 int ocr_conv3x3_bnbwd_rows(int Nb, int W, int H, int Cin, int Cout);
 int ocr_conv3x3_dgrad_bnbwd_bf16(const void* dy, const void* wdgrad, void* dx, int Nb, int W, int H, int Cin, int Cout, const void* mask_y,
                                  const void* z, const float* mean, const float* rstd, float* partials, void* stream);
diff --git a/lstm_ctc_ocr_amd/_native.py b/lstm_ctc_ocr_amd/_native.py
--- a/lstm_ctc_ocr_amd/_native.py
+++ b/lstm_ctc_ocr_amd/_native.py
@@ -38,6 +38,8 @@
     "ocr_conv3x3_kernel_choice": ([_I, _I, _I, _I, _I, _I, _I, _I], _I),
     "ocr_conv3x3_pool_supported": ([_I, _I, _I, _I, _I, _I, _I], _I),
     "ocr_conv3x3_relu_pool_bf16": ([_P, _P, _P, _P, _I, _I, _I, _I, _I, _P, _I, _I, _P], _I),
+    "ocr_conv3x3_pool_codes_supported": ([_I, _I, _I, _I, _I, _I, _I], _I),
+    "ocr_conv3x3_relu_pool_codes_bf16": ([_P, _P, _P, _P, _P, _I, _I, _I, _I, _I, _P, _I, _I, _P], _I),
     "ocr_gemm_tn_bf16": ([_P, _L, _P, _L, _P, _L, _I, _I, _I, _I, _I, _L, _F, _I, _P, _P], _I),
     "ocr_gemm_tn_split_workspace_floats": ([_I, _I, _I], _L),
     "ocr_gemm_tn_split_bf16": ([_P, _L, _P, _L, _P, _L, _I, _I, _I, _F, _P, _P, _L, _P], _I),
@@ -64,6 +66,9 @@
     "ocr_bn_train_bwd": ([_P, _P, _P, _P, _P, _P, _P, _P, _P, _L, _I, _I, _P, _P], _I),
     "ocr_bn_train_fwd2": ([_P, _P, _P, _P, _P, _P, _L, _I, _F, _I, _P, _P, _I, _P, _P], _I),
     "ocr_bn_train_bwd2": ([_P, _P, _P, _P, _P, _P, _P, _P, _P, _L, _I, _I, _P, _I, _I, _P], _I),
+    "ocr_maxpool_bwd_codes": ([_P, _P, _P, _I, _I, _I, _I, _I, _I, _I, _P], _I),
+    "ocr_bn_train_fwd_codes": ([_P, _P, _P, _P, _P, _L, _I, _F, _I, _P, _I, _P, _P, _P], _I),
+    "ocr_bn_train_bwd_codes": ([_P, _P, _P, _P, _P, _P, _P, _P, _P, _L, _I, _I, _P, _P], _I),
     "ocr_conv3x3_bnbwd_rows": ([_I, _I, _I, _I, _I], _I),
     "ocr_conv3x3_dgrad_bnbwd_bf16": ([_P, _P, _P, _I, _I, _I, _I, _I, _P, _P, _P, _P, _P, _P], _I),
     "ocr_conv3x3_stats_rows": ([_I, _I, _I, _I, _I, _I], _I),
diff --git a/lstm_ctc_ocr_amd/csrc/common.h b/lstm_ctc_ocr_amd/csrc/common.h
--- a/lstm_ctc_ocr_amd/csrc/common.h
+++ b/lstm_ctc_ocr_amd/csrc/common.h
@@ -39,6 +39,25 @@
 }
 __device__ __forceinline__ float bf_lo(uint32_t p) { return __uint_as_float(p << 16); }
 __device__ __forceinline__ float bf_hi(uint32_t p) { return __uint_as_float(p & 0xffff0000u); }
+
+template <int CNT>
+__device__ __forceinline__ uint32_t pool_code_word(const u32x4 (&rows)[CNT]) {
+    uint32_t word = 0;
+#pragma unroll
+    for (int c = 0; c < 8; ++c) {
+        float v[CNT];
+#pragma unroll
+        for (int e = 0; e < CNT; ++e) {
+            const uint32_t pr = c < 2 ? rows[e].x : c < 4 ? rows[e].y : c < 6 ? rows[e].z : rows[e].w;
+            v[e] = (c & 1) ? bf_hi(pr) : bf_lo(pr);
+        }
+        int best = 0; float bv = v[0];
+#pragma unroll
+        for (int e = 1; e < CNT; ++e) if (v[e] > bv) { bv = v[e]; best = e; }
+        word |= (uint32_t)(best | ((bv > 0.f) ? 4 : 0)) << (4 * c);
+    }
+    return word;
+}
 
 __device__ __forceinline__ float wave_sum(float v) {
 #pragma unroll
diff --git a/lstm_ctc_ocr_amd/csrc/conv_k3.hip b/lstm_ctc_ocr_amd/csrc/conv_k3.hip
--- a/lstm_ctc_ocr_amd/csrc/conv_k3.hip
+++ b/lstm_ctc_ocr_amd/csrc/conv_k3.hip
@@ -11,6 +11,7 @@
     bf16_t* pool; int pool_kind;
     int prio;
     const bf16_t* bnz; const float* bn_mean; const float* bn_rstd;
+    uint32_t* codes;
 };
 
 #ifdef OCR_EXPERIMENTS
@@ -45,7 +46,8 @@
           int NST , int H ,
           bool SINGLE = false ,
           bool GENW = false ,
-          bool BNB = false >
+          bool BNB = false ,
+          bool CODES = false >
 __device__ __forceinline__ void k3_body(const K3Args& g) {
     constexpr int NW = 8, FN = 4, BM = 256;
     constexpr int WN = BN / 64, WMW = 4 / WN;
@@ -325,7 +327,7 @@
                     if (!(bf_lo(q.w) > 0.f)) v.w &= 0xffff0000u;
                     if (!(bf_hi(q.w) > 0.f)) v.w &= 0x0000ffffu;
                 }
-                *(u32x4*)(g.out + ((long)m0 + lp) * g.N + n0 + u * 8) = v;
+                if (!CODES || g.out != nullptr) *(u32x4*)(g.out + ((long)m0 + lp) * g.N + n0 + u * 8) = v;
                 if (!BNB && g.pool_kind == 3) {
                     const float f[8] = {bf_lo(v.x), bf_hi(v.x), bf_lo(v.y), bf_hi(v.y), bf_lo(v.z), bf_hi(v.z), bf_lo(v.w), bf_hi(v.w)};
 #pragma unroll
@@ -362,12 +364,18 @@
                     else { cl = 2 * (q / (H >> 1)); lp0 = cl * H + 2 * (q % (H >> 1)); }
                     const unsigned char* r0 = smem + lp0 * ROWB;
                     const int u0 = (u ^ ((cl & SWM) << 1)) << 4;
-                    u32x4 m = k3_max8(*(const u32x4*)(r0 + u0), *(const u32x4*)(r0 + ROWB + u0));
+                    u32x4 win[4] = {*(const u32x4*)(r0 + u0), *(const u32x4*)(r0 + ROWB + u0)};
+                    u32x4 m = k3_max8(win[0], win[1]);
                     if (kind == 2) {
                         const int u1 = (u ^ (((cl + 1) & SWM) << 1)) << 4;
-                        m = k3_max8(m, k3_max8(*(const u32x4*)(r0 + H * ROWB + u1), *(const u32x4*)(r0 + (H + 1) * ROWB + u1)));
+                        win[2] = *(const u32x4*)(r0 + H * ROWB + u1); win[3] = *(const u32x4*)(r0 + (H + 1) * ROWB + u1);
+                        m = k3_max8(m, k3_max8(win[2], win[3]));
                     }
                     *(u32x4*)(g.pool + (pbase + q) * g.N + n0 + u * 8) = m;
+                    if (CODES) {
+                        const u32x4 pair[2] = {win[0], win[1]};
+                        g.codes[(pbase + q) * (g.N >> 3) + (n0 >> 3) + u] = kind == 2 ? pool_code_word(win) : pool_code_word(pair);
+                    }
                 }
             }
             return;
@@ -418,6 +426,9 @@
 __global__ __launch_bounds__(512) __attribute__((amdgpu_waves_per_eu(2, 2))) void conv_k3w_kernel(K3Args g) { k3_body<FM, BN, NST, H, false, true>(g); }
 template <int FM, int BN, int NST, int H, bool GENW>
 __global__ __launch_bounds__(512) __attribute__((amdgpu_waves_per_eu(2, 2))) void conv_k3b_kernel(K3Args g) { k3_body<FM, BN, NST, H, false, GENW, true>(g); }
+
+template <int FM, int BN, int NST, int H, bool SINGLE>
+__global__ __launch_bounds__(512) __attribute__((amdgpu_waves_per_eu(2, 2))) void conv_k3c_kernel(K3Args g) { k3_body<FM, BN, NST, H, SINGLE, false, false, true>(g); }
 
 template <int FM, int BN, int NST, int H, bool GENW>
 static int run_k3b(const K3Args& g, hipStream_t stream) {
@@ -439,6 +450,16 @@
     static_assert(lds <= 163840, "LDS");
     static_assert(256 * BN * 2 + 2 * (512 / (BN / 8)) * BN * 4 <= lds, "staged image + the statistics scratch behind it");
     const int mt = g.M / 256, nt = (g.N + BN - 1) / BN;
+    if (g.codes) {
+        if constexpr (GENW) return OCR_ERR_INVALID;
+        else {
+            if ((g.pool_kind != 1 && g.pool_kind != 2) || (g.N & 63)) return OCR_ERR_INVALID;
+            if (ocr_allow_lds<conv_k3c_kernel<FM, BN, NST, H, SINGLE>>(lds) != hipSuccess) return OCR_ERR_EXEC;
+            conv_k3c_kernel<FM, BN, NST, H, SINGLE><<<mt * nt, 512, lds, stream>>>(g);
+            OCR_CHECK_LAUNCH();
+            return OCR_OK;
+        }
+    }
     if constexpr (GENW) {
         if (ocr_allow_lds<conv_k3w_kernel<FM, BN, NST, H>>(lds) != hipSuccess) return OCR_ERR_EXEC;
         conv_k3w_kernel<FM, BN, NST, H><<<mt * nt, 512, lds, stream>>>(g);
@@ -452,7 +473,7 @@
 
 int launch_k3(const ConvPlan& p, const ConvOperands& o, hipStream_t stream) {
     const K3Args g = {(const bf16_t*)o.x, (const bf16_t*)o.wpack, p.M, p.Cout, p.Cin, p.W, p.H, (bf16_t*)o.y, o.bias, (const bf16_t*)o.mask,
-                      p.flags, (bf16_t*)o.pool, p.epi_kind, p.prio, (const bf16_t*)o.bnz, o.bn_mean, o.bn_rstd};
+                      p.flags, (bf16_t*)o.pool, p.epi_kind, p.prio, (const bf16_t*)o.bnz, o.bn_mean, o.bn_rstd, (uint32_t*)o.codes};
     const int H = p.H;
     const bool A = p.tile == 'A';
     if (p.epi_kind == CONV_EPI_BNBWD) {
diff --git a/lstm_ctc_ocr_amd/csrc/conv_plan.h b/lstm_ctc_ocr_amd/csrc/conv_plan.h
--- a/lstm_ctc_ocr_amd/csrc/conv_plan.h
+++ b/lstm_ctc_ocr_amd/csrc/conv_plan.h
@@ -41,6 +41,7 @@
     const float* bias; const void* mask;
     void* pool;
     const void* bnz; const float* bn_mean; const float* bn_rstd;
+    void* codes;
 };
 int launch_halo(const ConvPlan& p, const ConvOperands& o, hipStream_t stream);
 int launch_k2(const ConvPlan& p, const ConvOperands& o, hipStream_t stream);
diff --git a/lstm_ctc_ocr_amd/csrc/conv_ws.hip b/lstm_ctc_ocr_amd/csrc/conv_ws.hip
--- a/lstm_ctc_ocr_amd/csrc/conv_ws.hip
+++ b/lstm_ctc_ocr_amd/csrc/conv_ws.hip
@@ -9,6 +9,7 @@
     bf16_t* out; const float* bias; const bf16_t* mask; int flags;
     bf16_t* pool; int pool_kind;
     int ntiles, slots, per_slot, xcd_map;
+    uint32_t* codes;
 };
 
 typedef __attribute__((address_space(3))) void* ws_lptr_t;
@@ -33,6 +34,31 @@
 __device__ __forceinline__ u32x4 ws_max8(u32x4 a, u32x4 b) {
     u32x4 r = {ws_max2(a.x, b.x), ws_max2(a.y, b.y), ws_max2(a.z, b.z), ws_max2(a.w, b.w)};
     return r;
+}
+
+typedef unsigned short ws_u16x2 __attribute__((ext_vector_type(2)));
+template <int CNT>
+__device__ __forceinline__ uint32_t ws_code2(const uint32_t (&p)[CNT]) {
+    const ws_u16x2 one = {1, 1};
+    ws_u16x2 v[CNT];
+#pragma unroll
+    for (int e = 0; e < CNT; ++e) v[e] = __builtin_bit_cast(ws_u16x2, p[e]);
+    ws_u16x2 m = v[0];
+#pragma unroll
+    for (int e = 1; e < CNT; ++e) m = __builtin_elementwise_max(m, v[e]);
+    ws_u16x2 t = __builtin_elementwise_min((ws_u16x2)(m - v[CNT - 2]), one);
+#pragma unroll
+    for (int e = CNT - 3; e >= 0; --e) t = __builtin_elementwise_min((ws_u16x2)(m - v[e]), one) * (ws_u16x2)(t + one);
+    const ws_u16x2 code = t + (ws_u16x2)(__builtin_elementwise_min(m, one) << (ws_u16x2){2, 2});
+    return __builtin_bit_cast(uint32_t, code);
+}
+template <int CNT>
+__device__ __forceinline__ uint32_t ws_code_word(const u32x4 (&p)[CNT]) {
+    uint32_t x[CNT], y[CNT], z[CNT], w[CNT];
+#pragma unroll
+    for (int e = 0; e < CNT; ++e) { x[e] = p[e].x; y[e] = p[e].y; z[e] = p[e].z; w[e] = p[e].w; }
+    const uint32_t c0 = ws_code2(x), c1 = ws_code2(y), c2 = ws_code2(z), c3 = ws_code2(w);
+    return ((c0 | (c0 >> 12)) & 0xffu) | (((c1 | (c1 >> 12)) & 0xffu) << 8) | (((c2 | (c2 >> 12)) & 0xffu) << 16) | ((c3 | (c3 >> 12)) << 24);
 }
 
 template <int H, int NC, int KSPLIT>
@@ -62,7 +88,8 @@
     static_assert(((H + 1) * PS) * 128 < 65536, "ds_read immediates");
 };
 
-template <int H, int NC, int KSPLIT, bool MASK >
+template <int H, int NC, int KSPLIT, bool MASK ,
+          bool CODES = false >
 __global__ __launch_bounds__(256) __attribute__((amdgpu_waves_per_eu(1, 1))) void conv_ws_kernel(WsArgs g) {
     using G = WsCfg<H, NC, KSPLIT>;
     constexpr int CF = G::CF, HF = G::HF, PS = G::PS, PI = G::PI, HWE = G::HWE, NPE = G::NPE;
@@ -290,29 +317,31 @@
             }
             asm volatile("s_waitcnt lgkmcnt(0)" ::: "memory");
             u32x4 val[NIT], mkv[MASK ? NIT : 1];
-#pragma unroll
-            for (int it = 0; it < NIT; ++it) {
-                const int idx = it * 64 + lane, row = idx >> 3, u = idx & 7;
-                val[it] = *(const u32x4*)(S + row * 128 + ((u ^ (((row / HWE) & 3) << 1)) << 4));
-                if (has_mask) mkv[it] = *(const u32x4*)(smem + G::MOFF + wave * G::STW + idx * 16);
-            }
-#pragma unroll
-            for (int it = 0; it < NIT; ++it) {
-                const int idx = it * 64 + lane, row = idx >> 3, u = idx & 7;
-                u32x4 v = val[it];
-                if (has_mask) {
-                    const u32x4 q = mkv[it];
-                    if (!(bf_lo(q.x) > 0.f)) v.x &= 0xffff0000u;
-                    if (!(bf_hi(q.x) > 0.f)) v.x &= 0x0000ffffu;
-                    if (!(bf_lo(q.y) > 0.f)) v.y &= 0xffff0000u;
-                    if (!(bf_hi(q.y) > 0.f)) v.y &= 0x0000ffffu;
-                    if (!(bf_lo(q.z) > 0.f)) v.z &= 0xffff0000u;
-                    if (!(bf_hi(q.z) > 0.f)) v.z &= 0x0000ffffu;
-                    if (!(bf_lo(q.w) > 0.f)) v.w &= 0xffff0000u;
-                    if (!(bf_hi(q.w) > 0.f)) v.w &= 0x0000ffffu;
-                }
-                const long m = (long)(col0 + row / HWE) * H + h_lo + row % HWE;
-                *(u32x4*)(g.out + m * N + n0 + u * 8) = v;
+            if (!CODES || g.out != nullptr) {
+#pragma unroll
+                for (int it = 0; it < NIT; ++it) {
+                    const int idx = it * 64 + lane, row = idx >> 3, u = idx & 7;
+                    val[it] = *(const u32x4*)(S + row * 128 + ((u ^ (((row / HWE) & 3) << 1)) << 4));
+                    if (has_mask) mkv[it] = *(const u32x4*)(smem + G::MOFF + wave * G::STW + idx * 16);
+                }
+#pragma unroll
+                for (int it = 0; it < NIT; ++it) {
+                    const int idx = it * 64 + lane, row = idx >> 3, u = idx & 7;
+                    u32x4 v = val[it];
+                    if (has_mask) {
+                        const u32x4 q = mkv[it];
+                        if (!(bf_lo(q.x) > 0.f)) v.x &= 0xffff0000u;
+                        if (!(bf_hi(q.x) > 0.f)) v.x &= 0x0000ffffu;
+                        if (!(bf_lo(q.y) > 0.f)) v.y &= 0xffff0000u;
+                        if (!(bf_hi(q.y) > 0.f)) v.y &= 0x0000ffffu;
+                        if (!(bf_lo(q.z) > 0.f)) v.z &= 0xffff0000u;
+                        if (!(bf_hi(q.z) > 0.f)) v.z &= 0x0000ffffu;
+                        if (!(bf_lo(q.w) > 0.f)) v.w &= 0xffff0000u;
+                        if (!(bf_hi(q.w) > 0.f)) v.w &= 0x0000ffffu;
+                    }
+                    const long m = (long)(col0 + row / HWE) * H + h_lo + row % HWE;
+                    *(u32x4*)(g.out + m * N + n0 + u * 8) = v;
+                }
             }
             if (g.pool_kind == 1) {
                 constexpr int NQ = NC * (HWE / 2), PIT = NQ * 8 / 64;
@@ -329,6 +358,7 @@
                     const int idx = it * 64 + lane, q = idx >> 3, u = idx & 7, col = q / (HWE / 2), ph = q % (HWE / 2);
                     const long pm = (long)(col0 + col) * (H / 2) + (h_lo >> 1) + ph;
                     *(u32x4*)(g.pool + pm * N + n0 + u * 8) = ws_max8(p0[it], p1[it]);
+                    if (CODES) { const u32x4 win[2] = {p0[it], p1[it]}; g.codes[pm * (N >> 3) + (n0 >> 3) + u] = ws_code_word(win); }
                 }
             } else if (g.pool_kind == 2) {
                 constexpr int NQ = (NC / 2) * (HWE / 2), PIT = NQ * 8 / 64;
@@ -347,6 +377,10 @@
                     const int idx = it * 64 + lane, q = idx >> 3, u = idx & 7, pc = q / (HWE / 2), ph = q % (HWE / 2);
                     const long pm = (long)((col0 >> 1) + pc) * (H / 2) + (h_lo >> 1) + ph;
                     *(u32x4*)(g.pool + pm * N + n0 + u * 8) = ws_max8(ws_max8(p0[it], p1[it]), ws_max8(p2[it], p3[it]));
+                    if (CODES) {
+                        const u32x4 win[4] = {p0[it], p1[it], p2[it], p3[it]};
+                        g.codes[pm * (N >> 3) + (n0 >> 3) + u] = ws_code_word(win);
+                    }
                 }
             }
         };
@@ -361,22 +395,23 @@
     if (clk && blockIdx.x == 0 && tid == 0) ocr_clk_exit(clk);
 }
 
-template <int H, int NC, int KSPLIT, bool MASK>
+template <int H, int NC, int KSPLIT, bool MASK, bool CODES = false>
 static int launch_ws_(const WsArgs& g, int grid, hipStream_t stream) {
     using G = WsCfg<H, NC, KSPLIT>;
     constexpr int lds = MASK ? G::LDS_MASK : G::LDS_PLAIN;
-    if (ocr_allow_lds<conv_ws_kernel<H, NC, KSPLIT, MASK>>(lds) != hipSuccess) return OCR_ERR_EXEC;
-    conv_ws_kernel<H, NC, KSPLIT, MASK><<<grid, 256, lds, stream>>>(g);
+    if (ocr_allow_lds<conv_ws_kernel<H, NC, KSPLIT, MASK, CODES>>(lds) != hipSuccess) return OCR_ERR_EXEC;
+    conv_ws_kernel<H, NC, KSPLIT, MASK, CODES><<<grid, 256, lds, stream>>>(g);
     OCR_CHECK_LAUNCH();
     return OCR_OK;
 }
 template <int H, int NC, int KSPLIT>
 static int launch_ws(const WsArgs& g, int grid, hipStream_t stream) {
+    if (g.codes) return (g.flags & WS_MASK) || !g.pool_kind ? OCR_ERR_INVALID : launch_ws_<H, NC, KSPLIT, false, true>(g, grid, stream);
     return (g.flags & WS_MASK) ? launch_ws_<H, NC, KSPLIT, true>(g, grid, stream) : launch_ws_<H, NC, KSPLIT, false>(g, grid, stream);
 }
 int launch_ws(const ConvPlan& p, const ConvOperands& o, hipStream_t stream) {
     const WsArgs g = {(const bf16_t*)o.x, (const bf16_t*)o.wpack, p.M, p.Cout, p.Cin, p.W, p.H, (bf16_t*)o.y, o.bias, (const bf16_t*)o.mask,
-                      p.flags, (bf16_t*)o.pool, p.epi_kind, p.Cout / 64, p.slots, p.per_slot, p.xcd_map};
+                      p.flags, (bf16_t*)o.pool, p.epi_kind, p.Cout / 64, p.slots, p.per_slot, p.xcd_map, (uint32_t*)o.codes};
     if (p.H == 16 && p.ws_ksplit == 1) return launch_ws<16, 16, 1>(g, p.grid, stream);
     if (p.H == 16) return launch_ws<16, 8, 2>(g, p.grid, stream);
     return launch_ws<8, 16, 2>(g, p.grid, stream);
diff --git a/lstm_ctc_ocr_amd/csrc/gemm.hip b/lstm_ctc_ocr_amd/csrc/gemm.hip
--- a/lstm_ctc_ocr_amd/csrc/gemm.hip
+++ b/lstm_ctc_ocr_amd/csrc/gemm.hip
@@ -496,3 +496,15 @@
     const ConvPlan p = conv3x3_plan(Nb * W * H, W, H, Cin, Cout, EPI_BIAS | EPI_RELU, conv3x3_pool_kind(kw, kh));
     return conv3x3_launch(p, {x, wpack, y, bias, nullptr, pooled}, (hipStream_t)stream);
 }
+static bool conv3x3_plan_has_codes(const ConvPlan& p) { return p.family == CONV_WS || (p.family == CONV_K3 && !p.genw); }
+extern "C" int ocr_conv3x3_pool_codes_supported(int Nb, int W, int H, int Cin, int Cout, int kw, int kh) {
+    const int kind = conv3x3_pool_kind(kw, kh);
+    return kind && conv3x3_plan_has_codes(conv3x3_plan(conv3x3_pixels(Nb, W, H, Cin, Cout), W, H, Cin, Cout, EPI_BIAS | EPI_RELU, kind));
+}
+extern "C" int ocr_conv3x3_relu_pool_codes_bf16(const void* x, const void* wpack, void* y, void* pooled, void* codes, int Nb, int W, int H,
+                                                int Cin, int Cout, const float* bias, int kw, int kh, void* stream) {
+    if (!x || !wpack || !pooled || !codes || ((size_t)codes & 3) || !bias || !ocr_conv3x3_pool_codes_supported(Nb, W, H, Cin, Cout, kw, kh))
+        return OCR_ERR_INVALID;
+    const ConvPlan p = conv3x3_plan(Nb * W * H, W, H, Cin, Cout, EPI_BIAS | EPI_RELU, conv3x3_pool_kind(kw, kh));
+    return conv3x3_launch(p, {x, wpack, y, bias, nullptr, pooled, nullptr, nullptr, nullptr, codes}, (hipStream_t)stream);
+}
diff --git a/lstm_ctc_ocr_amd/csrc/nn_ops.hip b/lstm_ctc_ocr_amd/csrc/nn_ops.hip
--- a/lstm_ctc_ocr_amd/csrc/nn_ops.hip
+++ b/lstm_ctc_ocr_amd/csrc/nn_ops.hip
@@ -534,6 +534,42 @@
     }
 }
 
+template <int KW, int KH>
+__global__ __launch_bounds__(256) void maxpool_bwd_codes_kernel(const uint32_t* __restrict__ codes, const bf16_t* __restrict__ dy,
+                                                                bf16_t* __restrict__ dx, int Nb, int W, int H, int C,
+                                                                int relu_mask) {
+    constexpr int kw = KW, kh = KH;
+    const int Wo = W / kw, Ho = H / kh, groups = C >> 3;
+    const long total = (long)Nb * Wo * Ho * groups;
+    for (long idx = (long)blockIdx.x * 256 + threadIdx.x; idx < total; idx += (long)gridDim.x * 256) {
+        int gq = (int)(idx % groups);
+        long op = idx / groups;
+        int ho = (int)(op % Ho);
+        long q = op / Ho;
+        int wo = (int)(q % Wo);
+        long n = q / Wo;
+        long boff = (((n * W + (long)wo * kw) * H) + (long)ho * kh) * C + gq * 8;
+        const uint32_t word = codes[idx];
+        float g[8];
+        unpack8(*(const u32x4*)(dy + op * C + gq * 8), g);
+        if (relu_mask) {
+#pragma unroll
+            for (int c = 0; c < 8; ++c) if (!((word >> (4 * c)) & 4u)) g[c] = 0.f;
+        }
+#pragma unroll
+        for (int a = 0; a < kw; ++a)
+#pragma unroll
+            for (int b = 0; b < kh; ++b) {
+                const int cnt = a * kh + b;
+                float o[8];
+#pragma unroll
+                for (int c = 0; c < 8; ++c) o[c] = (((word >> (4 * c)) & 3u) == (uint32_t)cnt) ? g[c] : 0.f;
+                u32x4 pk = {pack_bf2(o[0], o[1]), pack_bf2(o[2], o[3]), pack_bf2(o[4], o[5]), pack_bf2(o[6], o[7])};
+                *(u32x4*)(dx + boff + ((long)a * H + b) * C) = pk;
+            }
+    }
+}
+
 template <typename AccT, bool STORE = false>
 __device__ __forceinline__ void block_channel_reduce(const float (&v)[8], float* red, AccT* dst, int C, int groups,
                                                      int rl, int gq, int rlanes) {
@@ -650,7 +686,7 @@
 __global__ __launch_bounds__(256) void bn_apply_pool_kernel(const bf16_t* __restrict__ x, bf16_t* __restrict__ y, bf16_t* __restrict__ pooled,
                                                             const float* __restrict__ mean, const float* __restrict__ rstd,
                                                             const float* __restrict__ gamma, const float* __restrict__ beta,
-                                                            long M, int C, int relu, int pairs_per_block) {
+                                                            long M, int C, int relu, int pairs_per_block, uint32_t* __restrict__ codes) {
     const int groups = C >> 3;
     const int rl = threadIdx.x / groups, gq = threadIdx.x % groups, rlanes = 256 / groups;
     if (rl >= rlanes) return;
@@ -674,9 +710,10 @@
                 if (relu) o[c] = fmaxf(o[c], 0.f);
             }
             pk[e] = (u32x4){pack_bf2(o[0], o[1]), pack_bf2(o[2], o[3]), pack_bf2(o[4], o[5]), pack_bf2(o[6], o[7])};
-            *(u32x4*)(y + (2 * q + e) * C + gq * 8) = pk[e];
+            if (codes == nullptr) *(u32x4*)(y + (2 * q + e) * C + gq * 8) = pk[e];
         }
         *(u32x4*)(pooled + q * C + gq * 8) = max8(pk[0], pk[1]);
+        if (codes != nullptr) codes[q * groups + gq] = pool_code_word(pk);
     }
 }
 __device__ __forceinline__ void bn_pool_route(const bf16_t* __restrict__ y, const bf16_t* __restrict__ dp, long r, int C, int gq,
@@ -691,10 +728,23 @@
         if (!win) g[c] = 0.f;
     }
 }
+__device__ __forceinline__ void bn_pool_route_codes(const uint32_t* __restrict__ codes, const bf16_t* __restrict__ dp, long r, int C, int gq,
+                                                    int relu, float (&g)[8]) {
+    const uint32_t word = codes[(r >> 1) * (C >> 3) + gq];
+    unpack8(*(const u32x4*)(dp + (r >> 1) * C + gq * 8), g);
+    const uint32_t odd = (uint32_t)(r & 1);
+#pragma unroll
+    for (int c = 0; c < 8; ++c) {
+        const uint32_t code = word >> (4 * c);
+        if ((code & 1u) != odd || (relu && !(code & 4u))) g[c] = 0.f;
+    }
+}
+template <bool CODES>
 __global__ __launch_bounds__(256) void bn_bwd_stats_kernel(const bf16_t* __restrict__ x, const bf16_t* __restrict__ y,
                                                            const bf16_t* __restrict__ dy, const float* __restrict__ mean,
                                                            const float* __restrict__ rstd, float* __restrict__ part,
-                                                           long M, int C, int rows_per_block, int relu, int pooled) {
+                                                           long M, int C, int rows_per_block, int relu, int pooled,
+                                                           const uint32_t* __restrict__ codes) {
     const int groups = C >> 3;
     const int rl = threadIdx.x / groups, gq = threadIdx.x % groups, rlanes = 256 / groups;
     const long r0 = (long)blockIdx.x * rows_per_block, r1 = min(M, r0 + rows_per_block);
@@ -706,12 +756,15 @@
         for (long r = r0 + rl; r < r1; r += rlanes) {
             float xv[8], yv[8], g[8];
             unpack8(*(const u32x4*)(x + r * C + gq * 8), xv);
-            if (relu || pooled) unpack8(*(const u32x4*)(y + r * C + gq * 8), yv);
-            if (pooled) bn_pool_route(y, dy, r, C, gq, yv, g);
-            else unpack8(*(const u32x4*)(dy + r * C + gq * 8), g);
-            if (relu) {
-#pragma unroll
-                for (int c = 0; c < 8; ++c) if (!(yv[c] > 0.f)) g[c] = 0.f;
+            if constexpr (CODES) bn_pool_route_codes(codes, dy, r, C, gq, relu, g);
+            else {
+                if (relu || pooled) unpack8(*(const u32x4*)(y + r * C + gq * 8), yv);
+                if (pooled) bn_pool_route(y, dy, r, C, gq, yv, g);
+                else unpack8(*(const u32x4*)(dy + r * C + gq * 8), g);
+                if (relu) {
+#pragma unroll
+                    for (int c = 0; c < 8; ++c) if (!(yv[c] > 0.f)) g[c] = 0.f;
+                }
             }
 #pragma unroll
             for (int c = 0; c < 8; ++c) { s[c] += g[c]; sx[c] = fmaf(g[c], (xv[c] - mu[c]) * rs[c], sx[c]); }
@@ -731,12 +784,14 @@
         dgamma[c] += (float)sx;
     }
 }
+template <bool CODES>
 __global__ __launch_bounds__(256) void bn_bwd_apply_kernel(const bf16_t* __restrict__ x, const bf16_t* __restrict__ y,
                                                            const bf16_t* __restrict__ dy, bf16_t* __restrict__ dx,
                                                            const float* __restrict__ mean, const float* __restrict__ rstd,
                                                            const float* __restrict__ gamma, const double* __restrict__ sums,
                                                            float* __restrict__ dgamma, float* __restrict__ dbeta,
-                                                           long M, int C, int relu, int rows_per_block, int pooled) {
+                                                           long M, int C, int relu, int rows_per_block, int pooled,
+                                                           const uint32_t* __restrict__ codes) {
     const int groups = C >> 3;
     const int rl = threadIdx.x / groups, gq = threadIdx.x % groups, rlanes = 256 / groups;
     if (rl >= rlanes) return;
@@ -753,12 +808,15 @@
     for (long r = r0 + rl; r < r1; r += rlanes) {
         float xv[8], yv[8], g[8], o[8];
         unpack8(*(const u32x4*)(x + r * C + gq * 8), xv);
-        if (relu || pooled) unpack8(*(const u32x4*)(y + r * C + gq * 8), yv);
-        if (pooled) bn_pool_route(y, dy, r, C, gq, yv, g);
-        else unpack8(*(const u32x4*)(dy + r * C + gq * 8), g);
-        if (relu) {
-#pragma unroll
-            for (int c = 0; c < 8; ++c) if (!(yv[c] > 0.f)) g[c] = 0.f;
+        if constexpr (CODES) bn_pool_route_codes(codes, dy, r, C, gq, relu, g);
+        else {
+            if (relu || pooled) unpack8(*(const u32x4*)(y + r * C + gq * 8), yv);
+            if (pooled) bn_pool_route(y, dy, r, C, gq, yv, g);
+            else unpack8(*(const u32x4*)(dy + r * C + gq * 8), g);
+            if (relu) {
+#pragma unroll
+                for (int c = 0; c < 8; ++c) if (!(yv[c] > 0.f)) g[c] = 0.f;
+            }
         }
 #pragma unroll
         for (int c = 0; c < 8; ++c) {
@@ -1365,6 +1423,19 @@
     OCR_CHECK_LAUNCH();
     return OCR_OK;
 }
+extern "C" int ocr_maxpool_bwd_codes(const void* codes, const void* dy, void* dx, int Nb, int W, int H, int C, int kw, int kh,
+                                     int relu_mask, void* stream) {
+    if (!codes || ((size_t)codes & 3) || !dy || !dx || (C & 7) || Nb <= 0 || W <= 0 || H <= 0 || kh != 2 || kw < 1 || kw > 2 || W % kw || H % kh)
+        return OCR_ERR_INVALID;
+    long total = (long)Nb * (W / kw) * (H / kh) * (C >> 3);
+    const uint32_t* ci = (const uint32_t*)codes; const bf16_t* dyi = (const bf16_t*)dy; bf16_t* dxo = (bf16_t*)dx;
+    hipStream_t st = (hipStream_t)stream;
+    int gr = grid_for(total, 8192);
+    if (kw == 2) maxpool_bwd_codes_kernel<2, 2><<<gr, 256, 0, st>>>(ci, dyi, dxo, Nb, W, H, C, relu_mask);
+    else maxpool_bwd_codes_kernel<1, 2><<<gr, 256, 0, st>>>(ci, dyi, dxo, Nb, W, H, C, relu_mask);
+    OCR_CHECK_LAUNCH();
+    return OCR_OK;
+}
 extern "C" size_t ocr_bn_workspace_bytes(long M, int C) {
     if (M <= 0 || C <= 0) return 0;
     const long nblk = ceil_div(M, (long)bn_rows_per_block_host(M, 512));
@@ -1373,9 +1444,10 @@
 static constexpr int bn_rows_per_thread() { return 4; }
 static int bn_train_fwd_impl(const void* x, void* y, const float* gamma, const float* beta, float* save_mean,
                              float* save_rstd, long M, int C, float eps, int relu, void* workspace, const void* residual,
-                             int partial_rows, void* pooled, void* stream_) {
+                             int partial_rows, void* pooled, void* codes, void* stream_) {
     hipStream_t stream = (hipStream_t)stream_;
-    if (!x || !y || !gamma || !beta || !save_mean || !save_rstd || !workspace || (C & 7) || C > 2048 || M <= 0)
+    if (codes ? (!pooled || ((size_t)codes & 3)) : !y) return OCR_ERR_INVALID;
+    if (!x || !gamma || !beta || !save_mean || !save_rstd || !workspace || (C & 7) || C > 2048 || M <= 0)
         return OCR_ERR_INVALID;
     int rlanes = 256 / (C >> 3); if (rlanes < 1) return OCR_ERR_INVALID;
     if (partial_rows < 0 || (size_t)partial_rows * 2 * C * sizeof(float) > ocr_bn_workspace_bytes(M, C) - 2 * (size_t)C * sizeof(double)) return OCR_ERR_INVALID;
@@ -1404,7 +1476,7 @@
     const int arows = bn_rows_per_thread() * rlanes;
     if (pooled)
         bn_apply_pool_kernel<<<ceil_div(M / 2, (long)(arows / 2)), 256, 0, stream>>>((const bf16_t*)x, (bf16_t*)y, (bf16_t*)pooled, save_mean, save_rstd,
-                                                                                       gamma, beta, M, C, relu, arows / 2);
+                                                                                       gamma, beta, M, C, relu, arows / 2, (uint32_t*)codes);
     else
         bn_apply_kernel<<<ceil_div(M, (long)arows), 256, 0, stream>>>((const bf16_t*)x, (bf16_t*)y, save_mean, save_rstd, gamma,
                                                                         beta, M, C, relu, arows, (const bf16_t*)residual);
@@ -1413,17 +1485,23 @@
 }
 extern "C" int ocr_bn_train_fwd(const void* x, void* y, const float* gamma, const float* beta, float* save_mean,
                                 float* save_rstd, long M, int C, float eps, int relu, void* workspace, const void* residual, void* stream_) {
-    return bn_train_fwd_impl(x, y, gamma, beta, save_mean, save_rstd, M, C, eps, relu, workspace, residual, 0, nullptr, stream_);
+    return bn_train_fwd_impl(x, y, gamma, beta, save_mean, save_rstd, M, C, eps, relu, workspace, residual, 0, nullptr, nullptr, stream_);
 }
 extern "C" int ocr_bn_train_fwd2(const void* x, void* y, const float* gamma, const float* beta, float* save_mean, float* save_rstd, long M,
                                  int C, float eps, int relu, void* workspace, const void* residual, int partial_rows, void* pooled, void* stream_) {
-    return bn_train_fwd_impl(x, y, gamma, beta, save_mean, save_rstd, M, C, eps, relu, workspace, residual, partial_rows, pooled, stream_);
+    return bn_train_fwd_impl(x, y, gamma, beta, save_mean, save_rstd, M, C, eps, relu, workspace, residual, partial_rows, pooled, nullptr, stream_);
+}
+extern "C" int ocr_bn_train_fwd_codes(const void* x, const float* gamma, const float* beta, float* save_mean, float* save_rstd, long M, int C,
+                                      float eps, int relu, void* workspace, int partial_rows, void* pooled, void* codes, void* stream_) {
+    if (!codes) return OCR_ERR_INVALID;
+    return bn_train_fwd_impl(x, nullptr, gamma, beta, save_mean, save_rstd, M, C, eps, relu, workspace, nullptr, partial_rows, pooled, codes, stream_);
 }
 static int bn_train_bwd_impl(const void* x, const void* y, const void* dy, void* dx, const float* gamma,
                              const float* save_mean, const float* save_rstd, float* dgamma, float* dbeta, long M,
-                             int C, int relu, void* workspace, int pooled_dy, int partial_rows, void* stream_) {
+                             int C, int relu, void* workspace, int pooled_dy, int partial_rows, const void* codes, void* stream_) {
     hipStream_t stream = (hipStream_t)stream_;
-    if (!x || !y || !dy || !dx || !gamma || !save_mean || !save_rstd || !dgamma || !dbeta || !workspace || (C & 7) ||
+    if (codes ? (!pooled_dy || ((size_t)codes & 3)) : !y) return OCR_ERR_INVALID;
+    if (!x || !dy || !dx || !gamma || !save_mean || !save_rstd || !dgamma || !dbeta || !workspace || (C & 7) ||
         C > 2048 || M <= 0 || (pooled_dy && (M & 1)) || partial_rows < 0 || (partial_rows && pooled_dy))
         return OCR_ERR_INVALID;
     const int rpb = bn_rows_per_block_host(M, 512);
@@ -1445,28 +1523,38 @@
     if (partial_rows > nblk) return OCR_ERR_INVALID;
     if (partial_rows) relu = 0;
     else {
-        bn_bwd_stats_kernel<<<nblk, 256, 0, stream>>>((const bf16_t*)x, (const bf16_t*)y, (const bf16_t*)dy, save_mean,
-                                                      save_rstd, part, M, C, rpb, relu, pooled_dy);
+        if (codes) bn_bwd_stats_kernel<true><<<nblk, 256, 0, stream>>>((const bf16_t*)x, (const bf16_t*)y, (const bf16_t*)dy, save_mean,
+                                                                    save_rstd, part, M, C, rpb, relu, pooled_dy, (const uint32_t*)codes);
+        else bn_bwd_stats_kernel<false><<<nblk, 256, 0, stream>>>((const bf16_t*)x, (const bf16_t*)y, (const bf16_t*)dy, save_mean,
+                                                                   save_rstd, part, M, C, rpb, relu, pooled_dy, nullptr);
         OCR_CHECK_LAUNCH();
     }
     bn_bwd_finalize_kernel<<<ceil_div(C, 16), 256, 0, stream>>>(part, partial_rows ? partial_rows : nblk, sums, dgamma, dbeta, C);
     OCR_CHECK_LAUNCH();
     const int arows = bn_rows_per_thread() * (256 / (C >> 3));
-    bn_bwd_apply_kernel<<<ceil_div(M, (long)arows), 256, 0, stream>>>((const bf16_t*)x, (const bf16_t*)y, (const bf16_t*)dy,
-                                                                        (bf16_t*)dx, save_mean, save_rstd, gamma,
-                                                                        sums, dgamma, dbeta, M, C, relu, arows, pooled_dy);
+    if (codes) bn_bwd_apply_kernel<true><<<ceil_div(M, (long)arows), 256, 0, stream>>>((const bf16_t*)x, (const bf16_t*)y, (const bf16_t*)dy,
+                                                                                       (bf16_t*)dx, save_mean, save_rstd, gamma, sums, dgamma, dbeta,
+                                                                                       M, C, relu, arows, pooled_dy, (const uint32_t*)codes);
+    else bn_bwd_apply_kernel<false><<<ceil_div(M, (long)arows), 256, 0, stream>>>((const bf16_t*)x, (const bf16_t*)y, (const bf16_t*)dy,
+                                                                                      (bf16_t*)dx, save_mean, save_rstd, gamma, sums, dgamma, dbeta,
+                                                                                      M, C, relu, arows, pooled_dy, nullptr);
     OCR_CHECK_LAUNCH();
     return OCR_OK;
 }
 extern "C" int ocr_bn_train_bwd(const void* x, const void* y, const void* dy, void* dx, const float* gamma,
                                 const float* save_mean, const float* save_rstd, float* dgamma, float* dbeta, long M,
                                 int C, int relu, void* workspace, void* stream_) {
-    return bn_train_bwd_impl(x, y, dy, dx, gamma, save_mean, save_rstd, dgamma, dbeta, M, C, relu, workspace, 0, 0, stream_);
+    return bn_train_bwd_impl(x, y, dy, dx, gamma, save_mean, save_rstd, dgamma, dbeta, M, C, relu, workspace, 0, 0, nullptr, stream_);
 }
 extern "C" int ocr_bn_train_bwd2(const void* x, const void* y, const void* dy, void* dx, const float* gamma, const float* save_mean,
                                  const float* save_rstd, float* dgamma, float* dbeta, long M, int C, int relu, void* workspace,
                                  int pooled_dy, int partial_rows, void* stream_) {
-    return bn_train_bwd_impl(x, y, dy, dx, gamma, save_mean, save_rstd, dgamma, dbeta, M, C, relu, workspace, pooled_dy, partial_rows, stream_);
+    return bn_train_bwd_impl(x, y, dy, dx, gamma, save_mean, save_rstd, dgamma, dbeta, M, C, relu, workspace, pooled_dy, partial_rows, nullptr, stream_);
+}
+extern "C" int ocr_bn_train_bwd_codes(const void* x, const void* codes, const void* dy, void* dx, const float* gamma, const float* save_mean,
+                                      const float* save_rstd, float* dgamma, float* dbeta, long M, int C, int relu, void* workspace, void* stream_) {
+    if (!codes) return OCR_ERR_INVALID;
+    return bn_train_bwd_impl(x, nullptr, dy, dx, gamma, save_mean, save_rstd, dgamma, dbeta, M, C, relu, workspace, 1, 0, codes, stream_);
 }
 extern "C" int ocr_colsum_bf16(const void* a, float* out, long M, int C, long lda, void* stream) {
     if (!a || !out || (C & 7) || C > 2048 || M <= 0) return OCR_ERR_INVALID;
diff --git a/lstm_ctc_ocr_amd/engine.py b/lstm_ctc_ocr_amd/engine.py
--- a/lstm_ctc_ocr_amd/engine.py
+++ b/lstm_ctc_ocr_amd/engine.py
@@ -140,7 +140,18 @@
             if self.co == 64 and os.environ.get('OCR_CONV1_CODES', '1') != '0':
                 sp.buf[self.key + '/codes'] = torch.empty((s[0] * (s[1] // 2) * (s[2] // 2), 8), dtype=torch.int32, device=dev)
             return
-        sp.buf[self.key + '/y'] = torch.empty(o, dtype=BF16, device=dev)
+        windows = 0
+        if os.environ.get('OCR_POOL_CODES', '1') != '0':
+            p = self.pool_after
+            if self.bn_pool is not None:
+                windows = o[0] * o[1] * o[2] // 2
+            elif (p is not None and ops.conv3x3_pool_supported(s[0], s[1], s[2], self.ci, self.co, p.kw_t, p.kh_f)
+                    and ops.conv3x3_pool_codes_supported(s[0], s[1], s[2], self.ci, self.co, p.kw_t, p.kh_f)):
+                windows = o[0] * (o[1] // p.kw_t) * (o[2] // p.kh_f)
+        if windows:
+            sp.buf[self.key + '/pool_codes'] = torch.empty((windows, self.co // 8), dtype=torch.int32, device=dev)
+        else:
+            sp.buf[self.key + '/y'] = torch.empty(o, dtype=BF16, device=dev)
         sp.buf[self.key + '/dy'] = torch.empty(o, dtype=BF16, device=dev)
         if self.bn:
             sp.buf[self.key + '/z'] = torch.empty(o, dtype=BF16, device=dev)
@@ -192,6 +203,12 @@
             elif need and (have is None or have.numel() < need):
                 sp.buf['wgrad_ws'] = torch.empty(need, dtype=torch.uint8, device=dev)
 
+    def y(self, sp):
+        t = sp.buf.get(self.key + '/y')
+        if t is None:
+            t = sp.buf[self.key + '/y'] = torch.empty(sp.shape[self.key][1], dtype=BF16, device=self.eng.device)
+        return t
+
     def shadow_params(self):
         return [self.name + '/weights'] if self.kind in ('1x1', 'full') else []
 
@@ -218,7 +235,8 @@
             sp.rings_ready = set(getattr(sp, 'lstm_sync_keys', ())) if ones is not None else set()
             sp.rings_armed = ones is not None
             return
-        y = self.y(sp)
+        codes = sp.buf.get(self.key + '/pool_codes') if e.training else None
+        y = None if codes is not None else self.y(sp)
         if self.kind == 'c1':
             ops.conv1_fwd(x, e.param(self.name + '/weights'), bias, relu=self.relu, out=y)
             return
@@ -226,7 +244,10 @@
         relu_now = self.relu and not self.bn
         if self.kind == '3x3' and self.pool_after is not None and self.pool_after.key in sp.fused_pools:
             p = self.pool_after
-            ops.conv3x3_relu_pool(x, self.wpack.view(self.co, 3, 3, self.ci), y, p.y(sp), bias, p.kw_t, p.kh_f)
+            if codes is not None:
+                ops.conv3x3_relu_pool_codes(x, self.wpack.view(self.co, 3, 3, self.ci), None, p.y(sp), codes, bias, p.kw_t, p.kh_f)
+            else:
+                ops.conv3x3_relu_pool(x, self.wpack.view(self.co, 3, 3, self.ci), y, p.y(sp), bias, p.kw_t, p.kh_f)
         elif self.kind == '3x3' and self.bn and sp.bn_stat_rows[self.key]:
             ops.conv3x3_stats(x, self.wpack.view(self.co, 3, 3, self.ci), tgt, sp.buf[self.key + '/bnws'], bias=bias)
         elif self.kind == '3x3':
@@ -248,9 +269,9 @@
             pooled = self.bn_pool.y(sp).view(M // 2, self.co) if self.bn_pool is not None else None
             ops.bn_train_fwd(tgt.view(M, self.co), e.param('%s/%s/gamma' % (self.name, self.name)),
                              e.param('%s/%s/beta' % (self.name, self.name)), BN_EPS, relu,
-                             sp.buf[self.key + '/bnws'], out=y.view(M, self.co),
+                             sp.buf[self.key + '/bnws'], out=None if y is None else y.view(M, self.co),
                              save_mean=sp.buf[self.key + '/mean'], save_rstd=sp.buf[self.key + '/rstd'], residual=res,
-                             partial_rows=sp.bn_stat_rows[self.key], pooled=pooled)
+                             partial_rows=sp.bn_stat_rows[self.key], pooled=pooled, codes=codes)
 
     def bwd(self, sp):
         e = self.eng
@@ -277,18 +298,19 @@
         dz = dy
         if self.bn:
             dz = sp.buf[self.key + '/dz']
-            ymask, relu = self.y(sp), self.relu
+            codes = sp.buf.get(self.key + '/pool_codes')
+            ymask, relu = (self.y(sp) if codes is None else None), self.relu
             if self.mask_from is not None:
                 dy, ymask, relu = self.mask_from.dy(sp), self.mask_from.y(sp), True
             dy2 = dy.view(M, self.co)
             if self.bn_pool is not None:
                 dy2 = self.bn_pool.dy(sp).view(M // 2, self.co)
-            ops.bn_train_bwd(sp.buf[self.key + '/z'].view(M, self.co), ymask.view(M, self.co), dy2,
+            ops.bn_train_bwd(sp.buf[self.key + '/z'].view(M, self.co), None if ymask is None else ymask.view(M, self.co), dy2,
                              e.param('%s/%s/gamma' % (self.name, self.name)), sp.buf[self.key + '/mean'],
                              sp.buf[self.key + '/rstd'], e.grad('%s/%s/gamma' % (self.name, self.name)),
                              e.grad('%s/%s/beta' % (self.name, self.name)), relu, sp.buf[self.key + '/bnws'],
                              out=dz.view(M, self.co), pooled_dy=self.bn_pool is not None,
-                             partial_rows=getattr(sp, 'bn_bwd_rows', {}).get(self.key, 0))
+                             partial_rows=getattr(sp, 'bn_bwd_rows', {}).get(self.key, 0), codes=codes)
         dw = e.grad(self.name + '/weights')
         db = e.grad(self.name + '/biases') if self.biased else None
         if self.kind == 'c1':
@@ -398,7 +420,11 @@
             return
         pdy, finish = self.eng.grad_dst(sp, self.prev)
         if pdy is not None:
-            ops.maxpool_bwd(self.prev.y(sp), self.dy(sp), self.kw_t, self.kh_f, self.prev.mask_in_consumer, out=pdy)
+            codes = sp.buf.get(self.prev.key + '/pool_codes') if getattr(self.prev, 'pool_after', None) is self else None
+            if codes is not None:
+                ops.maxpool_bwd_codes(codes, self.dy(sp), self.kw_t, self.kh_f, self.prev.mask_in_consumer, out=pdy)
+            else:
+                ops.maxpool_bwd(self.prev.y(sp), self.dy(sp), self.kw_t, self.kh_f, self.prev.mask_in_consumer, out=pdy)
             finish()
 
 
diff --git a/lstm_ctc_ocr_amd/ops.py b/lstm_ctc_ocr_amd/ops.py
--- a/lstm_ctc_ocr_amd/ops.py
+++ b/lstm_ctc_ocr_amd/ops.py
@@ -136,6 +136,19 @@
     return out, pooled
 
 
+def conv3x3_pool_codes_supported(Nb, W, H, Cin, Cout, kw, kh):
+    return bool(nat.lib().ocr_conv3x3_pool_codes_supported(Nb, W, H, Cin, Cout, kw, kh))
+
+
+def conv3x3_relu_pool_codes(x, wpack, out, pooled, codes, bias, kw, kh):
+    Nb, W, H, Cin = x.shape
+    Cout = wpack.shape[0]
+    assert codes.dtype == torch.int32 and codes.numel() == Nb * (W // kw) * (H // kh) * (Cout // 8), (codes.dtype, tuple(codes.shape))
+    call("ocr_conv3x3_relu_pool_codes_bf16", ptr(_dev(x)), ptr(wpack), ptr(out), ptr(pooled), ptr(codes), Nb, W, H, Cin, Cout, ptr(bias),
+         kw, kh, _st())
+    return out, pooled, codes
+
+
 def gemm_tn(A, B, out, *, Mk=None, I=None, J=None, lda=None, ldb=None, ldo=None, row_group=0, row_skip=0,
             a_row_off=0, scale=1.0, splits=0, colsum=None):
     Mk = B.shape[0] if Mk is None else Mk
@@ -309,13 +322,31 @@
     return out
 
 
+def maxpool_bwd_codes(codes, dy, kw, kh, relu_mask, out=None):
+    Nb, Wo, Ho, C = dy.shape
+    W, H = Wo * kw, Ho * kh
+    assert codes.dtype == torch.int32 and codes.numel() == Nb * Wo * Ho * (C // 8), (codes.dtype, tuple(codes.shape))
+    if out is None:
+        out = torch.empty((Nb, W, H, C), dtype=BF16, device=dy.device)
+    call("ocr_maxpool_bwd_codes", ptr(_dev(codes)), ptr(dy), ptr(out), Nb, W, H, C, kw, kh, int(relu_mask), _st())
+    return out
+
+
 def bn_workspace(M, C, device):
     return torch.empty(int(nat.lib().ocr_bn_workspace_bytes(int(M), int(C))), dtype=torch.uint8, device=device)
 
 
 def bn_train_fwd(x2d, gamma, beta, eps, relu, workspace, out=None, save_mean=None, save_rstd=None, residual=None, partial_rows=0,
-                 pooled=None):
+                 pooled=None, codes=None):
     M, C = x2d.shape
+    if codes is not None:
+        assert pooled is not None and residual is None and out is None
+        assert codes.dtype == torch.int32 and tuple(codes.shape) == (M // 2, C // 8), (codes.dtype, tuple(codes.shape))
+        if save_mean is None: save_mean = torch.empty(C, dtype=F32, device=x2d.device)
+        if save_rstd is None: save_rstd = torch.empty(C, dtype=F32, device=x2d.device)
+        call("ocr_bn_train_fwd_codes", ptr(_dev(x2d)), ptr(gamma), ptr(beta), ptr(save_mean), ptr(save_rstd), M, C,
+             float(eps), int(relu), ptr(workspace), int(partial_rows), ptr(pooled), ptr(codes), _st())
+        return None, save_mean, save_rstd
     if out is None: out = torch.empty_like(x2d)
     if save_mean is None: save_mean = torch.empty(C, dtype=F32, device=x2d.device)
     if save_rstd is None: save_rstd = torch.empty(C, dtype=F32, device=x2d.device)
@@ -328,9 +359,16 @@
     return out, save_mean, save_rstd
 
 
-def bn_train_bwd(x2d, y2d, dy2d, gamma, save_mean, save_rstd, dgamma, dbeta, relu, workspace, out=None, pooled_dy=False, partial_rows=0):
+def bn_train_bwd(x2d, y2d, dy2d, gamma, save_mean, save_rstd, dgamma, dbeta, relu, workspace, out=None, pooled_dy=False, partial_rows=0,
+                 codes=None):
     M, C = x2d.shape
     if out is None: out = torch.empty_like(x2d)
+    if codes is not None:
+        assert pooled_dy and not partial_rows and tuple(dy2d.shape) == (M // 2, C)
+        assert codes.dtype == torch.int32 and tuple(codes.shape) == (M // 2, C // 8), (codes.dtype, tuple(codes.shape))
+        call("ocr_bn_train_bwd_codes", ptr(_dev(x2d)), ptr(codes), ptr(dy2d), ptr(out), ptr(gamma), ptr(save_mean), ptr(save_rstd),
+             ptr(dgamma), ptr(dbeta), M, C, int(relu), ptr(workspace), _st())
+        return out
     if pooled_dy or partial_rows:
         assert tuple(dy2d.shape) == ((M // 2, C) if pooled_dy else (M, C))
         call("ocr_bn_train_bwd2", ptr(_dev(x2d)), ptr(y2d), ptr(dy2d), ptr(out), ptr(gamma), ptr(save_mean), ptr(save_rstd),
```

Result: faster. 57500 images/sec, median of 6 (+1.1%).
